# kessel/dune-pnp

Hardware: NVIDIA B200
Metric: newton_step_dofs_per_s (higher is better)
Workload: dtype f64

## Files before the change

### dune_pnp_b200/capi.py

```python
import ctypes as C
import os

import numpy as np

_HERE = os.path.dirname(os.path.abspath(__file__))
LIB_PATH = os.path.join(_HERE, "libpnp_b200.so")

OP_PB, OP_POISSON, OP_DIFFUSION, OP_MASS, OP_PNP = range(5)
JAC_FD_FAITHFUL, JAC_ANALYTIC = 0, 1
SOLVER_BCGS, SOLVER_CG = 0, 1
PREC_NONE, PREC_JACOBI, PREC_SSOR, PREC_ILU0, PREC_AMG = range(5)
TIME_ALEXANDER2, TIME_IMPLICIT_EULER = 0, 1
STATUS = {0: "PNP_OK", 1: "PNP_E_NOT_CONVERGED", 2: "PNP_E_LINEAR_SOLVER", 3: "PNP_E_LINE_SEARCH", 4: "PNP_E_NAN",
          5: "PNP_E_BREAKDOWN", 6: "PNP_E_CUDA", 7: "PNP_E_CONFIG", 8: "PNP_E_ARG", 9: "PNP_E_MESH"}

_dp = C.POINTER(C.c_double)
_ip = C.POINTER(C.c_int)


class LinResult(C.Structure):
    _fields_ = [("converged", C.c_int), ("iterations", C.c_int), ("reduction", C.c_double), ("conv_rate", C.c_double),
                ("seconds", C.c_double), ("status", C.c_int)]


class NewtonOpts(C.Structure):
    _fields_ = [("reduction", C.c_double), ("abs_limit", C.c_double), ("min_linear_reduction", C.c_double),
                ("reassemble_threshold", C.c_double), ("max_iterations", C.c_int),
                ("line_search_max_iterations", C.c_int), ("damping", C.c_double), ("jac_mode", C.c_int),
                ("fd_epsilon", C.c_double), ("verbosity", C.c_int), ("line_search_strategy", C.c_int)]


class NewtonResult(C.Structure):
    _fields_ = [("converged", C.c_int), ("iterations", C.c_int), ("first_defect", C.c_double), ("defect", C.c_double),
                ("reduction", C.c_double), ("linear_iterations", C.c_int), ("line_search_trials", C.c_int),
                ("jacobian_assemblies", C.c_int), ("residual_assemblies", C.c_int), ("seconds_assembly", C.c_double),
                ("seconds_solve", C.c_double), ("seconds_total", C.c_double), ("n_history", C.c_int),
                ("defect_history", C.c_double * 64), ("linear_iterations_history", C.c_int * 64)]


class PnpError(RuntimeError):
    def __init__(self, status, msg):
        super().__init__("%s: %s" % (STATUS.get(status, status), msg))
        self.status = status


_LIB = None


def lib():
    global _LIB
    if _LIB is None:
        if not os.path.exists(LIB_PATH):
            raise ImportError("libpnp_b200.so is missing: run `python -c 'import __graft_entry__ as g; g.build()'` "
                              "(make -C dune_pnp_b200/csrc)")
        try:
            import importlib.util
            for pkg, names in (("nvidia.nccl", ["libnccl.so.2"]), ("nvidia.nvjitlink", ["libnvJitLink.so.12"]),
                               ("nvidia.cublas", ["libcublasLt.so.12", "libcublas.so.12"]),
                               ("nvidia.cusparse", ["libcusparse.so.12"]), ("nvidia.cusolver", ["libcusolver.so.11"])):
                spec = importlib.util.find_spec(pkg)
                if spec is None or not spec.submodule_search_locations:
                    continue
                for nm in names:
                    cand = os.path.join(list(spec.submodule_search_locations)[0], "lib", nm)
                    if os.path.exists(cand):
                        C.CDLL(cand, mode=C.RTLD_GLOBAL)
        except Exception:
            pass
        L = C.CDLL(LIB_PATH)
        L.pnp_last_error.restype = C.c_char_p
        L.pnp_launch_count.restype = C.c_long
        _LIB = L
    return _LIB


def _d(a):
    return None if a is None else a.ctypes.data_as(_dp)


def _i(a):
    return None if a is None else a.ctypes.data_as(_ip)


def tune(name, value):
    st = lib().pnp_tune(name.encode(), C.c_double(value))
    if st != 0:
        raise PnpError(st, "unknown tuning knob " + name)


class Context:

    def __init__(self, device=0, parent=None):
        self._h = C.c_void_p()
        self._children = []
        if parent is not None:
            st = lib().pnp_ctx_create_child(parent._h, C.byref(self._h))
            parent._children.append(self)
        else:
            st = lib().pnp_ctx_create(device, C.byref(self._h))
        if st != 0:
            raise PnpError(st, "cannot create a context on CUDA device %d (no CPU fallback exists)" % device)

    def close(self):
        if self._h:
            lib().pnp_ctx_destroy(self._h)
            self._h = C.c_void_p()

    def __del__(self):
        try:
            self.close()
        except Exception:
            pass

    def _ck(self, st):
        if st != 0:
            raise PnpError(st, lib().pnp_last_error(self._h).decode())

    def profile_spmv(self, enable):
        self._ck(lib().pnp_profile_spmv(self._h, int(enable)))

    def profile_spmv_get(self):
        n = (C.c_long * 3)(); ms = (C.c_double * 3)()
        self._ck(lib().pnp_profile_spmv_get(self._h, n, ms))
        return list(n), list(ms)

    def profile_bytes(self, reset=False):
        out = (C.c_double * 6)()
        self._ck(lib().pnp_profile_bytes(self._h, int(reset), out))
        return dict(zip(("spmv_fine", "spmv_coarse", "assembly", "blas1", "transfer", "dense"), list(out)))

    def profiler_range(self, start):
        self._ck(lib().pnp_profiler_range(self._h, int(start)))

    def timer_start(self):
        self._ck(lib().pnp_timer_start(self._h))

    def timer_stop(self):
        ms = C.c_double()
        self._ck(lib().pnp_timer_stop(self._h, C.byref(ms)))
        return ms.value

    def launch_count(self):
        return lib().pnp_launch_count(self._h)

    def mesh_set(self, x, y, tri, ba, bb, bphys):
        x = np.ascontiguousarray(x, dtype=np.float64); y = np.ascontiguousarray(y, dtype=np.float64)
        tri = np.ascontiguousarray(tri, dtype=np.int32); ba = np.ascontiguousarray(ba, dtype=np.int32)
        bb = np.ascontiguousarray(bb, dtype=np.int32); bphys = np.ascontiguousarray(bphys, dtype=np.int32)
        self._ck(lib().pnp_mesh_set(self._h, C.c_long(len(x)), _d(x), _d(y), C.c_long(len(tri)), _i(tri), C.c_long(len(ba)),
                                    _i(ba), _i(bb), _i(bphys)))

    def mesh_read_gmsh(self, path):
        self._ck(lib().pnp_mesh_read_gmsh(self._h, path.encode()))

    def mesh_refine(self, levels):
        self._ck(lib().pnp_mesh_refine(self._h, levels))

    def carry_set(self, vecs):
        arr = (C.c_int * len(vecs))(*vecs)
        self._ck(lib().pnp_carry_set(self._h, arr, len(vecs)))

    def carry_get(self, index, vec):
        self._ck(lib().pnp_carry_get(self._h, index, vec))

    def carry_set_host(self, field):
        field = np.ascontiguousarray(field, dtype=np.float64)
        self._ck(lib().pnp_carry_set_host(self._h, field.shape[0] if field.ndim == 2 else 1, _d(field)))

    def carry_get_host(self, index, fields):
        out = np.zeros((fields, self.mesh_sizes()["nv"]))
        self._ck(lib().pnp_carry_get_host(self._h, index, _d(out)))
        return out

    def mesh_set_local(self, n_own, x, y, tri, ba, bb, bphys):
        x = np.ascontiguousarray(x, dtype=np.float64); y = np.ascontiguousarray(y, dtype=np.float64)
        tri = np.ascontiguousarray(tri, dtype=np.int32); ba = np.ascontiguousarray(ba, dtype=np.int32)
        bb = np.ascontiguousarray(bb, dtype=np.int32); bphys = np.ascontiguousarray(bphys, dtype=np.int32)
        self._ck(lib().pnp_mesh_set_local(self._h, C.c_long(len(x)), C.c_long(n_own), _d(x), _d(y), C.c_long(len(tri)), _i(tri),
                                          C.c_long(len(ba)), _i(ba), _i(bb), _i(bphys)))

    def mesh_owned(self):
        n = C.c_long()
        self._ck(lib().pnp_mesh_owned(self._h, C.byref(n)))
        return n.value

    @staticmethod
    def comm_unique_id():
        buf = C.create_string_buffer(128)
        if lib().pnp_comm_unique_id(buf) != 0:
            raise PnpError(6, "ncclGetUniqueId failed")
        return buf.raw

    def comm_init(self, rank, world, unique_id):
        self._ck(lib().pnp_comm_init(self._h, rank, world, C.c_char_p(unique_id) if world > 1 else None))

    def halo_set(self, nbr, send_ptr, send_idx, recv_ptr):
        nbr = np.ascontiguousarray(nbr, dtype=np.int32); send_ptr = np.ascontiguousarray(send_ptr, dtype=np.int32)
        send_idx = np.ascontiguousarray(send_idx, dtype=np.int32); recv_ptr = np.ascontiguousarray(recv_ptr, dtype=np.int32)
        self._ck(lib().pnp_halo_set(self._h, len(nbr), _i(nbr), _i(send_ptr), _i(send_idx), _i(recv_ptr)))

    def mg_push_level(self, child, par0, par1):
        par0 = np.ascontiguousarray(par0, dtype=np.int32); par1 = np.ascontiguousarray(par1, dtype=np.int32)
        self._ck(lib().pnp_mg_push_level(self._h, child._h, _i(par0), _i(par1)))

    def mg_set_coarse_global(self, gid, n_global):
        gid = np.ascontiguousarray(gid, dtype=np.int32)
        self._ck(lib().pnp_mg_set_coarse_global(self._h, _i(gid), C.c_long(n_global)))

    def mg_set_coarse_replica(self, replica, gid, n_global):
        gid = np.ascontiguousarray(gid, dtype=np.int32)
        self._ck(lib().pnp_mg_set_coarse_replica(self._h, replica._h, _i(gid), C.c_long(n_global)))

    def mg_set_coarse_aggregates(self, agg, n_agg):
        agg = np.ascontiguousarray(agg, dtype=np.int32)
        self._ck(lib().pnp_mg_set_coarse_aggregates(self._h, _i(agg), C.c_long(n_agg)))

    def halo_exchange(self, vec):
        self._ck(lib().pnp_halo_exchange(self._h, vec))

    def mesh_finalize(self, renumber=True):
        self._ck(lib().pnp_mesh_finalize(self._h, int(renumber)))

    def mesh_sizes(self):
        v = [C.c_long() for _ in range(4)]
        self._ck(lib().pnp_mesh_sizes(self._h, *[C.byref(a) for a in v]))
        return dict(nv=v[0].value, nT=v[1].value, nB=v[2].value, nslots=v[3].value)

    def mesh_get(self):
        s = self.mesh_sizes()
        x = np.zeros(s["nv"]); y = np.zeros(s["nv"]); tri = np.zeros((s["nT"], 3), dtype=np.int32)
        ba = np.zeros(s["nB"], dtype=np.int32); bb = np.zeros(s["nB"], dtype=np.int32); ph = np.zeros(s["nB"], dtype=np.int32)
        self._ck(lib().pnp_mesh_get(self._h, _d(x), _d(y), _i(tri), _i(ba), _i(bb), _i(ph)))
        return dict(x=x, y=y, tri=tri, ba=ba, bb=bb, bphys=ph)

    def params_set(self, sys, surf):
        sys = np.ascontiguousarray(sys, dtype=np.float64); surf = np.ascontiguousarray(surf, dtype=np.float64)
        self._ck(lib().pnp_params_set(self._h, _d(sys), _d(surf)))

    def params_read(self, path):
        self._ck(lib().pnp_params_read(self._h, path.encode()))

    def params_get(self):
        sys = np.zeros(16)
        self._ck(lib().pnp_params_get(self._h, _d(sys), None, None, 0))
        surf = np.zeros((int(sys[0]), 9)); buf = C.create_string_buffer(512)
        self._ck(lib().pnp_params_get(self._h, _d(sys), _d(surf), buf, 512))
        return sys, surf, buf.value.decode()

    def operator(self, op, comp0=0):
        h = C.c_int()
        self._ck(lib().pnp_operator_create(self._h, op, comp0, C.byref(h)))
        return h.value

    def operator_set_coefficient(self, op, which, vec):
        self._ck(lib().pnp_operator_set_coefficient(self._h, op, which, vec))

    def operator_set_valency(self, op, valency):
        self._ck(lib().pnp_operator_set_valency(self._h, op, C.c_double(valency)))

    def constraints(self, op, fields):
        out = np.zeros(fields * self.ndof(), dtype=np.int8)
        self._ck(lib().pnp_constraints_get(self._h, op, out.ctypes.data_as(C.c_char_p)))
        return out.astype(bool)

    def pattern(self, op, fields):
        nv = self.ndof()
        nnz = C.c_long(); rowptr = np.zeros(fields * nv + 1, dtype=np.int32)
        self._ck(lib().pnp_pattern_get(self._h, op, C.byref(nnz), _i(rowptr), None))
        col = np.zeros(nnz.value, dtype=np.int32)
        self._ck(lib().pnp_pattern_get(self._h, op, C.byref(nnz), _i(rowptr), _i(col)))
        return rowptr, col

    def vec(self, fields, host=None):
        h = C.c_int()
        self._ck(lib().pnp_vec_create(self._h, fields, C.byref(h)))
        if host is not None:
            self.upload(h.value, host)
        return h.value
# ... 158 lines not shown
```

### dune_pnp_b200/csrc/pnp_amg.cu

```cuda
#include <cub/cub.cuh>
#include <cusolverDn.h>

#include <chrono>
#include <cmath>
#include <cstdlib>
#include <cstring>

#include "pnp_common.cuh"
#include "pnp_spmv_tma.cuh"
#include "pnp_sweep.cuh"

namespace pnp {

std::shared_ptr<SweepPlan> sweep_plan_build(Ctx&, const SweepView&, int F);
void sweep_gs(Ctx&, const SweepPlan&, const SweepView&, const double* vals, long stride, const double* d, double* x, int dir);

namespace {

constexpr int BLK = 256;

struct Level {
  int nv = 0; long nslots = 0;
  const int* rp = nullptr; const unsigned* col = nullptr; const double* vals = nullptr;
  DBuf<int> rp_own; DBuf<unsigned> col_own; DBuf<double> vals_own;
  DBuf<double> dinv, x, x2, b, r;
  double lmax = 2.0;
  DBuf<int> agg, par1;
  DBuf<int> agg_ptr, agg_mem;
  DBuf<int> seg_ptr, seg_items;
  DBuf<unsigned char> seg_w;
  double alpha = 1.0;
  Ctx* lc = nullptr;
  Vec u; Matrix Amat;
  const unsigned char* dm = nullptr;
  bool redisc = false;
  DBuf<XY> xy_own; DBuf<unsigned char> dmask_own;
  std::shared_ptr<SweepPlan> gs_plan;
};

}

struct Amg {
  int NP = 1, F = 1;
  bool symbolic = false;
  long nv0 = -1, nslots0 = -1;
  long mg_epoch = -1;
  double sym_key = 0.0;
  double omega = 0.7, alpha = 1.6;
  int coarse_sweeps = 40;
  int gamma = 1;
  int wlevels = 99;
  int smoother = 0;
  double cheb_ratio = 8.0;
  int comp0 = 0;
  int pre_steps = -1, post_steps = -1;
  int dense_max = 4096, dense_n = 0;
  cusolverDnHandle_t cus = nullptr;
  DBuf<double> dense, dense_work;
  DBuf<int> dense_piv, dense_info;
  bool distributed = false;
  bool redisc = false;
  DBuf<double> grhs;
  std::unique_ptr<Solver> rep_solver; Matrix rep_A; Vec rep_u; DBuf<double> rep_x;
  int n_geo = 0;
  std::vector<std::unique_ptr<Level>> L;
  DBuf<unsigned char> tmp;
  void* temp(size_t bytes) { if (bytes > tmp.n) tmp.alloc(bytes); return tmp.p; }
  cudaGraphExec_t cg_exec = nullptr;
  bool cg_failed = false;
  int cg_calls = 0;
  double cg_key[8] = {0, 0, 0, 0, 0, 0, 0, 0};
  std::vector<std::pair<double*, double*>> cg_before, cg_after;
  long cg_launches = 0; double cg_bytes[Ctx::ACC_N] = {0, 0, 0, 0, 0, 0};
  void cg_reset() { if (cg_exec) cudaGraphExecDestroy(cg_exec); cg_exec = nullptr; cg_calls = 0; }
  ~Amg() { if (cg_exec) cudaGraphExecDestroy(cg_exec); if (cus) cusolverDnDestroy(cus); }
};

namespace {

__device__ __forceinline__ unsigned hash32(unsigned x) {
  x ^= x >> 16; x *= 0x7feb352du; x ^= x >> 15; x *= 0x846ca68bu; x ^= x >> 16;
  return x;
}
__global__ void k_mis_select(const int* __restrict__ rp, const unsigned* __restrict__ col, int nv,
                             const unsigned char* __restrict__ st, unsigned char* __restrict__ st_out) {
  for (int v = blockIdx.x * blockDim.x + threadIdx.x; v < nv; v += gridDim.x * blockDim.x) {
    unsigned char s = st[v];
    if (s == 0) {
      const unsigned pv = hash32((unsigned)v);
      bool win = true;
      for (int k = rp[v] + 1; k < rp[v + 1]; k++) {
        const int w = (int)(col[k] & STAR_VMASK);
        if (w >= nv || w == v || st[w] != 0) continue;
        const unsigned pw = hash32((unsigned)w);
        if (pw > pv || (pw == pv && w > v)) { win = false; break; }
      }
      if (win) s = 1;
    }
    st_out[v] = s;
  }
}
__global__ void k_mis_cover(const int* __restrict__ rp, const unsigned* __restrict__ col, int nv,
                            unsigned char* __restrict__ st, int* __restrict__ undecided) {
  int local = 0;
  for (int v = blockIdx.x * blockDim.x + threadIdx.x; v < nv; v += gridDim.x * blockDim.x) {
    if (st[v] != 0) continue;
    bool covered = false;
    for (int k = rp[v] + 1; k < rp[v + 1]; k++) {
      const int w = (int)(col[k] & STAR_VMASK);
      if (w < nv && st[w] == 1) { covered = true; break; }
    }
    if (covered) st[v] = 2; else local++;
  }
  if (local) atomicAdd(undecided, local);
}
__global__ void k_root_flag(const unsigned char* __restrict__ st, int nv, int* __restrict__ flag) {
  for (int v = blockIdx.x * blockDim.x + threadIdx.x; v < nv; v += gridDim.x * blockDim.x) flag[v] = st[v] == 1;
}
__global__ void k_attach(const int* __restrict__ rp, const unsigned* __restrict__ col, const double* __restrict__ vals,
                         int nv, const unsigned char* __restrict__ st, const int* __restrict__ root_id,
                         int* __restrict__ agg) {
  for (int v = blockIdx.x * blockDim.x + threadIdx.x; v < nv; v += gridDim.x * blockDim.x) {
    if (st[v] == 1) { agg[v] = root_id[v]; continue; }
    double best = -1.0; int bw = -1;
    for (int k = rp[v] + 1; k < rp[v + 1]; k++) {
      const int w = (int)(col[k] & STAR_VMASK);
      if (w >= nv || st[w] != 1) continue;
      const double s = fabs(vals[k]);
      if (s > best || (s == best && w < bw)) { best = s; bw = w; }
    }
    agg[v] = root_id[bw];
  }
}
__global__ void k_coarse_keys(const int* __restrict__ rp, const unsigned* __restrict__ col, int nv,
                              const int* __restrict__ agg, uint64_t* __restrict__ keys, int* __restrict__ slot_id) {
  for (int v = blockIdx.x * blockDim.x + threadIdx.x; v < nv; v += gridDim.x * blockDim.x) {
    const unsigned I = (unsigned)agg[v];
    for (int k = rp[v]; k < rp[v + 1]; k++) {
      const unsigned w = col[k] & STAR_VMASK;
      if (w >= (unsigned)nv) { keys[k] = ~0ull; slot_id[k] = k; continue; }
      const unsigned J = (unsigned)agg[w];
      keys[k] = ((uint64_t)I << 32) | (J == I ? 0u : J + 1u);
      slot_id[k] = k;
    }
  }
}
__global__ void k_coarse_cols(const uint64_t* __restrict__ ukeys, long n, unsigned* __restrict__ col) {
  for (long i = blockIdx.x * (long)blockDim.x + threadIdx.x; i < n; i += (long)gridDim.x * blockDim.x) {
    const unsigned lo = (unsigned)(ukeys[i] & 0xffffffffu);
    col[i] = lo == 0 ? (unsigned)(ukeys[i] >> 32) : lo - 1u;
  }
}
__global__ void k_row_starts(const uint64_t* __restrict__ ukeys, long n, int nc, int* __restrict__ rp) {
  for (int I = blockIdx.x * blockDim.x + threadIdx.x; I <= nc; I += gridDim.x * blockDim.x)
    rp[I] = (int)lower_bound_u64(ukeys, n, (uint64_t)(unsigned)I << 32);
}
__global__ void k_lower_bounds_i32(const int* __restrict__ sorted, int n, int m, int* __restrict__ out) {
  for (int I = blockIdx.x * blockDim.x + threadIdx.x; I <= m; I += gridDim.x * blockDim.x) {
    int lo = 0, hi = n;
    while (lo < hi) { int mid = (lo + hi) >> 1; if (sorted[mid] < I) lo = mid + 1; else hi = mid; }
    out[I] = lo;
  }
}
__global__ void k_iota(int* a, int n) {
  for (int i = blockIdx.x * blockDim.x + threadIdx.x; i < n; i += gridDim.x * blockDim.x) a[i] = i;
}

template <int NP>
__global__ void k_galerkin(const int* __restrict__ seg_ptr, const int* __restrict__ seg_items,
                           const unsigned char* __restrict__ seg_w, long nsc, const double* __restrict__ vf, long nsf, double* __restrict__ vc,
                           const unsigned char* __restrict__ dmask, const unsigned* __restrict__ colf, const int* __restrict__ rpf,
                           int comp0) {
  for (long cs = blockIdx.x * (long)blockDim.x + threadIdx.x; cs < nsc; cs += (long)gridDim.x * blockDim.x) {
    double acc[NP];
#pragma unroll
    for (int p = 0; p < NP; p++) acc[p] = 0.0;
    constexpr int U = 4;
    const int t1 = seg_ptr[cs + 1];
    for (int t0 = seg_ptr[cs]; t0 < t1; t0 += U) {
      int s[U]; double w[U]; double v[U][NP];
#pragma unroll
      for (int q = 0; q < U; q++) {
        const bool ok = t0 + q < t1;
        s[q] = ok ? seg_items[t0 + q] : -1;
        const unsigned char wc = (ok && seg_w) ? seg_w[t0 + q] : 0;
        w[q] = ok ? (wc == 0 ? 1.0 : (wc == 1 ? 0.5 : 0.25)) : 0.0;
      }
#pragma unroll
      for (int q = 0; q < U; q++)
#pragma unroll
        for (int p = 0; p < NP; p++) v[q][p] = s[q] >= 0 ? vf[p * nsf + s[q]] : 0.0;
      if (dmask) {
#pragma unroll
        for (int q = 0; q < U; q++) {
          if (s[q] < 0) continue;
          const unsigned wv = colf[s[q]] & STAR_VMASK;
          const unsigned m = dmask[wv];
          if (m && rpf[wv] == s[q]) {
            if (NP == 1) { if ((m >> comp0) & 1u) v[q][0] = 0.0; }
            else if (NP == PNP_COMPACT_PLANES) { if (m & 1u) v[q][0] = 0.0; }
            else {
              if (m & 1u) v[q][0] = 0.0;
              if (m & 2u) v[q][NP == 7 ? 4 : 0] = 0.0;
              if (m & 4u) v[q][NP == 7 ? 6 : 0] = 0.0;
            }
          }
        }
      }
#pragma unroll
      for (int q = 0; q < U; q++)
        if (s[q] >= 0) {
#pragma unroll
          for (int p = 0; p < NP; p++) acc[p] += w[q] * v[q][p];
        }
    }
#pragma unroll
    for (int p = 0; p < NP; p++) vc[p * nsc + cs] = acc[p];
  }
}
template <int NP>
__global__ void k_dinv(const int* __restrict__ rp, const double* __restrict__ vals, long stride, int nv,
                       double* __restrict__ dinv) {
  for (int v = blockIdx.x * blockDim.x + threadIdx.x; v < nv; v += gridDim.x * blockDim.x) {
    const int s = rp[v];
    if (NP == 1) { const double d = vals[s]; dinv[v] = d != 0.0 ? 1.0 / d : 0.0; }
// ... 74 lines not shown
      const double w = (par1 && par1[v] >= 0) ? 0.5 : 1.0;
#pragma unroll
      for (int k = 0; k < F; k++) acc[k] += w * r[F * v + k];
    }
#pragma unroll
    for (int k = 0; k < F; k++) bc[(long)F * I + k] = acc[k];
  }
}
template <int F>
__global__ void k_prolong(const int* __restrict__ agg, const int* __restrict__ par1, int nv, const double* __restrict__ xc,
                          double alpha, double* __restrict__ x, const unsigned char* __restrict__ dmask, int comp0) {
  for (int v = blockIdx.x * blockDim.x + threadIdx.x; v < nv; v += gridDim.x * blockDim.x) {
    const long I = agg[v];
    const long J = par1 ? par1[v] : -1;
    const unsigned m = dmask ? (F == 3 ? dmask[v] : (dmask[v] >> comp0) & 1u) : 0u;
#pragma unroll
    for (int k = 0; k < F; k++)
      if (!((m >> k) & 1u))
        x[(long)F * v + k] += alpha * (J >= 0 ? 0.5 * (xc[F * I + k] + xc[F * J + k]) : xc[F * I + k]);
  }
}
__global__ void k_level_geometry(const int* __restrict__ int2ext_c, const int* __restrict__ ext2int_f, const XY* __restrict__ xy_f,
                                 const unsigned char* __restrict__ dmask_f, int nvc, XY* __restrict__ xy_c,
                                 unsigned char* __restrict__ dmask_c) {
  for (int i = blockIdx.x * blockDim.x + threadIdx.x; i < nvc; i += gridDim.x * blockDim.x) {
    const int j = ext2int_f[int2ext_c[i]];
    xy_c[i] = xy_f[j]; dmask_c[i] = dmask_f[j];
  }
}
__global__ void k_geo_parents(const int* __restrict__ int2ext_f, int nvf, int nvc, const uint64_t* __restrict__ edges,
                              const int* __restrict__ ext2int_c, int* __restrict__ par0, int* __restrict__ par1) {
  for (int i = blockIdx.x * blockDim.x + threadIdx.x; i < nvf; i += gridDim.x * blockDim.x) {
    const int e = int2ext_f[i];
    if (e < nvc) { par0[i] = ext2int_c[e]; par1[i] = -1; }
    else {
      const uint64_t k = edges[e - nvc];
      par0[i] = ext2int_c[(int)(k >> 32)]; par1[i] = ext2int_c[(int)(k & 0xffffffffu)];
    }
  }
}
__global__ void k_geo_pairs(const int* __restrict__ par0, const int* __restrict__ par1, int nvf, int nrows_c,
                            int* __restrict__ key, int* __restrict__ val) {
  for (int i = blockIdx.x * blockDim.x + threadIdx.x; i < nvf; i += gridDim.x * blockDim.x) {
    key[2 * i] = (par0[i] >= 0 && par0[i] < nrows_c) ? par0[i] : 0x7fffffff; val[2 * i] = i;
    key[2 * i + 1] = (par1[i] >= 0 && par1[i] < nrows_c) ? par1[i] : 0x7fffffff; val[2 * i + 1] = i;
  }
}
template <int F>
__global__ void k_inject(const int* __restrict__ par0, const int* __restrict__ par1, int nvf, const double* __restrict__ uf,
                         double* __restrict__ uc) {
  for (int i = blockIdx.x * blockDim.x + threadIdx.x; i < nvf; i += gridDim.x * blockDim.x)
    if (par1[i] < 0 && par0[i] >= 0) {
#pragma unroll
      for (int k = 0; k < F; k++) uc[(long)F * par0[i] + k] = uf[(long)F * i + k];
    }
}
template <int F>
__global__ void k_mask_dirichlet(double* __restrict__ b, const unsigned char* __restrict__ dmask, int nv, int comp0) {
  for (int v = blockIdx.x * blockDim.x + threadIdx.x; v < nv; v += gridDim.x * blockDim.x) {
    const unsigned m = F == 3 ? dmask[v] : (dmask[v] >> comp0) & 1u;
#pragma unroll
    for (int k = 0; k < F; k++) if ((m >> k) & 1u) b[(long)F * v + k] = 0.0;
  }
}
template <int NP>
__global__ void k_dense_fill_global(const int* __restrict__ rp, const unsigned* __restrict__ col, const double* __restrict__ vals,
                                    long stride, int nrows, const int* __restrict__ gid, double* __restrict__ Ad, long n,
                                    const unsigned char* __restrict__ dmask, int comp0) {
  constexpr int F = NP == 1 ? 1 : 3;
  for (int r = blockIdx.x * blockDim.x + threadIdx.x; r < nrows; r += gridDim.x * blockDim.x) {
    const long rg = gid[r];
    for (int s = rp[r]; s < rp[r + 1]; s++) {
      const long cg = gid[col[s] & STAR_VMASK];
      const unsigned dm = (dmask && s == rp[r]) ? dmask[r] : 0u;
      if (NP == 1) { if (!((dm >> comp0) & 1u)) atomicAdd(&Ad[cg * n + rg], vals[s]); }
      else {
        const PnpBlock B = pnp_block_at<NP>(vals, stride, s);
#pragma unroll
        for (int ki = 0; ki < 3; ki++)
#pragma unroll
          for (int kj = 0; kj < 3; kj++)
            if (pnp_plane(ki, kj) >= 0 && !(ki == kj && ((dm >> ki) & 1u))) atomicAdd(&Ad[(F * cg + kj) * n + F * rg + ki], B.at(ki, kj));
      }
    }
  }
}
template <int F>
__global__ void k_to_global(const double* __restrict__ loc, const int* __restrict__ gid, int nrows, double* __restrict__ glob) {
  for (int v = blockIdx.x * blockDim.x + threadIdx.x; v < nrows; v += gridDim.x * blockDim.x)
#pragma unroll
    for (int k = 0; k < F; k++) atomicAdd(&glob[(long)F * gid[v] + k], loc[(long)F * v + k]);
}
template <int F>
__global__ void k_add_from_global(const double* __restrict__ glob, const int* __restrict__ gid, int nrows, double alpha,
                                  double* __restrict__ x, const unsigned char* __restrict__ dmask, int comp0) {
  for (int v = blockIdx.x * blockDim.x + threadIdx.x; v < nrows; v += gridDim.x * blockDim.x) {
    const unsigned m = F == 3 ? dmask[v] : (dmask[v] >> comp0) & 1u;
#pragma unroll
    for (int k = 0; k < F; k++) if (!((m >> k) & 1u)) x[(long)F * v + k] += alpha * glob[(long)F * gid[v] + k];
  }
}
template <int F>
__global__ void k_from_global(const double* __restrict__ glob, const int* __restrict__ gid, int nloc, double* __restrict__ loc) {
  for (int v = blockIdx.x * blockDim.x + threadIdx.x; v < nloc; v += gridDim.x * blockDim.x)
#pragma unroll
    for (int k = 0; k < F; k++) loc[(long)F * v + k] = glob[(long)F * gid[v] + k];
}
__device__ __forceinline__ int find_slot(const int* rp, const unsigned* col, int I, int J) {
  for (int s = rp[I]; s < rp[I + 1]; s++) if ((int)(col[s] & STAR_VMASK) == J) return s;
  return -1;
}
__global__ void k_geo_items(const int* __restrict__ rpf, const unsigned* __restrict__ colf, int nvf,
                            const int* __restrict__ par0, const int* __restrict__ par1, const int* __restrict__ rpc,
                            const unsigned* __restrict__ colc, int* __restrict__ key, unsigned* __restrict__ val,
                            int* __restrict__ err) {
  for (int i = blockIdx.x * blockDim.x + threadIdx.x; i < nvf; i += gridDim.x * blockDim.x) {
    const int I[2] = {par0[i], par1[i]};
    for (int s = rpf[i]; s < rpf[i + 1]; s++) {
      const int j = (int)(colf[s] & STAR_VMASK);
      const int J[2] = {par0[j], par1[j]};
#pragma unroll
      for (int a = 0; a < 2; a++)
#pragma unroll
        for (int b = 0; b < 2; b++) {
          const long o = 4l * s + 2 * a + b;
          if (I[a] < 0 || J[b] < 0) { key[o] = 0x7fffffff; val[o] = 0; continue; }
          const int cs = find_slot(rpc, colc, I[a], J[b]);
          if (cs < 0) { atomicExch(err, 1); key[o] = 0x7fffffff; val[o] = 0; continue; }
          const unsigned wc = (I[1] >= 0 ? 1u : 0u) + (J[1] >= 0 ? 1u : 0u);
          key[o] = cs; val[o] = (unsigned)s | (wc << 29);
        }
    }
  }
}
__global__ void k_geo_unpack(const unsigned* __restrict__ val, long n, int* __restrict__ items, unsigned char* __restrict__ w) {
  for (long t = blockIdx.x * (long)blockDim.x + threadIdx.x; t < n; t += (long)gridDim.x * blockDim.x) {
    items[t] = (int)(val[t] & 0x1fffffffu); w[t] = (unsigned char)(val[t] >> 29);
  }
}

#define KL(c, kern, n, ...)                                                                              \
  do { kern<<<grid_for((n), BLK), BLK, 0, (c).stream>>>(__VA_ARGS__); PNP_CHECK_LAUNCH(); (c).launches++; } while (0)

template <int EPI>
void level_op(Ctx& c, const Amg& A, const Level& l, const double* x, const double* b, double* y, double omega_or_c2 = -1.0,
              double c1 = 0.0, double* dvec = nullptr) {
  StarOpArgs a{l.rp, l.col, l.vals, l.nslots, l.nv, x, y};
  a.b = b; a.dinv = l.dinv.p; a.block = A.F == 3; a.omega = omega_or_c2 < 0 ? A.omega : omega_or_c2; a.c1 = c1; a.dvec = dvec;
  const bool fine = &l == A.L[0].get();
  if (A.distributed) halo_exchange(*l.lc, const_cast<double*>(x), A.F);
  if (fine) c.prof_mark(EPI == EPI_RESIDUAL ? 1 : 2);
  launch_star_op_auto<EPI, 0>(c, A.NP, a, fine);
  if (fine) c.prof_mark();
}

bool coarsen(Ctx& c, Amg& A, int li) {
  Level& f = *A.L[li];
  const int nv = f.nv;
  DBuf<unsigned char> st(nv), st2(nv);
  st.zero(c.stream);
  DBuf<int> d_und(1);
  for (int round = 0; round < 200; round++) {
    KL(c, k_mis_select, nv, f.rp, f.col, nv, st.p, st2.p);
    std::swap(st.p, st2.p);
    d_und.zero(c.stream);
    KL(c, k_mis_cover, nv, f.rp, f.col, nv, st.p, d_und.p);
    int und = 0;
    d_und.download(&und, 1, c.stream);
    if (und == 0) break;
    PNP_REQUIRE(round < 199, PNP_E_ARG, "AMG: independent-set selection did not terminate");
  }
  DBuf<int> flag(nv), root_id(nv);
  KL(c, k_root_flag, nv, st.p, nv, flag.p);
  size_t bytes = 0;
  cub::DeviceScan::ExclusiveSum(nullptr, bytes, flag.p, root_id.p, nv, c.stream);
  PNP_CUDA(cub::DeviceScan::ExclusiveSum(A.temp(bytes), bytes, flag.p, root_id.p, nv, c.stream));
  int last_id = 0, last_flag = 0;
  PNP_CUDA(cudaMemcpyAsync(&last_id, root_id.p + nv - 1, sizeof(int), cudaMemcpyDeviceToHost, c.stream));
  PNP_CUDA(cudaMemcpyAsync(&last_flag, flag.p + nv - 1, sizeof(int), cudaMemcpyDeviceToHost, c.stream));
  PNP_CUDA(cudaStreamSynchronize(c.stream));
  const int nc = last_id + last_flag;
  if (nc < 1 || nc > 0.8 * nv) return false;
  f.alpha = A.alpha;
  f.agg.alloc(nv);
  KL(c, k_attach, nv, f.rp, f.col, f.vals, nv, st.p, root_id.p, f.agg.p);
  {
    DBuf<int> ids(nv), agg_sorted(nv);
    f.agg_mem.alloc(nv); f.agg_ptr.alloc(nc + 1);
    KL(c, k_iota, nv, ids.p, nv);
    cub::DeviceRadixSort::SortPairs(nullptr, bytes, f.agg.p, agg_sorted.p, ids.p, f.agg_mem.p, nv, 0, 32, c.stream);
    PNP_CUDA(cub::DeviceRadixSort::SortPairs(A.temp(bytes), bytes, f.agg.p, agg_sorted.p, ids.p, f.agg_mem.p, nv, 0, 32,
                                            c.stream));
    KL(c, k_lower_bounds_i32, nc + 1, agg_sorted.p, nv, nc, f.agg_ptr.p);
  }
  auto nl = std::make_unique<Level>();
  {
    const long ns = f.nslots;
    PNP_REQUIRE(ns < (1l << 31), PNP_E_MESH, "AMG: too many matrix slots on one level");
    DBuf<uint64_t> keys(ns), skeys(ns), ukeys(ns);
    DBuf<int> slot(ns), counts(ns + 1), d_nu(1);
    f.seg_items.alloc(ns);
    KL(c, k_coarse_keys, nv, f.rp, f.col, nv, f.agg.p, keys.p, slot.p);
    cub::DeviceRadixSort::SortPairs(nullptr, bytes, keys.p, skeys.p, slot.p, f.seg_items.p, (int)ns, 0, 64, c.stream);
    PNP_CUDA(cub::DeviceRadixSort::SortPairs(A.temp(bytes), bytes, keys.p, skeys.p, slot.p, f.seg_items.p, (int)ns, 0, 64,
                                            c.stream));
    cub::DeviceRunLengthEncode::Encode(nullptr, bytes, skeys.p, ukeys.p, counts.p, d_nu.p, (int)ns, c.stream);
    PNP_CUDA(cub::DeviceRunLengthEncode::Encode(A.temp(bytes), bytes, skeys.p, ukeys.p, counts.p, d_nu.p, (int)ns, c.stream));
    int nu = 0;
    d_nu.download(&nu, 1, c.stream);
    {
      uint64_t lastkey = 0;
      PNP_CUDA(cudaMemcpyAsync(&lastkey, ukeys.p + (nu - 1), sizeof(uint64_t), cudaMemcpyDeviceToHost, c.stream));
      PNP_CUDA(cudaStreamSynchronize(c.stream));
      if (lastkey == ~0ull) nu--;
    }
    nl->nv = nc; nl->nslots = nu;
    PNP_CUDA(cudaMemsetAsync(counts.p + nu, 0, sizeof(int), c.stream));
    f.seg_ptr.alloc((size_t)nu + 1);
    cub::DeviceScan::ExclusiveSum(nullptr, bytes, counts.p, f.seg_ptr.p, nu + 1, c.stream);
    PNP_CUDA(cub::DeviceScan::ExclusiveSum(A.temp(bytes), bytes, counts.p, f.seg_ptr.p, nu + 1, c.stream));
    nl->rp_own.alloc((size_t)nc + 1); nl->col_own.alloc(nu);
    KL(c, k_row_starts, nc + 1, ukeys.p, (long)nu, nc, nl->rp_own.p);
    KL(c, k_coarse_cols, nu, ukeys.p, (long)nu, nl->col_own.p);
    c.launches += 8;
    PNP_CUDA(cudaStreamSynchronize(c.stream));
  }
  nl->vals_own.alloc((size_t)A.NP * nl->nslots);
  nl->rp = nl->rp_own.p; nl->col = nl->col_own.p; nl->vals = nl->vals_own.p;
  A.L.push_back(std::move(nl));
  return true;
}

void coarsen_geometric(Ctx& c, Amg& A, int li, const HierLevel& h, const int* int2ext_f, bool redisc) {
  Level& f = *A.L[li];
  const int nvf = f.nv, nvc = (int)h.nv;
  size_t bytes = 0;
  f.agg.alloc(nvf); f.par1.alloc(nvf);
  KL(c, k_geo_parents, nvf, int2ext_f, nvf, nvc, h.edges.p, h.ext2int.p, f.agg.p, f.par1.p);
  {
    DBuf<int> key(2 * (size_t)nvf), val(2 * (size_t)nvf), skey(2 * (size_t)nvf), sval(2 * (size_t)nvf);
    KL(c, k_geo_pairs, nvf, f.agg.p, f.par1.p, nvf, nvc, key.p, val.p);
    cub::DeviceRadixSort::SortPairs(nullptr, bytes, key.p, skey.p, val.p, sval.p, 2 * nvf, 0, 32, c.stream);
    PNP_CUDA(cub::DeviceRadixSort::SortPairs(A.temp(bytes), bytes, key.p, skey.p, val.p, sval.p, 2 * nvf, 0, 32, c.stream));
    f.agg_ptr.alloc((size_t)nvc + 1);
    KL(c, k_lower_bounds_i32, nvc + 1, skey.p, 2 * nvf, nvc, f.agg_ptr.p);
    int nvalid = 0;
    PNP_CUDA(cudaMemcpyAsync(&nvalid, f.agg_ptr.p + nvc, sizeof(int), cudaMemcpyDeviceToHost, c.stream));
    PNP_CUDA(cudaStreamSynchronize(c.stream));
    f.agg_mem.alloc(nvalid);
    PNP_CUDA(cudaMemcpyAsync(f.agg_mem.p, sval.p, (size_t)nvalid * sizeof(int), cudaMemcpyDeviceToDevice, c.stream));
    PNP_CUDA(cudaStreamSynchronize(c.stream));
  }
  auto nl = std::make_unique<Level>();
  nl->nv = nvc; nl->nslots = h.nslots; nl->rp = h.rp.p; nl->col = h.adj.p;
  nl->redisc = redisc;
  if (redisc) {
    nl->xy_own.alloc(nvc); nl->dmask_own.alloc(nvc);
    KL(c, k_level_geometry, nvc, h.int2ext.p, c.ext2int.p, c.xy.p, c.dmask.p, nvc, nl->xy_own.p, nl->dmask_own.p);
    nl->dm = nl->dmask_own.p;
    nl->u.fields = A.F; nl->u.d.alloc((size_t)A.F * nvc);
  } else {
    const long n4 = 4 * f.nslots;
    PNP_REQUIRE(n4 < (1l << 31) && f.nslots < (1l << 29), PNP_E_MESH, "multigrid: too many matrix slots on one level");
    DBuf<int> key(n4), skey(n4), err(1);
    DBuf<unsigned> val(n4), sval(n4);
    err.zero(c.stream);
    KL(c, k_geo_items, nvf, f.rp, f.col, nvf, f.agg.p, f.par1.p, nl->rp, nl->col, key.p, val.p, err.p);
    int herr = 0;
    err.download(&herr, 1, c.stream);
    PNP_REQUIRE(herr == 0, PNP_E_MESH, "multigrid: refinement levels are not nested");
    cub::DeviceRadixSort::SortPairs(nullptr, bytes, key.p, skey.p, val.p, sval.p, (int)n4, 0, 32, c.stream);
    PNP_CUDA(cub::DeviceRadixSort::SortPairs(A.temp(bytes), bytes, key.p, skey.p, val.p, sval.p, (int)n4, 0, 32, c.stream));
    key.release(); val.release();
    f.seg_ptr.alloc((size_t)nl->nslots + 1);
    KL(c, k_lower_bounds_i32, nl->nslots + 1, skey.p, (int)n4, (int)nl->nslots, f.seg_ptr.p);
    int nvalid = 0;
    PNP_CUDA(cudaMemcpyAsync(&nvalid, f.seg_ptr.p + nl->nslots, sizeof(int), cudaMemcpyDeviceToHost, c.stream));
    PNP_CUDA(cudaStreamSynchronize(c.stream));
    f.seg_items.alloc(nvalid); f.seg_w.alloc(nvalid);
    KL(c, k_geo_unpack, nvalid, sval.p, (long)nvalid, f.seg_items.p, f.seg_w.p);
    PNP_CUDA(cudaStreamSynchronize(c.stream));
    c.launches += 4;
  }
  f.alpha = 1.0;
  nl->vals_own.alloc((size_t)A.NP * nl->nslots);
  nl->vals = nl->vals_own.p;
  A.L.push_back(std::move(nl));
}

void alloc_work(Ctx& c, Amg& A, Level& l) {
  const size_t n = (size_t)A.F * l.nv, nall = (A.distributed && l.lc) ? (size_t)A.F * l.lc->nv : n;
  l.dinv.alloc(A.F == 3 ? 9 * (size_t)l.nv : n); l.x.alloc(nall); l.x2.alloc(nall); l.b.alloc(nall); l.r.alloc(nall);
  l.x.zero(c.stream); l.x2.zero(c.stream); l.b.zero(c.stream); l.r.zero(c.stream);
}

void coarsen_distributed(Ctx& c, Amg& A, int li, MgLevelRef& ref) {
  Level& f = *A.L[li];
  Ctx& fc = *f.lc; Ctx& kc = *ref.lc;
  const int nvf_all = (int)fc.nv, nvc = (int)kc.n_own;
  size_t bytes = 0;
  f.agg.alloc(nvf_all); f.par1.alloc(nvf_all);
  PNP_CUDA(cudaMemcpyAsync(f.agg.p, ref.par0.p, nvf_all * sizeof(int), cudaMemcpyDeviceToDevice, c.stream));
  PNP_CUDA(cudaMemcpyAsync(f.par1.p, ref.par1.p, nvf_all * sizeof(int), cudaMemcpyDeviceToDevice, c.stream));
  {
    DBuf<int> key(2 * (size_t)nvf_all), val(2 * (size_t)nvf_all), skey(2 * (size_t)nvf_all), sval(2 * (size_t)nvf_all);
    KL(c, k_geo_pairs, nvf_all, f.agg.p, f.par1.p, nvf_all, nvc, key.p, val.p);
// ... 115 lines not shown
  for (int r = blockIdx.x * blockDim.x + threadIdx.x; r < nv; r += gridDim.x * blockDim.x)
    for (int s = rp[r]; s < rp[r + 1]; s++) {
      const long cidx = col[s] & STAR_VMASK;
      if (cidx >= nv) continue;
      if (NP == 1) Ad[cidx * n + r] = vals[s];
      else {
        const PnpBlock B = pnp_block_at<NP>(vals, stride, s);
#pragma unroll
        for (int ki = 0; ki < 3; ki++)
#pragma unroll
          for (int kj = 0; kj < 3; kj++)
            if (pnp_plane(ki, kj) >= 0) Ad[(F * cidx + kj) * n + F * r + ki] = B.at(ki, kj);
      }
    }
}
__global__ void k_dense_fix_diag(double* __restrict__ Ad, long n) {
  for (long i = blockIdx.x * (long)blockDim.x + threadIdx.x; i < n; i += (long)gridDim.x * blockDim.x)
    if (Ad[i * n + i] == 0.0) Ad[i * n + i] = 1.0;
}
#define PNP_CUSOLVER(call)                                                                                          \
  do { cusolverStatus_t s_ = (call); if (s_ != CUSOLVER_STATUS_SUCCESS)                                             \
    throw ::pnp::Error(PNP_E_CUDA, std::string(#call) + " -> cusolver status " + std::to_string((int)s_)); } while (0)

void dense_factor(Ctx& c, Amg& A) {
  Level& l = *A.L.back();
  const long n = (long)A.F * l.nv;
  A.dense_n = (int)n;
  if (!A.cus) PNP_CUSOLVER(cusolverDnCreate(&A.cus));
  PNP_CUSOLVER(cusolverDnSetStream(A.cus, c.stream));
  if (A.dense.n != (size_t)(n * n)) { A.dense.alloc(n * n); A.dense_piv.alloc(n); A.dense_info.alloc(1); }
  A.dense.zero(c.stream);
  if (A.NP == 1) KL(c, k_dense_fill<1>, l.nv, l.rp, l.col, l.vals, l.nslots, l.nv, A.dense.p, n);
  else if (A.NP == PNP_COMPACT_PLANES) KL(c, k_dense_fill<PNP_COMPACT_PLANES>, l.nv, l.rp, l.col, l.vals, l.nslots, l.nv, A.dense.p, n);
  else KL(c, k_dense_fill<7>, l.nv, l.rp, l.col, l.vals, l.nslots, l.nv, A.dense.p, n);
  KL(c, k_dense_fix_diag, n, A.dense.p, n);
  int lwork = 0;
  PNP_CUSOLVER(cusolverDnDgetrf_bufferSize(A.cus, (int)n, (int)n, A.dense.p, (int)n, &lwork));
  if (A.dense_work.n < (size_t)lwork) A.dense_work.alloc(lwork);
  PNP_CUSOLVER(cusolverDnDgetrf(A.cus, (int)n, (int)n, A.dense.p, (int)n, A.dense_work.p, A.dense_piv.p, A.dense_info.p));
  c.acct(Ctx::ACC_DENSE, 24.0 * (double)n * (double)n);
  int info = 0;
  A.dense_info.download(&info, 1, c.stream);
  PNP_REQUIRE(info == 0, PNP_E_BREAKDOWN, "multigrid: coarsest-level matrix is singular (LU info " + std::to_string(info) + ")");
}
void dense_solve(Ctx& c, Amg& A, Level& l) {
  const long n = A.dense_n;
  PNP_CUDA(cudaMemcpyAsync(l.x.p, l.b.p, n * sizeof(double), cudaMemcpyDeviceToDevice, c.stream));
  PNP_CUSOLVER(cusolverDnDgetrs(A.cus, CUBLAS_OP_N, (int)n, 1, A.dense.p, (int)n, A.dense_piv.p, l.x.p, (int)n, A.dense_info.p));
  c.launches += 2; c.acct(Ctx::ACC_DENSE, 8.0 * (double)n * (double)n);
}

void dense_factor_global(Ctx& c, Amg& A) {
  Level& l = *A.L.back();
  const long n = (long)A.F * c.mg_nglobal;
  A.dense_n = (int)n;
  if (!A.cus) PNP_CUSOLVER(cusolverDnCreate(&A.cus));
  PNP_CUSOLVER(cusolverDnSetStream(A.cus, c.stream));
  if (A.dense.n != (size_t)(n * n)) { A.dense.alloc(n * n); A.dense_piv.alloc(n); A.dense_info.alloc(1); A.grhs.alloc(n); }
  A.dense.zero(c.stream);
  const unsigned char* dm = c.mg_aggregated ? l.lc->dmask.p : nullptr;
  if (A.NP == 1) KL(c, k_dense_fill_global<1>, l.nv, l.rp, l.col, l.vals, l.nslots, l.nv, c.mg_gid.p, A.dense.p, n, dm, A.comp0);
  else if (A.NP == PNP_COMPACT_PLANES)
    KL(c, k_dense_fill_global<PNP_COMPACT_PLANES>, l.nv, l.rp, l.col, l.vals, l.nslots, l.nv, c.mg_gid.p, A.dense.p, n, dm, A.comp0);
  else KL(c, k_dense_fill_global<7>, l.nv, l.rp, l.col, l.vals, l.nslots, l.nv, c.mg_gid.p, A.dense.p, n, dm, A.comp0);
  allreduce_sum(c, A.dense.p, (size_t)(n * n));
  KL(c, k_dense_fix_diag, n, A.dense.p, n);
  int lwork = 0;
  PNP_CUSOLVER(cusolverDnDgetrf_bufferSize(A.cus, (int)n, (int)n, A.dense.p, (int)n, &lwork));
  if (A.dense_work.n < (size_t)lwork) A.dense_work.alloc(lwork);
  static const bool timing = std::getenv("PNP_AMG_TIMING") != nullptr;
  if (timing) PNP_CUDA(cudaStreamSynchronize(c.stream));
  const auto t0 = std::chrono::steady_clock::now();
  PNP_CUSOLVER(cusolverDnDgetrf(A.cus, (int)n, (int)n, A.dense.p, (int)n, A.dense_work.p, A.dense_piv.p, A.dense_info.p));
  int info = 0;
  A.dense_info.download(&info, 1, c.stream);
  if (timing) std::printf("[amg] rank %d global dense LU n = %ld: %.1f ms\n", c.rank, n,
                          1e3 * std::chrono::duration<double>(std::chrono::steady_clock::now() - t0).count());
  PNP_REQUIRE(info == 0, PNP_E_BREAKDOWN, "multigrid: coarsest-level matrix is singular (LU info " + std::to_string(info) + ")");
}
void dense_correct_aggregated(Ctx& c, Amg& A, Level& l) {
  const long n = A.dense_n;
  A.grhs.zero(c.stream);
  if (A.F == 1) KL(c, k_to_global<1>, l.nv, l.r.p, c.mg_gid.p, l.nv, A.grhs.p);
  else KL(c, k_to_global<3>, l.nv, l.r.p, c.mg_gid.p, l.nv, A.grhs.p);
  allreduce_sum(c, A.grhs.p, (size_t)n);
  PNP_CUSOLVER(cusolverDnDgetrs(A.cus, CUBLAS_OP_N, (int)n, 1, A.dense.p, (int)n, A.dense_piv.p, A.grhs.p, (int)n, A.dense_info.p));
  if (A.F == 1) KL(c, k_add_from_global<1>, l.nv, A.grhs.p, c.mg_gid.p, l.nv, A.alpha, l.x.p, l.lc->dmask.p, A.comp0);
  else KL(c, k_add_from_global<3>, l.nv, A.grhs.p, c.mg_gid.p, l.nv, A.alpha, l.x.p, l.lc->dmask.p, A.comp0);
  c.launches += 2;
}
void dense_solve_global(Ctx& c, Amg& A, Level& l) {
  const long n = A.dense_n;
  A.grhs.zero(c.stream);
  if (A.F == 1) KL(c, k_to_global<1>, l.nv, l.b.p, c.mg_gid.p, l.nv, A.grhs.p);
  else KL(c, k_to_global<3>, l.nv, l.b.p, c.mg_gid.p, l.nv, A.grhs.p);
  allreduce_sum(c, A.grhs.p, (size_t)n);
  PNP_CUSOLVER(cusolverDnDgetrs(A.cus, CUBLAS_OP_N, (int)n, 1, A.dense.p, (int)n, A.dense_piv.p, A.grhs.p, (int)n, A.dense_info.p));
  const int nloc = (int)l.lc->nv;
  if (A.F == 1) KL(c, k_from_global<1>, nloc, A.grhs.p, c.mg_gid.p, nloc, l.x.p);
  else KL(c, k_from_global<3>, nloc, A.grhs.p, c.mg_gid.p, nloc, l.x.p);
  c.launches += 2;
}

}
void amg_setup(Ctx& c, Solver& S, const Matrix& M);
void amg_apply(Ctx& c, Solver& S, const Matrix&, const double* d, double* y);
namespace {
void replica_setup(Ctx& c, Amg& A) {
  Ctx& rc = *c.mg_replica;
  Level& l = *A.L.back();
  const long n = (long)A.F * c.mg_nglobal;
  A.dense_n = (int)n;
  if (A.grhs.n != (size_t)n) { A.grhs.alloc(n); A.rep_x.alloc(n); A.rep_u.d.alloc(n); }
  A.rep_u.fields = A.F;
  A.rep_u.d.zero(c.stream);
  if (A.F == 1) KL(c, k_to_global<1>, l.nv, l.u.d.p, c.mg_gid.p, l.nv, A.rep_u.d.p);
  else KL(c, k_to_global<3>, l.nv, l.u.d.p, c.mg_gid.p, l.nv, A.rep_u.d.p);
  allreduce_sum(c, A.rep_u.d.p, (size_t)n);
  Operator op = c.last_op; op.aux0 = op.aux1 = -1;
  A.rep_A.op = op.op; A.rep_A.nplanes = A.NP;
  if (A.rep_A.vals.n != (size_t)A.NP * rc.nslots) A.rep_A.vals.alloc((size_t)A.NP * rc.nslots);
  rc.launches = 0;
  assemble_jacobian(rc, op, A.rep_u, A.rep_A, c.last_mode, c.last_eps);
  if (!A.rep_solver) { A.rep_solver = std::make_unique<Solver>(); A.rep_solver->prec = PNP_PREC_AMG; }
  auto& ro = A.rep_solver->opts;
  ro["amg_geometric"] = 1;  ro["amg_omega"] = A.omega; ro["amg_alpha"] = A.alpha; ro["amg_gamma"] = A.gamma;
  ro["amg_dense_max"] = A.dense_max; ro["amg_coarse_sweeps"] = A.coarse_sweeps; ro["amg_smoother"] = A.smoother;
  ro["amg_cheb_ratio"] = A.cheb_ratio; ro["amg_pre_steps"] = A.pre_steps; ro["amg_post_steps"] = A.post_steps;
  amg_setup(rc, *A.rep_solver, A.rep_A);
  c.absorb(rc);
}
void replica_solve(Ctx& c, Amg& A, Level& l, int nu) {
  Ctx& rc = *c.mg_replica;
  const long n = (long)A.F * c.mg_nglobal;
  A.grhs.zero(c.stream);
  if (A.F == 1) KL(c, k_to_global<1>, l.nv, l.b.p, c.mg_gid.p, l.nv, A.grhs.p);
  else KL(c, k_to_global<3>, l.nv, l.b.p, c.mg_gid.p, l.nv, A.grhs.p);
  allreduce_sum(c, A.grhs.p, (size_t)n);
  A.rep_solver->prec_steps = nu;
  rc.launches = 0;
  amg_apply(rc, *A.rep_solver, A.rep_A, A.grhs.p, A.rep_x.p);
  const int nloc = (int)l.lc->nv;
  if (A.F == 1) KL(c, k_from_global<1>, nloc, A.rep_x.p, c.mg_gid.p, nloc, l.x.p);
  else KL(c, k_from_global<3>, nloc, A.rep_x.p, c.mg_gid.p, nloc, l.x.p);
  c.absorb(rc); c.launches += 2;
}

void jacobi0(Ctx& c, Amg& A, Level& l, double omega, double* dvec) {
  if (A.F == 1) KL(c, k_jacobi0<1>, l.nv, l.dinv.p, l.b.p, omega, l.x.p, l.nv, dvec);
  else KL(c, k_jacobi0<3>, l.nv, l.dinv.p, l.b.p, omega, l.x.p, l.nv, dvec);
  c.acct(Ctx::ACC_TRANSFER, ((A.F == 3 ? 72.0 : 8.0) + 16.0 * A.F + (dvec ? 8.0 * A.F : 0.0)) * l.nv);
}

void smooth(Ctx& c, Amg& A, Level& l, int steps, bool zero) {
  const long n = (long)A.F * l.nv;
  if (steps <= 0) { if (zero) PNP_CUDA(cudaMemsetAsync(l.x.p, 0, n * sizeof(double), c.stream)); return; }
  if (A.smoother == 0) {
    int s = 0;
    if (zero) { jacobi0(c, A, l, A.omega, nullptr); s = 1; }
    for (; s < steps; s++) { level_op<2>(c, A, l, l.x.p, l.b.p, l.x2.p); std::swap(l.x.p, l.x2.p); }
    return;
  }
  if (A.smoother == 2) {
    const bool finest = &l == A.L[0].get();
    const SweepView V{l.rp, l.col, finest ? c.int2ext.p : nullptr, l.nv};
    if (!l.gs_plan) l.gs_plan = sweep_plan_build(c, V, A.F);
    if (zero) PNP_CUDA(cudaMemsetAsync(l.x.p, 0, n * sizeof(double), c.stream));
    for (int s = 0; s < steps; s++) {
      sweep_gs(c, *l.gs_plan, V, l.vals, l.nslots, l.b.p, l.x.p, +1);
      sweep_gs(c, *l.gs_plan, V, l.vals, l.nslots, l.b.p, l.x.p, -1);
    }
    c.acct(finest ? Ctx::ACC_SPMV_FINE : Ctx::ACC_SPMV_COARSE, 2.0 * steps * ((8.0 * A.NP + 4.0) * (double)l.nslots + 24.0 * n));
    return;
  }
  const double lmx = 1.1 * l.lmax, lmn = l.lmax / A.cheb_ratio;
  const double theta = 0.5 * (lmx + lmn), delta = 0.5 * (lmx - lmn), sigma = theta / delta;
  double rho = 1.0 / sigma;
  int s = 0;
  if (zero) { jacobi0(c, A, l, 1.0 / theta, l.r.p); s = 1; }
  else { level_op<3>(c, A, l, l.x.p, l.b.p, l.x2.p, 1.0 / theta, 0.0, l.r.p); std::swap(l.x.p, l.x2.p); s = 1; }
  for (; s < steps; s++) {
    const double rho_new = 1.0 / (2.0 * sigma - rho);
    level_op<3>(c, A, l, l.x.p, l.b.p, l.x2.p, 2.0 * rho_new / delta, rho_new * rho, l.r.p);
    std::swap(l.x.p, l.x2.p);
    rho = rho_new;
  }
}

void cycle(Ctx& c, Amg& A, int li, int nu, int comp0, bool zero);

void coarse_correction(Ctx& c, Amg& A, int nu, int comp0) {
  auto direct = [&] {
    const int visits = 0 < A.wlevels ? A.gamma : 1;
    for (int g = 0; g < visits; g++) cycle(c, A, 1, nu, comp0, g == 0);
  };
  auto snapshot = [&](std::vector<std::pair<double*, double*>>& v) {
    v.clear();
    for (size_t li = 1; li < A.L.size(); li++) v.push_back({A.L[li]->x.p, A.L[li]->x2.p});
  };
  auto restore = [&](const std::vector<std::pair<double*, double*>>& v) {
    for (size_t li = 1; li < A.L.size(); li++) { A.L[li]->x.p = v[li - 1].first; A.L[li]->x2.p = v[li - 1].second; }
  };
  cudaStreamCaptureStatus cap = cudaStreamCaptureStatusNone;
  PNP_CUDA(cudaStreamIsCapturing(c.stream, &cap));
  if (!tune().graph || A.cg_failed || A.smoother != 0 || cap != cudaStreamCaptureStatusNone) { direct(); return; }
  const double key[8] = {(double)nu, A.omega, (double)A.gamma, (double)A.wlevels, (double)A.pre_steps, (double)A.post_steps,
                         (double)A.coarse_sweeps, (double)comp0 + 16.0 * A.dense_n};
  if (A.cg_exec && std::memcmp(key, A.cg_key, sizeof key) != 0) A.cg_reset();
  if (!A.cg_exec) {
    if (A.cg_calls++ < 1) { direct(); return; }
    std::memcpy(A.cg_key, key, sizeof key);
    snapshot(A.cg_before);
    const long l0 = c.launches;
    double b0[Ctx::ACC_N];
    for (int k = 0; k < Ctx::ACC_N; k++) b0[k] = c.alg_bytes[k];
    cudaGraph_t graph = nullptr;
    bool ok = cudaStreamBeginCapture(c.stream, cudaStreamCaptureModeThreadLocal) == cudaSuccess;
    if (ok) {
      try { direct(); } catch (const Error&) { ok = false; }
      if (cudaStreamEndCapture(c.stream, &graph) != cudaSuccess || !graph) ok = false;
    }
    if (ok && cudaGraphInstantiate(&A.cg_exec, graph, 0) != cudaSuccess) { ok = false; A.cg_exec = nullptr; }
    if (graph) cudaGraphDestroy(graph);
    A.cg_launches = c.launches - l0; c.launches = l0;
    for (int k = 0; k < Ctx::ACC_N; k++) { A.cg_bytes[k] = c.alg_bytes[k] - b0[k]; c.alg_bytes[k] = b0[k]; }
    snapshot(A.cg_after);
    if (!ok) {
      cudaGetLastError();
      A.cg_failed = true; A.cg_exec = nullptr;
      restore(A.cg_before);
      direct();
      return;
    }
  }
  restore(A.cg_before);
  PNP_CUDA(cudaGraphLaunch(A.cg_exec, c.stream));
  restore(A.cg_after);
  c.launches += A.cg_launches;
  for (int k = 0; k < Ctx::ACC_N; k++) c.alg_bytes[k] += A.cg_bytes[k];
}

void cycle(Ctx& c, Amg& A, int li, int nu, int comp0, bool zero) {
  Level& l = *A.L[li];
  const bool coarsest = li + 1 == (int)A.L.size();
  if (coarsest && A.dense_n > 0 && A.distributed && c.mg_aggregated) {
    smooth(c, A, l, nu, zero);
    level_op<1>(c, A, l, l.x.p, l.b.p, l.r.p);
    dense_correct_aggregated(c, A, l);
    smooth(c, A, l, nu, false);
    return;
  }
  if (coarsest && A.dense_n > 0) {
    if (A.distributed && c.mg_replica) replica_solve(c, A, l, nu);
    else if (A.distributed) dense_solve_global(c, A, l);
    else dense_solve(c, A, l);
    return;
  }
  const int nu_pre = A.pre_steps >= 0 ? A.pre_steps : nu, nu_post = A.post_steps >= 0 ? A.post_steps : nu;
  smooth(c, A, l, coarsest ? A.coarse_sweeps : nu_pre, zero);
  if (coarsest) return;
  Level& nx = *A.L[li + 1];
  level_op<1>(c, A, l, l.x.p, l.b.p, l.r.p);
  if (A.distributed) halo_exchange(*l.lc, l.r.p, A.F);
  if (A.F == 1) KL(c, k_restrict<1>, nx.nv, l.agg_ptr.p, l.agg_mem.p, l.par1.p, nx.nv, l.r.p, nx.b.p);
  else KL(c, k_restrict<3>, nx.nv, l.agg_ptr.p, l.agg_mem.p, l.par1.p, nx.nv, l.r.p, nx.b.p);
  c.acct(Ctx::ACC_TRANSFER, (8.0 * A.F + 4.0) * l.nv + 4.0 * (double)l.agg_mem.n + (8.0 * A.F + 4.0) * nx.nv);
  if (nx.dm) {
    if (A.F == 1) KL(c, k_mask_dirichlet<1>, nx.nv, nx.b.p, nx.dm, nx.nv, comp0);
    else KL(c, k_mask_dirichlet<3>, nx.nv, nx.b.p, nx.dm, nx.nv, comp0);
    c.acct(Ctx::ACC_TRANSFER, 1.0 * nx.nv);
  }
  if (li == 0) coarse_correction(c, A, nu, comp0);
  else {
    const int visits = li < A.wlevels ? A.gamma : 1;
    for (int g = 0; g < visits; g++) cycle(c, A, li + 1, nu, comp0, g == 0);
  }
  if (A.distributed && !(li + 2 == (int)A.L.size() && A.dense_n > 0 && !c.mg_aggregated)) halo_exchange(*nx.lc, nx.x.p, A.F);
  const unsigned char* dm = l.dm;
  if (A.F == 1) KL(c, k_prolong<1>, l.nv, l.agg.p, l.par1.p, l.nv, nx.x.p, l.alpha, l.x.p, dm, comp0);
  else KL(c, k_prolong<3>, l.nv, l.agg.p, l.par1.p, l.nv, nx.x.p, l.alpha, l.x.p, dm, comp0);
  c.acct(Ctx::ACC_TRANSFER, (16.0 * A.F + 9.0) * l.nv + 8.0 * A.F * nx.nv);
  smooth(c, A, l, nu_post, false);
}

}

int amg_graph_state(const Solver& S) { return !S.amg ? 0 : (S.amg->cg_exec ? 1 : (S.amg->cg_failed ? -1 : 0)); }

void amg_setup(Ctx& c, Solver& S, const Matrix& M) {
  if (!S.amg) S.amg = std::make_shared<Amg>();
  Amg& A = *S.amg;
  const int comp0 = M.comp0;
  A.comp0 = comp0;
  const bool want_redisc = S.opt("amg_geometric", 1) != 0 && S.opt("amg_rediscretise", 1) != 0 && c.n_own == c.nv &&
                           !c.hier.empty() && c.mg.empty() && c.last_u && c.last_vals == M.vals.p &&
                           (M.op == OP_PB || M.op == OP_PNP || M.op == OP_MASS);
  const double sym_key = S.opt("amg_geometric", 1) + 3.0 * S.opt("amg_dense_max", 4096) + 1e7 * S.opt("amg_alpha", 1.6);
  if (!A.symbolic || A.NP != M.nplanes || A.nv0 != c.n_own || A.nslots0 != c.nslots || A.redisc != want_redisc ||
      A.mg_epoch != c.mg_epoch || A.sym_key != sym_key) {
    A.L.clear(); A.cg_reset(); A.cg_failed = false;
    A.NP = M.nplanes; A.F = M.nplanes == 1 ? 1 : 3;
    A.nv0 = c.n_own; A.nslots0 = c.nslots; A.mg_epoch = c.mg_epoch; A.sym_key = sym_key;
    auto l0 = std::make_unique<Level>();
    l0->nv = (int)c.n_own; l0->nslots = c.nslots; l0->rp = c.rp.p; l0->col = c.adj.p; l0->vals = M.vals.p;
    A.L.push_back(std::move(l0));
    A.alpha = S.opt("amg_alpha", 1.6);
    A.L[0]->lc = &c;
    A.L[0]->dm = c.dmask.p;
    A.redisc = want_redisc;
    A.distributed = S.opt("amg_geometric", 1) != 0 && !c.mg.empty() && c.mg_nglobal > 0 &&
                    (M.op == OP_PB || M.op == OP_PNP || M.op == OP_MASS);
    if (A.distributed) {
      for (auto& ref : c.mg) coarsen_distributed(c, A, (int)A.L.size() - 1, ref);
      A.n_geo = (int)c.mg.size();
    }
    const bool geometric = !A.distributed && S.opt("amg_geometric", 1) != 0 && c.n_own == c.nv && !c.hier.empty();
    if (!A.distributed) A.n_geo = 0;
    if (geometric) {
      const int* i2e = c.int2ext.p;
      const double* uf = c.last_u;
      for (int hi = (int)c.hier.size() - 1; hi >= 0; hi--) {
        const int li = (int)A.L.size() - 1;
        coarsen_geometric(c, A, li, c.hier[hi], i2e, A.redisc);
        i2e = c.hier[hi].int2ext.p;
        uf = level_values(c, A, li, uf, comp0);
        A.n_geo++;
      }
    }
    A.dense_max = (int)S.opt("amg_dense_max", 4096);
    for (int li = (int)A.L.size() - 1; li < 24 && !A.distributed; li++) {
      if (A.L[li]->nv <= 64 || (long)A.F * A.L[li]->nv <= A.dense_max) break;
      if (!coarsen(c, A, li)) break;
      level_values(c, A, li, nullptr, comp0);
    }
    for (auto& l : A.L) alloc_work(c, A, *l);
    if (!A.distributed) {
      Level& l0r = *A.L[0];
      const size_t nall = (size_t)A.F * c.nv;
      l0r.x.alloc(nall); l0r.x2.alloc(nall);
      l0r.x.zero(c.stream); l0r.x2.zero(c.stream);
    }
    A.symbolic = true;
    if (S.verbosity > 0) {
      std::printf("multigrid hierarchy (%d geometric transfers):", A.n_geo);
      for (auto& l : A.L) std::printf(" %d", l->nv);
      std::printf("\n");
    }
  }
  A.L[0]->vals = M.vals.p;
  static const bool timing = std::getenv("PNP_AMG_TIMING") != nullptr;
  if (timing) PNP_CUDA(cudaStreamSynchronize(c.stream));
  const auto t_num0 = std::chrono::steady_clock::now();
  A.omega = S.opt("amg_omega", 0.7); A.gamma = (int)S.opt("amg_gamma", 1); A.wlevels = (int)S.opt("amg_wlevels", 99);
  A.coarse_sweeps = (int)S.opt("amg_coarse_sweeps", 40); A.smoother = (int)S.opt("amg_smoother", 0);
  PNP_REQUIRE(A.smoother >= 0 && A.smoother <= 2, PNP_E_ARG, "amg_smoother: 0 damped Jacobi, 1 Chebyshev, 2 symmetric Gauss-Seidel");
  PNP_REQUIRE(A.smoother != 2 || !A.distributed, PNP_E_ARG, "the Gauss-Seidel smoother sweeps the rows of one GPU: use Jacobi / Chebyshev on a partitioned mesh");
  PNP_REQUIRE(A.smoother != 2 || A.NP != PNP_COMPACT_PLANES, PNP_E_ARG, "the Gauss-Seidel smoother sweeps 7-plane PNP matrices only");
  A.cheb_ratio = S.opt("amg_cheb_ratio", 8.0);
  A.pre_steps = (int)S.opt("amg_pre_steps", -1); A.post_steps = (int)S.opt("amg_post_steps", -1);
  numeric(c, A, comp0);
  if (timing) {
    PNP_CUDA(cudaStreamSynchronize(c.stream));
    std::printf("[amg] rank %d numeric setup %.1f ms (levels %zu, dense n = %d, distributed %d)\n", c.rank,
                1e3 * std::chrono::duration<double>(std::chrono::steady_clock::now() - t_num0).count(), A.L.size(), A.dense_n,
                (int)A.distributed);
  }
}

void amg_apply(Ctx& c, Solver& S, const Matrix&, const double* d, double* y) {
  Amg& A = *S.amg;
  Level& l0 = *A.L[0];
  const long n = (long)A.F * l0.nv;
  const int nu = S.prec_steps > 0 ? S.prec_steps : 1;
  if (c.n_own == c.nv) {
    double *keep_b = l0.b.p, *keep_x = l0.x.p, *keep_x2 = l0.x2.p;
    const int pre = A.pre_steps >= 0 ? A.pre_steps : nu, post = A.post_steps >= 0 ? A.post_steps : nu;
    const int swaps = A.smoother == 2 ? 0 : (pre > 0 ? pre - 1 : 0) + post;
    struct Restore {
      Level& l; double *b, *x, *x2;
      ~Restore() { l.b.p = b; l.x.p = x; l.x2.p = x2; }
    } restore{l0, keep_b, keep_x, keep_x2};
    l0.b.p = const_cast<double*>(d);
    if (swaps & 1) l0.x2.p = y; else l0.x.p = y;
    cycle(c, A, 0, nu, A.comp0, true);
    double* result = l0.x.p;
    if (result != y) { PNP_CUDA(cudaMemcpyAsync(y, result, n * sizeof(double), cudaMemcpyDeviceToDevice, c.stream)); c.acct(Ctx::ACC_BLAS1, 16.0 * n); }
    return;
  }
  PNP_CUDA(cudaMemcpyAsync(l0.b.p, d, n * sizeof(double), cudaMemcpyDeviceToDevice, c.stream));
  cycle(c, A, 0, nu, A.comp0, true);
  PNP_CUDA(cudaMemcpyAsync(y, l0.x.p, n * sizeof(double), cudaMemcpyDeviceToDevice, c.stream));
}

}
```

### dune_pnp_b200/csrc/pnp_capi.cu

```cuda
#include <cuda_profiler_api.h>

#include <cstring>

#include "pnp_common.cuh"

namespace pnp {
int newton_apply(Ctx&, const Operator&, Vec&, Solver&, const pnp_newton_opts&, pnp_newton_result&);
int amg_graph_state(const Solver&);
LinResult slp_apply(Ctx&, const Operator&, Vec&, Solver&, double, int, double);
int onestep_apply(Ctx&, int, const Operator&, const Operator&, Solver&, double, Vec&, Vec&, Vec&, double, int, double, LinResult*);
namespace {
__global__ void k_fill(double* x, long n, double v) {
  for (long i = blockIdx.x * (long)blockDim.x + threadIdx.x; i < n; i += (long)gridDim.x * blockDim.x) x[i] = v;
}
__global__ void k_pack3(const double* a, const double* b, const double* c, long nv, double* out) {
  for (long i = blockIdx.x * (long)blockDim.x + threadIdx.x; i < nv; i += (long)gridDim.x * blockDim.x) {
    out[3 * i] = a[i]; out[3 * i + 1] = b[i]; out[3 * i + 2] = c[i];
  }
}
__global__ void k_extract(const double* in, long nv, int field, double* out) {
  for (long i = blockIdx.x * (long)blockDim.x + threadIdx.x; i < nv; i += (long)gridDim.x * blockDim.x) out[i] = in[3 * i + field];
}
void to_lin(const LinResult& lr, pnp_lin_result* out) {
  if (!out) return;
  out->converged = lr.converged; out->iterations = lr.iterations; out->reduction = lr.reduction;
  out->conv_rate = lr.conv_rate; out->seconds = lr.seconds; out->status = lr.status;
}
}
}

using namespace pnp;


#define API_BEGIN(ctx)                                  \
  if (!(ctx)) return PNP_E_ARG;                         \
  Ctx& c = (ctx)->c;                                    \
  try {                                                 \
    PNP_CUDA(cudaSetDevice(c.device));
#define API_END                                                      \
    return PNP_OK;                                                   \
  } catch (const pnp::Error& e) { c.err = e.what(); return e.code; } \
  catch (const std::exception& e) { c.err = e.what(); return PNP_E_ARG; }

namespace pnp {
Ctx* ctx_make_owned_child(Ctx& p) {
  pnp_ctx* h = new pnp_ctx;
  h->c.device = p.device; h->c.stream = p.stream; h->c.owns_stream = false; h->c.sm_count = p.sm_count;
  h->c.params = p.params;
  h->c.parent = &p; p.children.push_back(&h->c);
  p.owned_children.push_back(h);
  return &h->c;
}
void ctx_destroy_owned_child(Ctx& p, Ctx* child) {
  for (size_t i = 0; i < p.owned_children.size(); i++) {
    pnp_ctx* h = (pnp_ctx*)p.owned_children[i];
    if (&h->c != child) continue;
    p.owned_children.erase(p.owned_children.begin() + i);
    pnp_ctx_destroy(h);
    return;
  }
}
}

extern "C" {

pnp_status pnp_ctx_create(int device, pnp_ctx** out) {
  if (!out) return PNP_E_ARG;
  *out = nullptr;
  int ndev = 0;
  if (cudaGetDeviceCount(&ndev) != cudaSuccess || device < 0 || device >= ndev) return PNP_E_CUDA;
  pnp_ctx* h = new pnp_ctx;
  h->c.device = device;
  if (cudaSetDevice(device) != cudaSuccess || cudaStreamCreate(&h->c.stream) != cudaSuccess) { delete h; return PNP_E_CUDA; }
  cudaDeviceGetAttribute(&h->c.sm_count, cudaDevAttrMultiProcessorCount, device);
  *out = h;
  return PNP_OK;
}
pnp_status pnp_ctx_create_child(pnp_ctx* parent, pnp_ctx** out) {
  if (!parent || !out) return PNP_E_ARG;
  pnp_ctx* h = new pnp_ctx;
  Ctx& p = parent->c;
  h->c.device = p.device; h->c.stream = p.stream; h->c.owns_stream = false; h->c.sm_count = p.sm_count;
  h->c.rank = p.rank; h->c.world = p.world; h->c.nccl = p.nccl;
  h->c.params = p.params;
  h->c.parent = &p; p.children.push_back(&h->c);
  *out = h;
  return PNP_OK;
}
void pnp_ctx_destroy(pnp_ctx* ctx) {
  if (!ctx) return;
  Ctx& c = ctx->c;
  cudaSetDevice(c.device);
  if (c.parent) {
    Ctx& p = *c.parent;
    for (size_t i = 0; i < p.children.size(); i++) if (p.children[i] == &c) { p.children.erase(p.children.begin() + i); break; }
    for (size_t i = 0; i < p.mg.size(); i++) if (p.mg[i].lc == &c) { p.mg.resize(i); p.mg_gid.release(); p.mg_nglobal = 0; p.mg_replica = nullptr; break; }
    if (p.mg_replica == &c) { p.mg_replica = nullptr; p.mg_gid.release(); p.mg_nglobal = 0; }
    p.mg_epoch++;
  }
  if (c.stream) cudaStreamSynchronize(c.stream);
  c.solvers.clear();
  {
    std::vector<void*> owned;
    owned.swap(c.owned_children);
    for (void* h : owned) pnp_ctx_destroy((pnp_ctx*)h);
  }
  for (Ctx* k : c.children) { k->solvers.clear(); k->parent = nullptr; k->stream = nullptr; k->nccl = nullptr; }
  if (c.h_red) cudaFreeHost(c.h_red);
  for (cudaEvent_t e : c.prof_ev) cudaEventDestroy(e);
  if (c.tm0) cudaEventDestroy(c.tm0);
  if (c.tm1) cudaEventDestroy(c.tm1);
  if (c.owns_comm) comm_destroy(c);
  cudaStream_t s = c.owns_stream ? c.stream : nullptr;
  delete ctx;
  if (s) cudaStreamDestroy(s);
}
pnp_status pnp_mg_push_level(pnp_ctx* ctx, pnp_ctx* child, const int* par0, const int* par1) {
  API_BEGIN(ctx)
  PNP_REQUIRE(c.degree == 1, PNP_E_ARG, "built for linear elements only");
  PNP_REQUIRE(child && par0 && par1, PNP_E_ARG, "null arguments");
  Ctx& f = c.mg.empty() ? c : *c.mg.back().lc;
  Ctx& k = child->c;
  PNP_REQUIRE(f.finalized && k.finalized, PNP_E_ARG, "both levels must be finalized");
  std::vector<int> fi2e = f.int2ext.to_host(c.stream), ke2i = k.ext2int.to_host(c.stream);
  std::vector<int> p0(f.nv), p1(f.nv);
  for (long i = 0; i < f.nv; i++) {
    const int e = fi2e[i];
    PNP_REQUIRE(par0[e] < k.nv && par1[e] < k.nv, PNP_E_ARG, "parent index out of range");
    p0[i] = par0[e] >= 0 ? ke2i[par0[e]] : -1;
    p1[i] = par1[e] >= 0 ? ke2i[par1[e]] : -1;
  }
  MgLevelRef r; r.lc = &k;
  r.par0.alloc(f.nv); r.par1.alloc(f.nv);
  r.par0.upload(p0.data(), f.nv, c.stream); r.par1.upload(p1.data(), f.nv, c.stream);
  PNP_CUDA(cudaStreamSynchronize(c.stream));
  c.mg.push_back(std::move(r));
  c.mg_epoch++;
  API_END
}
pnp_status pnp_mg_set_coarse_aggregates(pnp_ctx* ctx, const int* agg, long n_aggregates) {
  const pnp_status st = pnp_mg_set_coarse_global(ctx, agg, n_aggregates);
  if (st == PNP_OK) ctx->c.mg_aggregated = true;
  return st;
}
pnp_status pnp_mg_set_coarse_global(pnp_ctx* ctx, const int* gid, long n_global) {
  API_BEGIN(ctx)
  c.mg_aggregated = false; c.mg_replica = nullptr;
  PNP_REQUIRE(!c.mg.empty() && gid && n_global > 0, PNP_E_ARG, "no multigrid level pushed");
  Ctx& k = *c.mg.back().lc;
  std::vector<int> i2e = k.int2ext.to_host(c.stream), g(k.nv);
  for (long i = 0; i < k.nv; i++) { g[i] = gid[i2e[i]]; PNP_REQUIRE(g[i] >= 0 && g[i] < n_global, PNP_E_ARG, "global index out of range"); }
  c.mg_gid.alloc(k.nv); c.mg_gid.upload(g.data(), k.nv, c.stream);
  PNP_CUDA(cudaStreamSynchronize(c.stream));
  c.mg_nglobal = n_global; c.mg_epoch++;
  API_END
}
pnp_status pnp_mg_set_coarse_replica(pnp_ctx* ctx, pnp_ctx* replica, const int* gid, long n_global) {
  API_BEGIN(ctx)
  c.mg_aggregated = false; c.mg_replica = nullptr;
  PNP_REQUIRE(!c.mg.empty() && gid && n_global > 0 && replica, PNP_E_ARG, "no multigrid level pushed / null arguments");
  Ctx& k = *c.mg.back().lc;
  Ctx& r = replica->c;
  PNP_REQUIRE(r.finalized && r.n_own == r.nv && r.nv == n_global, PNP_E_ARG, "the replica must hold the whole coarsest mesh, finalized");
  std::vector<int> i2e = k.int2ext.to_host(c.stream), re2i = r.ext2int.to_host(c.stream), g(k.nv);
  for (long i = 0; i < k.nv; i++) {
    const int gi = gid[i2e[i]];
    PNP_REQUIRE(gi >= 0 && gi < n_global, PNP_E_ARG, "global index out of range");
    g[i] = re2i[gi];
  }
  c.mg_gid.alloc(k.nv); c.mg_gid.upload(g.data(), k.nv, c.stream);
  PNP_CUDA(cudaStreamSynchronize(c.stream));
  c.mg_nglobal = n_global; c.mg_replica = &r; c.mg_epoch++;
  API_END
}
pnp_status pnp_profile_spmv(pnp_ctx* ctx, int enable) {
  API_BEGIN(ctx) c.prof = enable != 0; c.prof_used = 0; API_END
}
pnp_status pnp_profile_spmv_get(pnp_ctx* ctx, long* launches, double* total_ms) {
  API_BEGIN(ctx)
  PNP_CUDA(cudaStreamSynchronize(c.stream));
  for (int k = 0; k < 3; k++) { if (launches) launches[k] = 0; if (total_ms) total_ms[k] = 0; }
  for (size_t i = 0; i + 1 < c.prof_used; i += 2) {
    float t = 0; PNP_CUDA(cudaEventElapsedTime(&t, c.prof_ev[i], c.prof_ev[i + 1]));
    const int k = c.prof_kind[i / 2];
    if (launches) launches[k]++;
    if (total_ms) total_ms[k] += t;
  }
  API_END
}
pnp_status pnp_profile_bytes(pnp_ctx* ctx, int reset, double* out6) {
  API_BEGIN(ctx)
  for (int k = 0; k < Ctx::ACC_N; k++) { if (out6) out6[k] = c.alg_bytes[k]; if (reset) c.alg_bytes[k] = 0; }
  API_END
}
pnp_status pnp_profiler_range(pnp_ctx* ctx, int start) {
  API_BEGIN(ctx)
  PNP_CUDA(cudaStreamSynchronize(c.stream));
  if (start) cudaProfilerStart(); else cudaProfilerStop();
  API_END
}
pnp_status pnp_timer_start(pnp_ctx* ctx) {
  API_BEGIN(ctx)
  if (!c.tm0) { PNP_CUDA(cudaEventCreate(&c.tm0)); PNP_CUDA(cudaEventCreate(&c.tm1)); }
  PNP_CUDA(cudaEventRecord(c.tm0, c.stream));
  API_END
}
pnp_status pnp_timer_stop(pnp_ctx* ctx, double* ms) {
  API_BEGIN(ctx)
  PNP_REQUIRE(c.tm0 && ms, PNP_E_ARG, "timer not started");
  PNP_CUDA(cudaEventRecord(c.tm1, c.stream));
  PNP_CUDA(cudaEventSynchronize(c.tm1));
  float t = 0; PNP_CUDA(cudaEventElapsedTime(&t, c.tm0, c.tm1));
  *ms = t;
  API_END
}
pnp_status pnp_tune(const char* name, double value) {
  if (!name) return PNP_E_ARG;
  const std::string n(name);
  Tune& t = tune();
  if (n == "tma") t.tma = value != 0;
  else if (n == "tma_stages") t.tma_stages = (int)value;
  else if (n == "tma_lpr") t.tma_lpr = (int)value;
  else if (n == "graph") t.graph = value != 0;
  else if (n == "fd_warp") t.fd_warp = value != 0;
  else if (n == "jac_compact") t.jac_compact = value != 0;
  else if (n == "p2_chunk") t.p2_chunk = (long)value;
  else if (n == "tma_min_rows") t.tma_min_rows = (long)value;
  else return PNP_E_ARG;
  return PNP_OK;
}
const char* pnp_last_error(pnp_ctx* ctx) { return ctx ? ctx->c.err.c_str() : "null context"; }
long pnp_launch_count(pnp_ctx* ctx) { return ctx ? ctx->c.launches : 0; }

pnp_status pnp_mesh_set(pnp_ctx* ctx, long nv, const double* x, const double* y, long nT, const int* tri, long nB,
                        const int* ba, const int* bb, const int* bphys) {
  API_BEGIN(ctx) mesh_set(c, nv, x, y, nT, tri, nB, ba, bb, bphys, nv); API_END
}
pnp_status pnp_mesh_set_local(pnp_ctx* ctx, long nv, long n_own, const double* x, const double* y, long nT, const int* tri,
                              long nB, const int* ba, const int* bb, const int* bphys) {
  API_BEGIN(ctx) mesh_set(c, nv, x, y, nT, tri, nB, ba, bb, bphys, n_own); API_END
}
pnp_status pnp_comm_unique_id(char* out128) {
  try { comm_unique_id(out128); return PNP_OK; } catch (...) { return PNP_E_CUDA; }
}
pnp_status pnp_comm_init(pnp_ctx* ctx, int rank, int world, const char* unique_id128) {
  API_BEGIN(ctx) comm_init(c, rank, world, unique_id128); API_END
}
pnp_status pnp_comm_init_file(pnp_ctx* ctx, int rank, int world, const char* path) {
  API_BEGIN(ctx)
  PNP_REQUIRE(world == 1 || path, PNP_E_ARG, "null rendezvous path");
  comm_bootstrap_file(c, rank, world, path ? path : "");
  API_END
}
pnp_status pnp_comm_allgatherv(pnp_ctx* ctx, const void* send, long nbytes, void* recv, long cap, long* counts) {
  API_BEGIN(ctx)
  PNP_REQUIRE(nbytes >= 0 && counts && (nbytes == 0 || send), PNP_E_ARG, "bad all-gather arguments");
  std::vector<long> cnt;
  std::vector<unsigned char> all = comm_allgatherv(c, send, nbytes, cnt);
  for (int r = 0; r < c.world; r++) counts[r] = cnt[r];
  if (recv) {
    PNP_REQUIRE((long)all.size() <= cap, PNP_E_ARG, "receive buffer too small");
    std::memcpy(recv, all.data(), all.size());
  }
  API_END
}
pnp_status pnp_halo_set(pnp_ctx* ctx, int n_nbr, const int* nbr, const int* send_ptr, const int* send_idx, const int* recv_ptr) {
  API_BEGIN(ctx) halo_set(c, n_nbr, nbr, send_ptr, send_idx, recv_ptr); API_END
}
pnp_status pnp_halo_exchange(pnp_ctx* ctx, int vec_handle) {
  API_BEGIN(ctx)
  PNP_REQUIRE(c.degree == 1, PNP_E_ARG, "built for linear elements only");
  halo_exchange(c, c.vec(vec_handle).d.p, c.vec(vec_handle).fields);
  PNP_CUDA(cudaStreamSynchronize(c.stream));
  API_END
}
pnp_status pnp_mesh_read_gmsh(pnp_ctx* ctx, const char* path) {
  API_BEGIN(ctx)
  std::vector<double> x, y; std::vector<int> tri, ba, bb, ph;
  read_gmsh_file(path, x, y, tri, ba, bb, ph);
  mesh_set(c, (long)x.size(), x.data(), y.data(), (long)tri.size() / 3, tri.data(), (long)ba.size(), ba.data(), bb.data(),
           ph.data(), (long)x.size());
  API_END
}
pnp_status pnp_mesh_refine(pnp_ctx* ctx, int levels) { API_BEGIN(ctx) mesh_refine(c, levels); API_END }
pnp_status pnp_carry_set(pnp_ctx* ctx, const int* vec_handles, int n) { API_BEGIN(ctx) PNP_REQUIRE(c.degree == 1, PNP_E_ARG, "built for linear elements only"); carry_set(c, vec_handles, n); API_END }
pnp_status pnp_carry_get(pnp_ctx* ctx, int index, int vec_handle) { API_BEGIN(ctx) PNP_REQUIRE(c.degree == 1, PNP_E_ARG, "built for linear elements only"); carry_get(c, index, c.vec(vec_handle)); API_END }
pnp_status pnp_carry_set_host(pnp_ctx* ctx, int fields, const double* host) {
  API_BEGIN(ctx)
  PNP_REQUIRE(c.degree == 1, PNP_E_ARG, "built for linear elements only");
  PNP_REQUIRE(c.nv > 0 && fields >= 1 && host, PNP_E_ARG, "no mesh / bad field count");
  Vec cf; cf.fields = fields; cf.d.alloc((size_t)fields * c.nv);
  cf.d.upload(host, (size_t)fields * c.nv, c.stream);
  PNP_CUDA(cudaStreamSynchronize(c.stream));
  c.carry.clear();
  c.carry.push_back(std::move(cf));
  API_END
}
pnp_status pnp_carry_get_host(pnp_ctx* ctx, int index, double* host) {
  API_BEGIN(ctx)
  PNP_REQUIRE(c.degree == 1, PNP_E_ARG, "built for linear elements only");
  PNP_REQUIRE(index >= 0 && index < (int)c.carry.size() && host, PNP_E_ARG, "no such carried field");
  c.carry[index].d.download(host, c.carry[index].d.n, c.stream);
  API_END
}
pnp_status pnp_mesh_finalize(pnp_ctx* ctx, int renumber) { API_BEGIN(ctx) mesh_finalize(c, renumber != 0); API_END }
pnp_status pnp_mesh_sizes(pnp_ctx* ctx, long* nv, long* nT, long* nB, long* nslots) {
  API_BEGIN(ctx)
  if (nv) *nv = c.nv;
  if (nT) *nT = c.nT; if (nB) *nB = c.nB; if (nslots) *nslots = c.finalized ? c.nslots : 0;
  API_END
}
pnp_status pnp_mesh_get(pnp_ctx* ctx, double* x, double* y, int* tri, int* ba, int* bb, int* bphys) {
  API_BEGIN(ctx)
  if (x) c.cx.download(x, c.nv, c.stream);
  if (y) c.cy.download(y, c.nv, c.stream);
  if (tri) c.ctri.download(tri, 3 * c.nT, c.stream);
  if (ba) c.cba.download(ba, c.nB, c.stream);
  if (bb) c.cbb.download(bb, c.nB, c.stream);
  if (bphys) c.cbphys.download(bphys, c.nB, c.stream);
  API_END
}

pnp_status pnp_params_set(pnp_ctx* ctx, const double* sys, const double* surf) {
  API_BEGIN(ctx)
  PNP_REQUIRE(sys && (sys[0] == 0 || surf), PNP_E_ARG, "null parameter arrays");
  HostParams p;
  p.n_surfaces = (int)sys[0]; p.cylindrical = sys[1] != 0; p.l_b = sys[2]; p.c0 = sys[3]; p.PI = sys[4];
  p.linearSolverIterations = (int)sys[5]; p.newtonReassembleThreshold = sys[6]; p.newtonReduction = sys[7];
  p.newtonMinLinearReduction = sys[8]; p.newtonMaxIterations = sys[9]; p.newtonLineSearchMaxIteration = sys[10];
  p.tau = sys[11]; p.nSteps = (int)sys[12]; p.outputFreq = (int)sys[13]; p.potentialUpdateFreq = (int)sys[14];
  p.verbosity = (int)sys[15];
  PNP_REQUIRE(p.n_surfaces >= 0, PNP_E_CONFIG, "n_surfaces must be non-negative");
  p.surfaces.assign(p.n_surfaces, HostSurface());
  for (int i = 0; i < p.n_surfaces; i++)
    for (int k = 0; k < 3; k++) {
      p.surfaces[i].btype[k] = (int)surf[9 * i + 3 * k];
      p.surfaces[i].flux[k] = surf[9 * i + 3 * k + 1];
      p.surfaces[i].dval[k] = surf[9 * i + 3 * k + 2];
    }
  p.set = true;
  c.params = p;
  c.constraints_built = false;
  if (c.finalized) constraints_build(c);
  API_END
}
pnp_status pnp_params_read(pnp_ctx* ctx, const char* cfg_path) {
  API_BEGIN(ctx)
  read_config_file(cfg_path, c.params);
  c.constraints_built = false;
  if (c.finalized) constraints_build(c);
  API_END
}
pnp_status pnp_params_get(pnp_ctx* ctx, double* sys, double* surf, char* meshfile, int meshfile_cap) {
  API_BEGIN(ctx)
  PNP_REQUIRE(c.params.set, PNP_E_ARG, "parameters not set");
  const HostParams& p = c.params;
  const double v[16] = {(double)p.n_surfaces, (double)p.cylindrical, p.l_b, p.c0, p.PI, (double)p.linearSolverIterations,
                        p.newtonReassembleThreshold, p.newtonReduction, p.newtonMinLinearReduction, p.newtonMaxIterations,
                        p.newtonLineSearchMaxIteration, p.tau, (double)p.nSteps, (double)p.outputFreq,
                        (double)p.potentialUpdateFreq, (double)p.verbosity};
  if (sys) std::memcpy(sys, v, sizeof v);
  if (surf)
    for (int i = 0; i < p.n_surfaces; i++)
      for (int k = 0; k < 3; k++) {
        surf[9 * i + 3 * k] = p.surfaces[i].btype[k];
        surf[9 * i + 3 * k + 1] = p.surfaces[i].flux[k];
        surf[9 * i + 3 * k + 2] = p.surfaces[i].dval[k];
      }
  if (meshfile && meshfile_cap > 0) { std::strncpy(meshfile, p.meshfile.c_str(), meshfile_cap - 1); meshfile[meshfile_cap - 1] = 0; }
  API_END
}
pnp_status pnp_constraints_build(pnp_ctx* ctx) { API_BEGIN(ctx) constraints_build(c); API_END }

pnp_status pnp_operator_create(pnp_ctx* ctx, int op, int comp0, int* handle) {
  API_BEGIN(ctx)
  PNP_REQUIRE(op >= PNP_OP_PB && op <= PNP_OP_PNP && comp0 >= 0 && comp0 < 3 && handle, PNP_E_ARG, "bad operator arguments");
  auto o = std::make_unique<Operator>();
  o->op = op; o->comp0 = comp0;
  c.ops.push_back(std::move(o));
  *handle = (int)c.ops.size() - 1;
// ... 10 lines not shown
pnp_status pnp_constraints_get(pnp_ctx* ctx, int h, char* out) {
  API_BEGIN(ctx)
  PNP_REQUIRE(c.constraints_built, PNP_E_ARG, "constraints not built");
  const Operator& op = c.oper(h);
  if (c.degree >= 2) { p2_constraints_get(c, op, out); return PNP_OK; }
  const int F = op_fields(op.op);
  std::vector<unsigned char> m = c.dmask.to_host(c.stream);
  std::vector<int> i2e = c.int2ext.to_host(c.stream);
  for (long v = 0; v < c.nv; v++)
    for (int k = 0; k < F; k++) out[(long)k * c.nv + i2e[v]] = (char)((m[v] >> (F == 3 ? k : op.comp0)) & 1);
  API_END
}
pnp_status pnp_pattern_get(pnp_ctx* ctx, int h, long* nnz, int* rowptr, int* col) {
  API_BEGIN(ctx)
  long n = pattern_export(c, h, rowptr, col);
  if (nnz) *nnz = n;
  API_END
}

pnp_status pnp_vec_create(pnp_ctx* ctx, int fields, int* handle) {
  API_BEGIN(ctx)
  PNP_REQUIRE(c.finalized, PNP_E_ARG, "mesh not finalized");
  PNP_REQUIRE((fields == 1 || fields == 3) && handle, PNP_E_ARG, "fields must be 1 or 3");
  auto v = std::make_unique<Vec>();
  v->fields = fields; v->d.alloc((size_t)fields * c.cols()); v->d.zero(c.stream);
  c.vecs.push_back(std::move(v));
  *handle = (int)c.vecs.size() - 1;
  API_END
}
pnp_status pnp_vec_destroy(pnp_ctx* ctx, int h) {
  API_BEGIN(ctx)
  if (c.vec(h).d.p == c.last_u) { c.last_u = nullptr; c.last_vals = nullptr; }
  c.vecs[h].reset();
  API_END
}
pnp_status pnp_vec_upload(pnp_ctx* ctx, int h, const double* host) { API_BEGIN(ctx) vec_upload(c, c.vec(h), host); API_END }
pnp_status pnp_vec_download(pnp_ctx* ctx, int h, double* host) { API_BEGIN(ctx) vec_download(c, c.vec(h), host); API_END }
pnp_status pnp_vec_set(pnp_ctx* ctx, int h, double value) {
  API_BEGIN(ctx)
  Vec& v = c.vec(h);
  k_fill<<<grid_for((long)v.d.n, 256), 256, 0, c.stream>>>(v.d.p, (long)v.d.n, value);
  PNP_CHECK_LAUNCH(); c.launches++;
  API_END
}
pnp_status pnp_vec_copy(pnp_ctx* ctx, int dst, int src) {
  API_BEGIN(ctx)
  PNP_REQUIRE(c.vec(dst).d.n == c.vec(src).d.n, PNP_E_ARG, "vector sizes differ");
  vec_copy(c, c.vec(src).d.p, c.vec(dst).d.p, (long)c.vec(src).d.n);
  API_END
}
pnp_status pnp_vec_axpy(pnp_ctx* ctx, int y, double a, int x) {
  API_BEGIN(ctx)
  PNP_REQUIRE(c.vec(y).d.n == c.vec(x).d.n, PNP_E_ARG, "vector sizes differ");
  vec_axpy(c, a, c.vec(x).d.p, c.vec(y).d.p, (long)c.vec(x).d.n);
  API_END
}
pnp_status pnp_vec_norm(pnp_ctx* ctx, int x, double* out) {
  API_BEGIN(ctx) *out = vec_norm(c, c.vec(x).d.p, c.rows() * c.vec(x).fields); API_END
}
pnp_status pnp_vec_dot(pnp_ctx* ctx, int x, int y, double* out) {
  API_BEGIN(ctx)
  PNP_REQUIRE(c.vec(y).d.n == c.vec(x).d.n, PNP_E_ARG, "vector sizes differ");
  *out = vec_dot(c, c.vec(x).d.p, c.vec(y).d.p, c.rows() * c.vec(x).fields);
  API_END
}
pnp_status pnp_vec_pack3(pnp_ctx* ctx, int dst3, int phi, int cp, int cm) {
  API_BEGIN(ctx)
  PNP_REQUIRE(c.vec(dst3).fields == 3 && c.vec(phi).fields == 1 && c.vec(cp).fields == 1 && c.vec(cm).fields == 1,
              PNP_E_ARG, "pack3 needs one 3-field and three 1-field vectors");
  if (c.degree >= 2) {
    const int src[3] = {phi, cp, cm};
    for (int k = 0; k < 3; k++) vec_copy(c, c.vec(src[k]).d.p, c.vec(dst3).d.p + k * c.p2_nd, c.p2_nd);
    return PNP_OK;
  }
  k_pack3<<<grid_for(c.nv, 256), 256, 0, c.stream>>>(c.vec(phi).d.p, c.vec(cp).d.p, c.vec(cm).d.p, c.nv, c.vec(dst3).d.p);
  PNP_CHECK_LAUNCH(); c.launches++;
  API_END
}
pnp_status pnp_vec_extract(pnp_ctx* ctx, int src3, int field, int dst1) {
  API_BEGIN(ctx)
  PNP_REQUIRE(c.vec(src3).fields == 3 && c.vec(dst1).fields == 1 && field >= 0 && field < 3, PNP_E_ARG, "bad extract arguments");
  if (c.degree >= 2) { vec_copy(c, c.vec(src3).d.p + field * c.p2_nd, c.vec(dst1).d.p, c.p2_nd); return PNP_OK; }
  k_extract<<<grid_for(c.nv, 256), 256, 0, c.stream>>>(c.vec(src3).d.p, c.nv, field, c.vec(dst1).d.p);
  PNP_CHECK_LAUNCH(); c.launches++;
  API_END
}

pnp_status pnp_matrix_create(pnp_ctx* ctx, int op_handle, int* handle) {
  API_BEGIN(ctx)
  PNP_REQUIRE(c.finalized && handle, PNP_E_ARG, "mesh not finalized");
  auto m = std::make_unique<Matrix>();
  m->op = c.oper(op_handle).op; m->nplanes = op_planes(m->op);
  if (c.degree >= 2) { PNP_REQUIRE(c.constraints_built, PNP_E_ARG, "constraints not built"); p2_matrix_init(c, *m, c.oper(op_handle)); }
  else { m->vals.alloc((size_t)m->nplanes * c.nslots); m->vals.zero(c.stream); }
  c.mats.push_back(std::move(m));
  *handle = (int)c.mats.size() - 1;
  API_END
}
pnp_status pnp_matrix_destroy(pnp_ctx* ctx, int h) {
  API_BEGIN(ctx)
  if (c.mat(h).vals.p == c.last_vals) c.last_vals = nullptr;
  c.mats[h].reset();
  API_END
}
pnp_status pnp_residual(pnp_ctx* ctx, int op, int u, int r) {
  API_BEGIN(ctx)
  assemble_residual(c, c.oper(op), c.vec(u), c.vec(r));
  PNP_CUDA(cudaStreamSynchronize(c.stream));
  API_END
}
pnp_status pnp_jacobian(pnp_ctx* ctx, int op, int u, int A, int mode, double eps) {
  API_BEGIN(ctx)
  assemble_jacobian(c, c.oper(op), c.vec(u), c.mat(A), mode, eps);
  PNP_CUDA(cudaStreamSynchronize(c.stream));
  API_END
}
pnp_status pnp_matrix_values_get(pnp_ctx* ctx, int op, int A, double* val) {
  API_BEGIN(ctx) matrix_export(c, op, c.mat(A), val); API_END
}
pnp_status pnp_spmv(pnp_ctx* ctx, int A, int x, int y) {
  API_BEGIN(ctx)
  const Matrix& M = c.mat(A);
  PNP_REQUIRE(c.vec(x).fields == (M.nplanes == 1 ? 1 : 3) && c.vec(y).fields == c.vec(x).fields && x != y, PNP_E_ARG,
              "spmv operands do not match the matrix");
  spmv(c, M, c.vec(x).d.p, c.vec(y).d.p);
  PNP_CUDA(cudaStreamSynchronize(c.stream));
  API_END
}

pnp_status pnp_solver_create(pnp_ctx* ctx, int kind, int prec, int maxit, int prec_steps, int verbosity, int* handle) {
  API_BEGIN(ctx)
  PNP_REQUIRE((kind == PNP_SOLVER_BCGS || kind == PNP_SOLVER_CG) && prec >= PNP_PREC_NONE && prec <= PNP_PREC_AMG && handle,
              PNP_E_ARG, "bad solver arguments");
  auto s = std::make_unique<Solver>();
  s->kind = kind; s->prec = prec; s->maxit = maxit; s->prec_steps = prec_steps; s->verbosity = verbosity;
  c.solvers.push_back(std::move(s));
  *handle = (int)c.solvers.size() - 1;
  API_END
}
pnp_status pnp_solver_set_option(pnp_ctx* ctx, int s, const char* name, double value) {
  API_BEGIN(ctx)
  PNP_REQUIRE(name, PNP_E_ARG, "null option name");
  c.solver(s).opts[name] = value;
  API_END
}
pnp_status pnp_solver_get(pnp_ctx* ctx, int s, const char* name, double* value) {
  API_BEGIN(ctx)
  PNP_REQUIRE(name && value, PNP_E_ARG, "null argument");
  const std::string n(name);
  if (c.degree >= 2 && (n == "ssor_levels" || n == "ilu0_levels")) *value = c.solver(s).csr_levels;
  else if (n == "ssor_levels") *value = sweep_levels(c.solver(s), false);
  else if (n == "ilu0_levels") *value = sweep_levels(c.solver(s), true);
  else if (n == "amg_graph") *value = amg_graph_state(c.solver(s));
  else PNP_REQUIRE(false, PNP_E_ARG, "unknown solver fact");
  API_END
}
pnp_status pnp_precond_apply(pnp_ctx* ctx, int s, int A, int d, int v) {
  API_BEGIN(ctx)
  precond_apply(c, c.solver(s), c.mat(A), c.vec(d), c.vec(v));
  PNP_CUDA(cudaStreamSynchronize(c.stream));
  API_END
}
pnp_status pnp_solver_apply(pnp_ctx* ctx, int s, int A, int z, int r, double reduction, pnp_lin_result* out) {
  API_BEGIN(ctx)
  LinResult lr = solver_apply(c, c.solver(s), c.mat(A), c.vec(z), c.vec(r), reduction);
  to_lin(lr, out);
  if (lr.status == PNP_E_BREAKDOWN) { c.err = "BiCGSTAB breakdown (rho, omega or h vanished)"; return PNP_E_BREAKDOWN; }
  if (lr.status == PNP_E_NAN) { c.err = "non-finite residual norm in the linear solver"; return PNP_E_NAN; }
  API_END
}

void pnp_newton_opts_default(pnp_newton_opts* o) {
  if (!o) return;
  o->reduction = 1e-8; o->abs_limit = 1e-12; o->min_linear_reduction = 1e-3; o->reassemble_threshold = 0.0;
  o->max_iterations = 40; o->line_search_max_iterations = 10; o->damping = 0.5;
  o->jac_mode = PNP_JAC_FD_FAITHFUL; o->fd_epsilon = 1e-11; o->verbosity = 0;
  o->line_search_strategy = PNP_LS_HACKBUSCH_REUSKEN_ACCEPT_BEST;
}
pnp_status pnp_newton_opts_from_params(pnp_ctx* ctx, pnp_newton_opts* o) {
  API_BEGIN(ctx)
  PNP_REQUIRE(c.params.set && o, PNP_E_ARG, "parameters not set");
  pnp_newton_opts_default(o);
  o->reassemble_threshold = c.params.newtonReassembleThreshold;
  o->reduction = c.params.newtonReduction;
  o->min_linear_reduction = c.params.newtonMinLinearReduction;
  o->max_iterations = (int)c.params.newtonMaxIterations;
  o->line_search_max_iterations = (int)c.params.newtonLineSearchMaxIteration;
  o->verbosity = c.params.verbosity;
  API_END
}
pnp_status pnp_newton_apply(pnp_ctx* ctx, int op, int u, int solver, const pnp_newton_opts* o, pnp_newton_result* res) {
  API_BEGIN(ctx)
  PNP_REQUIRE(o && res, PNP_E_ARG, "null options/result");
  int st = newton_apply(c, c.oper(op), c.vec(u), c.solver(solver), *o, *res);
  if (st != PNP_OK) {
    static const char* msg[] = {"", "Newton did not converge within max_iterations", "linear solver did not converge",
                                "line search failed", "defect is not finite", "BiCGSTAB breakdown"};
    c.err = msg[st <= 5 ? st : 0];
    return st;
  }
  API_END
}
pnp_status pnp_slp_apply(pnp_ctx* ctx, int op, int u, int solver, double reduction, int jac_mode, double eps,
                         pnp_lin_result* out) {
  API_BEGIN(ctx)
  LinResult lr = slp_apply(c, c.oper(op), c.vec(u), c.solver(solver), reduction, jac_mode, eps);
  to_lin(lr, out);
  if (lr.status == PNP_E_BREAKDOWN) { c.err = "BiCGSTAB breakdown (rho, omega or h vanished)"; return PNP_E_BREAKDOWN; }
  if (lr.status == PNP_E_NAN) { c.err = "non-finite residual norm in the linear solver"; return PNP_E_NAN; }
  API_END
}
pnp_status pnp_onestep_apply(pnp_ctx* ctx, int method, int op_space, int op_time, int solver, double time, double dt,
                             int x_old, int dirichlet_values, int x_new, double reduction, int jac_mode, double eps,
                             pnp_lin_result* stage_results) {
  API_BEGIN(ctx)
  (void)time;
  LinResult lr[2];
  const int st = onestep_apply(c, method, c.oper(op_space), c.oper(op_time), c.solver(solver), dt, c.vec(x_old),
                               c.vec(dirichlet_values), c.vec(x_new), reduction, jac_mode, eps, lr);
  if (stage_results) for (int k = 0; k < (method == PNP_TIME_IMPLICIT_EULER ? 1 : 2); k++) to_lin(lr[k], stage_results + k);
  if (st == PNP_E_BREAKDOWN) { c.err = "BiCGSTAB breakdown in a stage solve"; return PNP_E_BREAKDOWN; }
  if (st == PNP_E_NAN) { c.err = "non-finite residual norm in a stage solve"; return PNP_E_NAN; }
  API_END
}
pnp_status pnp_ion_flux(pnp_ctx* ctx, int phi, int cp, int cm, double* ip, double* im) {
  API_BEGIN(ctx)
  PNP_REQUIRE(ip && im, PNP_E_ARG, "null output");
  ion_flux(c, c.vec(phi), c.vec(cp), c.vec(cm), ip, im);
  API_END
}
pnp_status pnp_write_cell_data(pnp_ctx* ctx, int v, const char* filename) {
  API_BEGIN(ctx)
  PNP_REQUIRE(filename, PNP_E_ARG, "null file name");
  write_cell_data(c, c.vec(v), filename);
  API_END
}
pnp_status pnp_write_vtk(pnp_ctx* ctx, const char* name, int n, const int* vec_handles, const char* const* names, int ascii) {
  API_BEGIN(ctx)
  PNP_REQUIRE(name && n >= 0 && (n == 0 || (vec_handles && names)), PNP_E_ARG, "null arguments");
  std::vector<const Vec*> f(n);
  for (int i = 0; i < n; i++) f[i] = &c.vec(vec_handles[i]);
  write_vtk(c, name, n, f.data(), names, ascii);
  API_END
}
pnp_status pnp_matrix_set_csr(pnp_ctx* ctx, int op_handle, int mat_handle, const int* rowptr, const int* col, const double* val) {
  API_BEGIN(ctx) matrix_import(c, op_handle, c.mat(mat_handle), rowptr, col, val); API_END
}
pnp_status pnp_mesh_renumber(pnp_ctx* ctx, const int* new_index) { API_BEGIN(ctx) mesh_renumber(c, new_index); API_END }
pnp_status pnp_mesh_owned(pnp_ctx* ctx, long* n_own) { API_BEGIN(ctx) if (n_own) *n_own = c.n_own; API_END }
pnp_status pnp_interpolate_bcext(pnp_ctx* ctx, int component, int pb_vec, int out_vec) {
  API_BEGIN(ctx)
  PNP_REQUIRE(c.n_own == c.nv, PNP_E_ARG, "interpolate(BCExtension) follows the global element order: run it before partitioning");
  if (c.degree >= 2) p2_interpolate_bcext(c, component, pb_vec >= 0 ? &c.vec(pb_vec) : nullptr, c.vec(out_vec));
  else interpolate_bcext(c, component, pb_vec >= 0 ? &c.vec(pb_vec) : nullptr, c.vec(out_vec));
  API_END
}
pnp_status pnp_space_set_degree(pnp_ctx* ctx, int degree) {
  API_BEGIN(ctx)
  PNP_REQUIRE(degree >= 1 && degree <= 3, PNP_E_ARG, "polynomial degree must be 1, 2 or 3");
  PNP_REQUIRE(!c.finalized, PNP_E_ARG, "set the degree before pnp_mesh_finalize");
  PNP_REQUIRE(degree == 1 || (c.world == 1 && !c.parent), PNP_E_ARG, "quadratic and cubic elements run on one GPU");
  c.degree = degree;
  API_END
}
pnp_status pnp_space_sizes(pnp_ctx* ctx, int* degree, long* n_edges, long* ndof) {
  API_BEGIN(ctx)
  PNP_REQUIRE(c.finalized, PNP_E_ARG, "mesh not finalized");
  if (degree) *degree = c.degree;
  if (c.degree >= 2) p2_sizes(c, n_edges, ndof);
  else { if (n_edges) *n_edges = 0; if (ndof) *ndof = c.nv; }
  API_END
}
pnp_status pnp_space_edges(pnp_ctx* ctx, int* va, int* vb) { API_BEGIN(ctx) p2_edges(c, va, vb); API_END }
pnp_status pnp_space_offsets(pnp_ctx* ctx, long* edge_offset, long* vertex_offset) {
  API_BEGIN(ctx)
  PNP_REQUIRE(c.finalized, PNP_E_ARG, "mesh not finalized");
  if (c.degree >= 2) p2_offsets(c, edge_offset, vertex_offset);
  else { if (edge_offset) *edge_offset = 0; if (vertex_offset) *vertex_offset = 0; }
  API_END
}
pnp_status pnp_operator_set_intorder(pnp_ctx* ctx, int h, int intorder) {
  API_BEGIN(ctx)
  PNP_REQUIRE(intorder == 0 || (intorder == 5 && c.degree >= 2), PNP_E_ARG,
              "quadrature order: 0 (the order the reference's drivers end up with) or, for degree 2 and 3, 5");
  c.oper(h).intorder = intorder;
  API_END
}

}
```

### dune_pnp_b200/csrc/pnp_common.cuh

```cuda
#pragma once
#include <cuda_runtime.h>

#include <cstdint>
#include <cstdio>
#include <map>
#include <memory>
#include <stdexcept>
#include <string>
#include <vector>

#include "../../include/pnp_b200.h"
#include "pnp_setup_algos.cuh"
#include "pnp_star.cuh"

namespace pnp {

struct Error : std::runtime_error {
  int code;
  Error(int c, const std::string& m) : std::runtime_error(m), code(c) {}
};

#define PNP_CUDA(call)                                                                               \
  do {                                                                                               \
    cudaError_t e_ = (call);                                                                         \
    if (e_ != cudaSuccess)                                                                           \
      throw ::pnp::Error(PNP_E_CUDA, std::string(__FILE__) + ":" + std::to_string(__LINE__) + " " +  \
                                         #call + " -> " + cudaGetErrorString(e_));                   \
  } while (0)
#define PNP_CHECK_LAUNCH() PNP_CUDA(cudaGetLastError())
#define PNP_REQUIRE(cond, code, msg)                                                                 \
  do { if (!(cond)) throw ::pnp::Error(code, std::string(msg)); } while (0)

template <class T> struct DBuf {
  T* p = nullptr;
  size_t n = 0;
  DBuf() = default;
  explicit DBuf(size_t n_) { alloc(n_); }
  DBuf(const DBuf&) = delete;
  DBuf& operator=(const DBuf&) = delete;
  DBuf(DBuf&& o) noexcept : p(o.p), n(o.n) { o.p = nullptr; o.n = 0; }
  DBuf& operator=(DBuf&& o) noexcept { if (this != &o) { release(); p = o.p; n = o.n; o.p = nullptr; o.n = 0; } return *this; }
  ~DBuf() { release(); }
  void release() { if (p) cudaFree(p); p = nullptr; n = 0; }
  void alloc(size_t n_) {
    release();
    n = n_;
    if (n) PNP_CUDA(cudaMalloc(&p, n * sizeof(T) + 64));
  }
  void zero(cudaStream_t s) { if (n) PNP_CUDA(cudaMemsetAsync(p, 0, n * sizeof(T), s)); }
  void upload(const T* h, size_t cnt, cudaStream_t s) {
    if (cnt) PNP_CUDA(cudaMemcpyAsync(p, h, cnt * sizeof(T), cudaMemcpyHostToDevice, s));
  }
  void download(T* h, size_t cnt, cudaStream_t s) const {
    if (cnt) PNP_CUDA(cudaMemcpyAsync(h, p, cnt * sizeof(T), cudaMemcpyDeviceToHost, s));
    PNP_CUDA(cudaStreamSynchronize(s));
  }
  std::vector<T> to_host(cudaStream_t s) const { std::vector<T> h(n); download(h.data(), n, s); return h; }
};

struct Tune {
  int tma = 1;
  int tma_stages = 2;
  int tma_lpr = 2;
  long tma_min_rows = -1;
  int graph = 1;
  int fd_warp = 1;
  int jac_compact = 1;
  long p2_chunk = 0;
};
inline Tune& tune() { static Tune t; return t; }

inline int grid_for(long n, int block, int max_blocks = 148 * 32) {
  long g = (n + block - 1) / block;
  if (g < 1) g = 1;
  return (int)(g > max_blocks ? max_blocks : g);
}

struct HostSurface { int btype[3] = {1, 1, 1}; double flux[3] = {0, 0, 0}; double dval[3] = {0, 0, 0}; };
struct HostParams {
  bool set = false;
  int n_surfaces = 0, verbosity = 0, cylindrical = 0;
  double l_b = 1, c0 = 0.06, PI = 3.1415;
  int linearSolverIterations = 50;
  double newtonReassembleThreshold = 0, newtonReduction = 1e-5, newtonMinLinearReduction = 1e-5;
  double newtonMaxIterations = 50, newtonLineSearchMaxIteration = 500, tau = 0.1;
  int nSteps = 100, outputFreq = 1, potentialUpdateFreq = 1;
  std::string meshfile;
  std::vector<HostSurface> surfaces;
};

struct Vec {
  int fields = 1;
  DBuf<double> d;
};
struct Matrix {
  int op = 0;
  int nplanes = 1;
  int comp0 = 0;
  DBuf<double> vals;
  const int* csr_rp = nullptr; const int* csr_col = nullptr; long csr_nnz = 0, csr_n = 0;
  void* csr_pattern = nullptr;
};

struct Operator {
  int op = OP_PB;
  int comp0 = 0;
  double valency = 1.0;
  int aux0 = -1, aux1 = -1;
  int intorder = 0;
};

struct HierLevel {
  long nv = 0, nslots = 0, nE = 0;
  DBuf<int> rp, int2ext, ext2int;
  DBuf<unsigned> adj;
  DBuf<uint64_t> edges;
};

struct Ctx;
struct MgLevelRef {
  Ctx* lc = nullptr;
  DBuf<int> par0, par1;
};

struct Amg;
struct P2Space;
struct SweepPrec;
struct SweepPlan;

struct Solver {
  int kind = PNP_SOLVER_BCGS, prec = PNP_PREC_NONE, maxit = 5000, prec_steps = 1, verbosity = 0;
  std::shared_ptr<Amg> amg;
  std::shared_ptr<SweepPrec> sweep;
  std::map<std::string, double> opts;
  double opt(const char* name, double dflt) const { auto it = opts.find(name); return it == opts.end() ? dflt : it->second; }
  DBuf<double> w[6];
  DBuf<double> dinv;
  DBuf<double> csr_lu; int csr_levels = 0;
  std::shared_ptr<void> pmg;
  void ensure(size_t n) { for (auto& b : w) if (b.n != n) b.alloc(n); if (dinv.n != n) dinv.alloc(n); }
};

struct Ctx {
  int device = 0;
  cudaStream_t stream = nullptr;
  std::string err;
  int sm_count = 148;
  long nv = 0, nT = 0, nB = 0;
  long n_own = 0;
  int degree = 1; long p2_nd = 0;
  std::shared_ptr<P2Space> p2;
  long rows() const { return degree >= 2 ? p2_nd : n_own; }
  long cols() const { return degree >= 2 ? p2_nd : nv; }
  int rank = 0, world = 1;
  void* nccl = nullptr;
  std::vector<int> halo_nbr, halo_send_ptr, halo_recv_ptr;
  std::vector<int> halo_send_ext;
  DBuf<int> halo_send_idx;
  DBuf<double> halo_send_buf;
  DBuf<double> cx, cy;
  DBuf<int> ctri, cba, cbb, cbphys;
  bool finalized = false;
  long nslots = 0;
  DBuf<int> rp;
  DBuf<unsigned> adj;
  DBuf<XY> xy;
  DBuf<unsigned char> dmask;
  DBuf<int> int2ext, ext2int;
  std::vector<BFace> bfaces;
  DBuf<BFace> d_bfaces;
  DBuf<int> d_bv, d_bv_ptr, d_bv_items;
  int n_bv = 0;
  DBuf<double> d_surf;
  DBuf<unsigned char> d_surf_dir;
  HostParams params;
  bool constraints_built = false;
  long launches = 0;
  enum { ACC_SPMV_FINE = 0, ACC_SPMV_COARSE = 1, ACC_ASSEMBLY = 2, ACC_BLAS1 = 3, ACC_TRANSFER = 4, ACC_DENSE = 5, ACC_N = 6 };
  double alg_bytes[ACC_N] = {0, 0, 0, 0, 0, 0};
  void acct(int cls, double bytes) { alg_bytes[cls] += bytes; }
  void absorb(Ctx& child) {
    launches += child.launches; child.launches = 0;
    for (int k = 0; k < ACC_N; k++) { alg_bytes[k] += child.alg_bytes[k]; child.alg_bytes[k] = 0; }
  }
  bool prof = false;
  std::vector<cudaEvent_t> prof_ev;
  std::vector<int> prof_kind;
  size_t prof_used = 0;
  cudaEvent_t tm0 = nullptr, tm1 = nullptr;
  void prof_mark(int kind = 0) {
    if (!prof) return;
    if (prof_used == prof_ev.size()) { cudaEvent_t e; cudaEventCreate(&e); prof_ev.push_back(e); }
    if (prof_used % 2 == 0) { if (prof_kind.size() <= prof_used / 2) prof_kind.resize(prof_used / 2 + 1); prof_kind[prof_used / 2] = kind; }
    cudaEventRecord(prof_ev[prof_used++], stream);
  }
  std::vector<std::unique_ptr<Vec>> vecs;
  std::vector<std::unique_ptr<Matrix>> mats;
  std::vector<std::unique_ptr<Operator>> ops;
  std::vector<std::unique_ptr<Solver>> solvers;
  Vec ws_r, ws_z, ws_prev;
  Matrix ws_A;
  Vec ws_stage[6];
  Matrix ws_B;
  DBuf<double> io_stage;
  bool owns_stream = true;
  std::vector<MgLevelRef> mg;
  DBuf<int> mg_gid; long mg_nglobal = 0; bool mg_aggregated = false;
  Ctx* mg_replica = nullptr;
  long mg_epoch = 0;
  Ctx* parent = nullptr;
  std::vector<Ctx*> children;
  std::vector<void*> owned_children;
  bool owns_comm = false;
  const double* last_u = nullptr; Operator last_op; int last_mode = 0; double last_eps = 1e-11;
  const double* last_vals = nullptr;
  std::vector<HierLevel> hier;
  std::vector<Vec> carry;
  void invalidate_mesh_objects() {
    finalized = false; constraints_built = false; p2.reset(); p2_nd = 0;
    vecs.clear(); mats.clear(); ops.clear(); solvers.clear();
    last_u = nullptr; last_vals = nullptr;
    ws_r.d.release(); ws_z.d.release(); ws_prev.d.release(); ws_A.vals.release(); ws_B.vals.release();
    for (auto& v : ws_stage) v.d.release();
    io_stage.release();
  }
  DBuf<double> red_partial, red_out;
  double* h_red = nullptr;

  StarView star() const { return StarView{rp.p, adj.p, xy.p, dmask.p, (int)n_own}; }
  PhysParams phys(double valency) const {
    PhysParams P; P.PI = params.PI; P.l_b = params.l_b; P.c0 = params.c0; P.valency = valency;
    P.cylindrical = params.cylindrical; return P;
  }
  Vec& vec(int h) { PNP_REQUIRE(h >= 0 && h < (int)vecs.size() && vecs[h], PNP_E_ARG, "bad vector handle"); return *vecs[h]; }
  Matrix& mat(int h) { PNP_REQUIRE(h >= 0 && h < (int)mats.size() && mats[h], PNP_E_ARG, "bad matrix handle"); return *mats[h]; }
  Operator& oper(int h) { PNP_REQUIRE(h >= 0 && h < (int)ops.size() && ops[h], PNP_E_ARG, "bad operator handle"); return *ops[h]; }
  Solver& solver(int h) { PNP_REQUIRE(h >= 0 && h < (int)solvers.size() && solvers[h], PNP_E_ARG, "bad solver handle"); return *solvers[h]; }
};

inline int op_fields(int op) { return op == OP_PNP ? 3 : 1; }
inline int op_planes(int op) { return op == OP_PNP ? 7 : 1; }

void mesh_set(Ctx&, long nv, const double* x, const double* y, long nT, const int* tri, long nB, const int* ba,
              const int* bb, const int* bphys, long n_own);
void mesh_refine(Ctx&, int levels);
void mesh_finalize(Ctx&, bool renumber);
void constraints_build(Ctx&);
void comm_init(Ctx&, int rank, int world, const char* unique_id128);
void comm_unique_id(char* out128);
void comm_destroy(Ctx&);
void comm_bootstrap_file(Ctx&, int rank, int world, const std::string& path);
std::vector<unsigned char> comm_allgatherv(Ctx&, const void* send, long nbytes, std::vector<long>& counts);
void halo_set(Ctx&, int n_nbr, const int* nbr, const int* send_ptr, const int* send_idx, const int* recv_ptr);
void halo_finalize(Ctx&);
void halo_exchange(Ctx&, double* x, int fields);
void allreduce_sum(Ctx&, double* dev, size_t n);
void allreduce_max_u64(Ctx&, unsigned long long* dev, size_t n);
void carry_set(Ctx&, const int* handles, int n);
void carry_get(Ctx&, int i, Vec& out);
void vec_upload(Ctx&, Vec&, const double* host_lex);
void vec_download(Ctx&, const Vec&, double* host_lex);
void vec_from_lex_device(Ctx&, Vec&, const double* d_lex);
void vec_to_lex_device(Ctx&, const Vec&, double* d_lex);
Ctx* ctx_make_owned_child(Ctx& parent);
void ctx_destroy_owned_child(Ctx& parent, Ctx* child);
long pattern_export(Ctx&, int op_handle, int* rowptr, int* col);
void matrix_export(Ctx&, int op_handle, const Matrix&, double* val);
void matrix_import(Ctx&, int op_handle, Matrix&, const int* rowptr, const int* col, const double* val);
void mesh_renumber(Ctx&, const int* new_index);
void read_gmsh_file(const std::string& path, std::vector<double>& x, std::vector<double>& y, std::vector<int>& tri,
                    std::vector<int>& ba, std::vector<int>& bb, std::vector<int>& bphys);
void read_config_file(const std::string& path, HostParams& p);
void interpolate_bcext(Ctx&, int comp, const Vec* pb, Vec& out);
void assemble_residual(Ctx&, const Operator&, Vec& u, Vec& r);
void assemble_jacobian(Ctx&, const Operator&, Vec& u, Matrix& A, int mode, double eps);
void assemble_jacobian_on(Ctx&, const StarView& M, long stride, const Operator&, const double* u, double* vals, int nplanes,
                          int mode, double eps);
void spmv(Ctx&, const Matrix& A, double* x, double* y);
double vec_norm(Ctx&, const double* x, long n);
double vec_dot(Ctx&, const double* x, const double* y, long n);
void vec_axpy(Ctx&, double a, const double* x, double* y, long n);
void vec_copy(Ctx&, const double* x, double* y, long n);
void vec_zero(Ctx&, double* x, long n);
struct LinResult { bool converged = false; int iterations = 0; double reduction = 1, conv_rate = 1; int status = 0; double seconds = 0; };
LinResult solver_apply(Ctx&, Solver&, const Matrix& A, Vec& z, Vec& r, double reduction);
void precond_apply(Ctx&, Solver&, const Matrix& A, Vec& d, Vec& v);
int sweep_levels(const Solver&, bool ilu);
void p2_build(Ctx&);
void p2_constraints(Ctx&);
void p2_matrix_init(Ctx&, Matrix&, const Operator&);
void p2_assemble_residual(Ctx&, const Operator&, Vec& u, Vec& r);
void p2_assemble_jacobian(Ctx&, const Operator&, Vec& u, Matrix& A, int mode, double eps);
void csr_spmv(Ctx&, const Matrix& A, const double* x, double* y);
void csr_diag_inverse(Ctx&, const Matrix& A, double* dinv);
void csr_sweep_setup(Ctx&, Solver&, const Matrix& A, bool ilu);
void csr_ssor_apply(Ctx&, Solver&, const Matrix& A, const double* d, double* y);
void csr_ilu0_apply(Ctx&, Solver&, const Matrix& A, const double* d, double* y);
void pmg_setup(Ctx&, Solver&, const Matrix& A);
void pmg_apply(Ctx&, Solver&, const Matrix& A, const double* d, double* y);
const unsigned char* p2_dirichlet_flags(Ctx&);
void p2_sizes(Ctx&, long* nE, long* nd);
void p2_offsets(Ctx&, long* eoff, long* voff);
void p2_edges(Ctx&, int* eva, int* evb);
void p2_constraints_get(Ctx&, const Operator&, char* out);
long p2_pattern_export(Ctx&, const Operator&, int* rowptr, int* col);
void p2_matrix_import(Ctx&, const Operator&, Matrix&, const int* rowptr, const int* col, const double* val);
void p2_interpolate_bcext(Ctx&, int comp, const Vec* pb, Vec& out);
void p2_ion_flux(Ctx&, const Vec& phi, const Vec& cp, const Vec& cm, double* ip, double* im);
void p2_write_cell_data(Ctx&, const Vec& u, const std::string& filename);
void p2_vertex_values(Ctx&, const Vec& u, double* out);
void ion_flux(Ctx&, const Vec& phi, const Vec& cp, const Vec& cm, double* ip, double* im);
void write_cell_data(Ctx&, const Vec& u, const std::string& filename);
void write_vtk(Ctx&, const std::string& name, int nfields, const Vec* const* fields, const char* const* names, int ascii);

}

struct pnp_ctx { pnp::Ctx c; };
```

### dune_pnp_b200/csrc/pnp_spmv_tma.cuh

```cuda
#pragma once
#include "pnp_spmv.cuh"

namespace pnp {

constexpr int TMA_TR = 128;
constexpr int tma_nw(int lpr) { return TMA_TR * lpr / 32; }
constexpr int tma_producers(int np, int epi, int ndot) { return np + 3 + ((epi != EPI_PLAIN || ndot >= 1) ? 1 : 0); }
constexpr int tma_threads(int np, int epi, int ndot, int lpr) { return (tma_nw(lpr) + tma_producers(np, epi, ndot)) * 32; }
constexpr int TMA_CAP = 960;
constexpr int TMA_MAX_STAGES = 3;
constexpr int TMA_W = 128;

template <int NP> struct TmaLayout {
  static constexpr int F = NP == 1 ? 1 : 3;
  static constexpr int PLANE = (TMA_CAP + 2) * 8;
  static constexpr int COLS = NP * PLANE;
  static constexpr int RP = COLS + (TMA_CAP + 4) * 4;
  static constexpr int B = RP + (TMA_TR + 4) * 4;
  static constexpr int XW = B + (F * TMA_TR + 2) * 8;
  static constexpr int STAGE = XW + (F * (TMA_TR + 2 * TMA_W) + 2) * 8;
  static constexpr int YBUF = TMA_TR * F * 8;
  static constexpr int HEAD = 128;
  static_assert(PLANE % 16 == 0 && COLS % 16 == 0 && RP % 16 == 0 && B % 16 == 0 && XW % 16 == 0 && STAGE % 16 == 0, "bulk copy alignment");
  static constexpr int smem_bytes(int stages) { return HEAD + stages * STAGE + YBUF; }
};

__device__ __forceinline__ unsigned smem_u32(const void* p) { return (unsigned)__cvta_generic_to_shared(p); }
__device__ __forceinline__ void mbar_init(uint64_t* bar, unsigned count) {
  asm volatile("mbarrier.init.shared::cta.b64 [%0], %1;" ::"r"(smem_u32(bar)), "r"(count) : "memory");
}
__device__ __forceinline__ void mbar_expect_tx(uint64_t* bar, unsigned bytes) {
  asm volatile("mbarrier.arrive.expect_tx.shared::cta.b64 _, [%0], %1;" ::"r"(smem_u32(bar)), "r"(bytes) : "memory");
}
__device__ __forceinline__ void mbar_arrive(uint64_t* bar) {
  asm volatile("mbarrier.arrive.shared::cta.b64 _, [%0];" ::"r"(smem_u32(bar)) : "memory");
}
__device__ __forceinline__ void mbar_wait(uint64_t* bar, unsigned parity) {
  unsigned done;
  do {
    asm volatile("{\n .reg .pred p;\n mbarrier.try_wait.parity.shared::cta.b64 p, [%1], %2;\n selp.u32 %0, 1, 0, p;\n}"
                 : "=r"(done) : "r"(smem_u32(bar)), "r"(parity) : "memory");
  } while (!done);
}
__device__ __forceinline__ void bulk_g2s(void* dst, const void* src, unsigned bytes, uint64_t* bar) {
  asm volatile("cp.async.bulk.shared::cluster.global.mbarrier::complete_tx::bytes [%0], [%1], %2, [%3];"
               ::"r"(smem_u32(dst)), "l"(src), "r"(bytes), "r"(smem_u32(bar)) : "memory");
}

template <int NP>
__device__ __forceinline__ void block_inverse_row(const double* dv, int k, double* o) {
  const PnpBlock B = pnp_block<NP>(dv);
  const double a = B.a, b = B.b, c_ = B.c, d = B.d, e = B.e, f = B.f, g = B.g;
  const double det = a * e * g - b * d * g - c_ * e * f;
  const double scale = fabs(a * e * g) + fabs(b * d * g) + fabs(c_ * e * f);
  if (fabs(det) > 1e-12 * scale && scale > 0.0) {
    const double id = 1.0 / det;
    if (k == 0) { o[0] = e * g * id; o[1] = -b * g * id; o[2] = -c_ * e * id; }
    else if (k == 1) { o[0] = -d * g * id; o[1] = (a * g - c_ * f) * id; o[2] = c_ * d * id; }
    else { o[0] = -e * f * id; o[1] = b * f * id; o[2] = (a * e - b * d) * id; }
  } else {
    const double dd = k == 0 ? a : (k == 1 ? e : g);
    const double inv = dd != 0.0 ? 1.0 / dd : 0.0;
    o[0] = k == 0 ? inv : 0.0; o[1] = k == 1 ? inv : 0.0; o[2] = k == 2 ? inv : 0.0;
  }
}

template <int NP, bool STAGED>
__device__ __forceinline__ void slot_product(const StarOpArgs& a, bool ok, int s, const double* sv, const int* vb, const unsigned* sc,
                                             int cbase, const double* sx, int wlo, unsigned wn, double* acc, double* dg) {
  constexpr int F = NP == 1 ? 1 : 3;
  const unsigned c = !ok ? 0u : ((STAGED ? sc[s - cbase] : a.col[s]) & STAR_VMASK);
  const unsigned cw = c - (unsigned)wlo;
  const bool in = cw < wn;
  double x[F], v[NP];
#pragma unroll
  for (int k = 0; k < F; k++) x[k] = !ok ? 0.0 : (in ? sx[F * cw + k] : a.x[(size_t)F * c + k]);
#pragma unroll
  for (int p = 0; p < NP; p++) v[p] = !ok ? 0.0 : (STAGED ? sv[vb[p] + s] : a.vals[(size_t)p * a.stride + s]);
  if (dg) {
#pragma unroll
    for (int p = 0; p < NP; p++) dg[p] = v[p];
  }
  if constexpr (NP == 1) acc[0] += v[0] * x[0];
  else block_mac<NP>(v, x, acc);
}

template <int NP, int EPI, int NDOT, int LPR>
__global__ void __launch_bounds__(tma_threads(NP, EPI, NDOT, LPR), 1) k_star_op_tma(const StarOpArgs a, const int nstages) {
  using L = TmaLayout<NP>;
  constexpr int F = L::F;
  constexpr int TMA_NW = tma_nw(LPR);
  constexpr int RW = 32 / LPR;
  extern __shared__ __align__(128) unsigned char smem[];
  uint64_t* full = reinterpret_cast<uint64_t*>(smem);
  uint64_t* empty = full + TMA_MAX_STAGES;
  unsigned char* stages = smem + L::HEAD;
  double* ybuf = reinterpret_cast<double*>(stages + (size_t)nstages * L::STAGE);
  const int warp = threadIdx.x >> 5, lane = threadIdx.x & 31;
  const int ntiles = (a.nv + TMA_TR - 1) / TMA_TR;
  const int sp = (int)(a.stride & 1);
  if (threadIdx.x == 0) {
    for (int s = 0; s < nstages; s++) { mbar_init(&full[s], tma_producers(NP, EPI, NDOT)); mbar_init(&empty[s], TMA_NW); }
    asm volatile("fence.mbarrier_init.release.cluster;" ::: "memory");
  }
  __syncthreads();
  double dsum[NDOT > 0 ? NDOT : 1];
#pragma unroll
  for (int j = 0; j < (NDOT > 0 ? NDOT : 1); j++) dsum[j] = 0.0;

  if (warp >= TMA_NW) {
    const int role = warp - TMA_NW;
    auto load_batch = [&](int batch, int& lo, int& hi) {
      const long tt = blockIdx.x + (long)(batch * 32 + lane) * gridDim.x;
      lo = 0; hi = 0;
      if (tt < ntiles) { lo = a.rp[tt * TMA_TR]; hi = a.rp[min((int)tt * TMA_TR + TMA_TR, a.nv)]; }
    };
    int cur_lo, cur_hi, nxt_lo, nxt_hi;
    load_batch(0, cur_lo, cur_hi);
    load_batch(1, nxt_lo, nxt_hi);
    int t = blockIdx.x;
    for (int it = 0; t < ntiles; t += gridDim.x, it++) {
      if (it > 0 && (it & 31) == 0) { cur_lo = nxt_lo; cur_hi = nxt_hi; load_batch(it / 32 + 1, nxt_lo, nxt_hi); }
      const int lo = __shfl_sync(0xffffffffu, cur_lo, it & 31), hi = __shfl_sync(0xffffffffu, cur_hi, it & 31);
      if (lane == 0) {
        const int stage = it % nstages;
        const unsigned parity = (unsigned)((it / nstages) & 1);
        mbar_wait(&empty[stage], parity ^ 1u);
        unsigned char* st = stages + (size_t)stage * L::STAGE;
        const int r0 = t * TMA_TR, rows = min(TMA_TR, a.nv - r0);
        const bool staged = hi - lo <= TMA_CAP;
        const void* src = nullptr; void* dst = nullptr; unsigned nb = 0;
        if (role < NP) {
          if (staged) {
            const int o = (lo + role * sp) & 1;
            nb = (unsigned)(((hi - lo + o) + 1) & ~1) * 8u;
            src = a.vals + (size_t)role * a.stride + (lo - o); dst = st + role * L::PLANE;
          }
        } else if (role == NP) {
          if (staged) {
            const int lo_c = lo & ~3;
            nb = (unsigned)(((hi - lo_c) + 3) & ~3) * 4u;
            src = a.col + lo_c; dst = st + L::COLS;
          }
        } else if (role == NP + 1) {
          nb = (unsigned)((rows + 1 + 3) & ~3) * 4u;
          src = a.rp + r0; dst = st + L::RP;
        } else if (role == NP + 2) {
          const int wlo = max(r0 - TMA_W, 0), whi = min(r0 + TMA_TR + TMA_W, a.nv);
          nb = (unsigned)((F * (whi - wlo) + 1) & ~1) * 8u;
          src = a.x + (size_t)F * wlo; dst = st + L::XW;
        } else {
          nb = (unsigned)((F * rows + 1) & ~1) * 8u;
          src = (EPI == EPI_PLAIN ? a.w1 : a.b) + (size_t)F * r0; dst = st + L::B;
        }
        if (nb) { mbar_expect_tx(&full[stage], nb); bulk_g2s(dst, src, nb, &full[stage]); }
        else mbar_arrive(&full[stage]);
      }
      __syncwarp();
    }
  } else {
    const int sub = lane % LPR;
    double* yw = ybuf + warp * RW * F;
    int t = blockIdx.x;
    for (int it = 0; t < ntiles; t += gridDim.x, it++) {
      const int stage = it % nstages;
      const unsigned parity = (unsigned)((it / nstages) & 1);
      mbar_wait(&full[stage], parity);
      const unsigned char* st = stages + (size_t)stage * L::STAGE;
      const double* sv = reinterpret_cast<const double*>(st);
      const unsigned* sc = reinterpret_cast<const unsigned*>(st + L::COLS);
      const int* srp = reinterpret_cast<const int*>(st + L::RP);
      const double* sb = reinterpret_cast<const double*>(st + L::B);
      const double* sx = reinterpret_cast<const double*>(st + L::XW);
      const int r0 = t * TMA_TR, rows = min(TMA_TR, a.nv - r0);
      const int wlo = max(r0 - TMA_W, 0);
      const unsigned wn = (unsigned)(min(r0 + TMA_TR + TMA_W, a.nv) - wlo);
      const double* sxo = sx + (size_t)F * (r0 - wlo);
      const int lo = srp[0], hi = srp[rows];
      const bool staged = hi - lo <= TMA_CAP;
      const int cbase = lo & ~3;
      int vb[NP];
#pragma unroll
      for (int p = 0; p < NP; p++) vb[p] = p * (TMA_CAP + 2) - lo + ((lo + p * sp) & 1);
      const int rl = RW * warp + lane / LPR;
      const bool valid = rl < rows;
      const int b0 = valid ? srp[rl] : hi, e0 = valid ? srp[rl + 1] : hi;
      double acc[F], dg[NP];
#pragma unroll
      for (int k = 0; k < F; k++) acc[k] = 0.0;
#pragma unroll
      for (int p = 0; p < NP; p++) dg[p] = 0.0;
      const int len = e0 - b0;
      const int maxlen = __reduce_max_sync(0xffffffffu, len);
      if (staged) {
        constexpr int MAXS = (8 + LPR - 1) / LPR;
        unsigned cj[MAXS];
        bool okj[MAXS];
        double xj[MAXS][F];
#pragma unroll
        for (int u = 0; u < MAXS; u++) {
          const int j = sub + u * LPR;
          okj[u] = j < len;
          cj[u] = okj[u] ? (sc[b0 + j - cbase] & STAR_VMASK) : 0u;
        }
#pragma unroll
        for (int u = 0; u < MAXS; u++) {
          const unsigned cw = cj[u] - (unsigned)wlo;
          const bool in = cw < wn;
          const bool ldg = okj[u] && !in, lds = okj[u] && in;
#pragma unroll
          for (int k = 0; k < F; k++) {
            double xg = 0.0, xs = 0.0;
            if (ldg) xg = a.x[(size_t)F * cj[u] + k];
            if (lds) xs = sx[F * cw + k];
            xj[u][k] = in ? xs : xg;
          }
        }
#pragma unroll
        for (int u = 0; u < MAXS; u++) {
          const int s = b0 + sub + u * LPR;
          double v[NP];
#pragma unroll
          for (int p = 0; p < NP; p++) v[p] = okj[u] ? sv[vb[p] + s] : 0.0;
          if (EPI == EPI_JACOBI && u == 0) {
#pragma unroll
            for (int p = 0; p < NP; p++) dg[p] = v[p];
          }
          if constexpr (NP == 1) acc[0] += v[0] * xj[u][0];
          else block_mac<NP>(v, xj[u], acc);
        }
        for (int j = sub + MAXS * LPR; j < maxlen; j += LPR)
          slot_product<NP, true>(a, j < len, b0 + j, sv, vb, sc, cbase, sx, wlo, wn, acc, nullptr);
      } else {
        slot_product<NP, false>(a, sub < len, b0 + sub, sv, vb, sc, cbase, sx, wlo, wn, acc, EPI == EPI_JACOBI ? dg : nullptr);
        for (int j = sub + LPR; j < maxlen; j += LPR)
          slot_product<NP, false>(a, j < len, b0 + j, sv, vb, sc, cbase, sx, wlo, wn, acc, nullptr);
      }
      if (LPR > 1) {
#pragma unroll
        for (int k = 0; k < F; k++)
#pragma unroll
          for (int o = LPR / 2; o > 0; o >>= 1) acc[k] += __shfl_xor_sync(0xffffffffu, acc[k], o);
      }
      const bool mine = valid && sub == 0;
      double yv[F];
#pragma unroll
      for (int k = 0; k < F; k++) yv[k] = 0.0;
      if (mine) {
        if (EPI == EPI_PLAIN) {
#pragma unroll
          for (int k = 0; k < F; k++) {
            yv[k] = acc[k];
            if (NDOT >= 1) dsum[0] += acc[k] * sb[F * rl + k];
            if (NDOT >= 2) dsum[NDOT >= 2 ? 1 : 0] += acc[k] * acc[k];
          }
        } else if (EPI == EPI_RESIDUAL) {
#pragma unroll
          for (int k = 0; k < F; k++) yv[k] = sb[F * rl + k] - acc[k];
        } else {
          double r[F], z[F];
#pragma unroll
          for (int k = 0; k < F; k++) r[k] = sb[F * rl + k] - acc[k];
          if constexpr (F == 3) {
#pragma unroll
            for (int k = 0; k < F; k++) {
              double o[3];
              block_inverse_row<NP>(dg, k, o);
              z[k] = o[0] * r[0] + o[1] * r[1] + o[2] * r[2];
            }
          } else z[0] = (dg[0] != 0.0 ? 1.0 / dg[0] : 0.0) * r[0];
#pragma unroll
          for (int k = 0; k < F; k++) yv[k] = sxo[F * rl + k] + a.omega * z[k];
        }
      }
      if (sub == 0) {
#pragma unroll
        for (int k = 0; k < F; k++) yw[F * (lane / LPR) + k] = yv[k];
      }
      __syncwarp();
      {
        const size_t g0 = (size_t)F * (r0 + RW * warp);
        const size_t gend = (size_t)F * a.nv;
#pragma unroll
        for (int i = lane; i < RW * F; i += 32)
          if (g0 + i < gend) a.y[g0 + i] = yw[i];
      }
      __syncwarp();
      if (lane == 0) mbar_arrive(&empty[stage]);
    }
  }
  if (NDOT > 0) {
    __shared__ double sm[NDOT > 0 ? NDOT : 1][TMA_NW];
#pragma unroll
    for (int j = 0; j < (NDOT > 0 ? NDOT : 1); j++) {
      double s = dsum[j];
#pragma unroll
      for (int o = 16; o > 0; o >>= 1) s += __shfl_xor_sync(0xffffffffu, s, o);
      if (lane == 0 && warp < TMA_NW) sm[j][warp] = s;
    }
    __syncthreads();
    if (warp == 0) {
#pragma unroll
      for (int j = 0; j < (NDOT > 0 ? NDOT : 1); j++) {
        double s = lane < TMA_NW ? sm[j][lane] : 0.0;
#pragma unroll
        for (int o = 16; o > 0; o >>= 1) s += __shfl_xor_sync(0xffffffffu, s, o);
        if (lane == 0) a.partial[(long)blockIdx.x * NDOT + j] = s;
      }
    }
  }
}

inline bool star_op_tma_ok(const Ctx& c, const StarOpArgs& a, int epi) {
  const Tune& t = tune();
  if (!t.tma || epi == EPI_CHEBYSHEV) return false;
  if ((long)a.nv < (t.tma_min_rows >= 0 ? t.tma_min_rows : 2l * TMA_TR * c.sm_count)) return false;
  auto al = [](const void* p) { return (reinterpret_cast<uintptr_t>(p) & 15u) == 0; };
  return al(a.rp) && al(a.col) && al(a.vals) && al(a.x) && (!a.b || al(a.b)) && (!a.w1 || al(a.w1));
}

inline int star_op_tma_stages() {
  const int v = tune().tma_stages;
  return v < 2 ? 2 : (v > TMA_MAX_STAGES ? TMA_MAX_STAGES : v);
}

template <int NP, int EPI, int NDOT, int LPR>
inline int launch_star_op_tma_lpr(Ctx& c, const StarOpArgs& a) {
  using L = TmaLayout<NP>;
  const int nstages = star_op_tma_stages();
  const int smem = L::smem_bytes(nstages);
  static unsigned long long configured = 0;
  if (!(configured >> (c.device & 63) & 1ull)) {
    PNP_CUDA(cudaFuncSetAttribute(k_star_op_tma<NP, EPI, NDOT, LPR>, cudaFuncAttributeMaxDynamicSharedMemorySize, L::smem_bytes(TMA_MAX_STAGES)));
    configured |= 1ull << (c.device & 63);
  }
  const int ntiles = (a.nv + TMA_TR - 1) / TMA_TR;
  const int grid = ntiles < c.sm_count ? ntiles : c.sm_count;
  k_star_op_tma<NP, EPI, NDOT, LPR><<<grid, tma_threads(NP, EPI, NDOT, LPR), smem, c.stream>>>(a, nstages);
  PNP_CHECK_LAUNCH(); c.launches++;
  return grid;
}
template <int NP, int EPI, int NDOT>
inline int launch_star_op_tma_inst(Ctx& c, const StarOpArgs& a) {
  return tune().tma_lpr == 2 ? launch_star_op_tma_lpr<NP, EPI, NDOT, 2>(c, a) : launch_star_op_tma_lpr<NP, EPI, NDOT, 1>(c, a);
}

template <int EPI, int NDOT>
inline double star_op_bytes(int nplanes, const StarOpArgs& a) {
  const double F = nplanes == 1 ? 1 : 3, nv = a.nv, ns = a.rp ? (double)a.stride : 0.0;
  double b = (8.0 * nplanes + 4.0) * ns + (4.0 + 16.0 * F) * nv;
  if (EPI != EPI_PLAIN) b += 8.0 * F * nv;
  if (EPI == EPI_PLAIN && NDOT >= 1) b += 8.0 * F * nv;
  if (EPI == EPI_CHEBYSHEV) b += 16.0 * F * nv;
  return b;
}
template <int EPI, int NDOT>
inline int launch_star_op_auto(Ctx& c, int nplanes, const StarOpArgs& a, bool fine = true) {
  c.acct(fine ? Ctx::ACC_SPMV_FINE : Ctx::ACC_SPMV_COARSE, star_op_bytes<EPI, NDOT>(nplanes, a));
  if (EPI != EPI_CHEBYSHEV && star_op_tma_ok(c, a, EPI)) {
    constexpr int E = EPI == EPI_CHEBYSHEV ? EPI_PLAIN : EPI;
    return nplanes == 1 ? launch_star_op_tma_inst<1, E, NDOT>(c, a)
         : nplanes == PNP_COMPACT_PLANES ? launch_star_op_tma_inst<PNP_COMPACT_PLANES, E, NDOT>(c, a)
                                         : launch_star_op_tma_inst<7, E, NDOT>(c, a);
  }
  return launch_star_op<EPI, NDOT>(c, nplanes, a);
}

}
```

### include/pnp_b200.h

```cpp
#ifndef PNP_B200_H
#define PNP_B200_H

#ifdef __cplusplus
extern "C" {
#endif

typedef struct pnp_ctx pnp_ctx;
typedef int pnp_status;

enum {
  PNP_OK = 0,
  PNP_E_NOT_CONVERGED = 1,
  PNP_E_LINEAR_SOLVER = 2,
  PNP_E_LINE_SEARCH = 3,
  PNP_E_NAN = 4,
  PNP_E_BREAKDOWN = 5,
  PNP_E_CUDA = 6,
  PNP_E_CONFIG = 7,
  PNP_E_ARG = 8,
  PNP_E_MESH = 9
};

enum { PNP_OP_PB = 0, PNP_OP_POISSON = 1, PNP_OP_DIFFUSION = 2, PNP_OP_MASS = 3, PNP_OP_PNP = 4 };
enum { PNP_JAC_FD_FAITHFUL = 0, PNP_JAC_ANALYTIC = 1 };
enum { PNP_SOLVER_BCGS = 0, PNP_SOLVER_CG = 1 };
enum { PNP_PREC_NONE = 0, PNP_PREC_JACOBI = 1, PNP_PREC_SSOR = 2, PNP_PREC_ILU0 = 3, PNP_PREC_AMG = 4 };

pnp_status pnp_ctx_create(int device, pnp_ctx** out);
void pnp_ctx_destroy(pnp_ctx* ctx);
const char* pnp_last_error(pnp_ctx* ctx);
pnp_status pnp_tune(const char* name, double value);
long pnp_launch_count(pnp_ctx* ctx);

pnp_status pnp_profile_spmv(pnp_ctx*, int enable);
pnp_status pnp_profile_spmv_get(pnp_ctx*, long* launches, double* total_ms);
pnp_status pnp_profile_bytes(pnp_ctx*, int reset, double* out6);
pnp_status pnp_profiler_range(pnp_ctx*, int start);
pnp_status pnp_timer_start(pnp_ctx*);
pnp_status pnp_timer_stop(pnp_ctx*, double* elapsed_ms);

pnp_status pnp_mesh_set(pnp_ctx*, long nv, const double* x, const double* y, long nT, const int* tri ,
                        long nB, const int* ba, const int* bb, const int* bphys);
pnp_status pnp_mesh_read_gmsh(pnp_ctx*, const char* path);
pnp_status pnp_mesh_set_local(pnp_ctx*, long nv, long n_own, const double* x, const double* y, long nT, const int* tri,
                              long nB, const int* ba, const int* bb, const int* bphys);
pnp_status pnp_mesh_owned(pnp_ctx*, long* n_own);
pnp_status pnp_comm_unique_id(char* out128);
pnp_status pnp_comm_init(pnp_ctx*, int rank, int world, const char* unique_id128);
pnp_status pnp_comm_init_file(pnp_ctx*, int rank, int world, const char* path);
pnp_status pnp_comm_allgatherv(pnp_ctx*, const void* send, long nbytes, void* recv, long cap, long* counts);
pnp_status pnp_halo_set(pnp_ctx*, int n_nbr, const int* nbr, const int* send_ptr, const int* send_idx, const int* recv_ptr);
pnp_status pnp_halo_exchange(pnp_ctx*, int vec_handle);
pnp_status pnp_ctx_create_child(pnp_ctx* parent, pnp_ctx** child);
pnp_status pnp_mg_push_level(pnp_ctx*, pnp_ctx* child, const int* par0, const int* par1);
pnp_status pnp_mg_set_coarse_global(pnp_ctx*, const int* global_vertex_index, long n_global);
pnp_status pnp_mg_set_coarse_aggregates(pnp_ctx*, const int* aggregate, long n_aggregates);
pnp_status pnp_mg_set_coarse_replica(pnp_ctx*, pnp_ctx* replica, const int* global_vertex_index, long n_global);
typedef struct pnp_part pnp_part;
pnp_status pnp_part_create(long nv, const double* x, const double* y, long nT, const int* tri, long nB, const int* ba,
                           const int* bb, const int* bphys, int world, int rank, int levels, pnp_part** out);
void pnp_part_destroy(pnp_part*);
const char* pnp_part_last_error(pnp_part*);
pnp_status pnp_part_ghost_keys(pnp_part*, int level, long* n, unsigned long long* keys );
pnp_status pnp_part_claim(pnp_part*, int level, const long* ghost_ptr , const unsigned long long* ghost_keys_all,
                          long* claim_ptr , long* claim_pos );
pnp_status pnp_part_finalize(pnp_part*, int level, const long* mine_ptr , const long* mine_pos);
pnp_status pnp_part_sizes(pnp_part*, int level, long* sizes);
pnp_status pnp_part_get(pnp_part*, int level, double* x, double* y, int* tri, int* ba, int* bb, int* bphys, int* nbr,
                        int* send_ptr, int* send_idx, int* recv_ptr, int* par0, int* par1, int* gid);
pnp_status pnp_partition_build(pnp_ctx* root, int levels, int replica_level, int field_level, int nfields, long nf,
                               const double* fx, const double* fy, const double* fields, int* start_vec);
pnp_status pnp_mesh_refine(pnp_ctx*, int levels);
pnp_status pnp_carry_set(pnp_ctx*, const int* vec_handles, int n);
pnp_status pnp_carry_get(pnp_ctx*, int index, int vec_handle);
pnp_status pnp_carry_set_host(pnp_ctx*, int fields, const double* host);
pnp_status pnp_carry_get_host(pnp_ctx*, int index, double* host);
pnp_status pnp_mesh_renumber(pnp_ctx*, const int* new_index);
pnp_status pnp_mesh_finalize(pnp_ctx*, int renumber);
pnp_status pnp_mesh_sizes(pnp_ctx*, long* nv, long* nT, long* nB, long* nslots);
pnp_status pnp_mesh_get(pnp_ctx*, double* x, double* y, int* tri, int* ba, int* bb, int* bphys);

pnp_status pnp_params_set(pnp_ctx*, const double* sys, const double* surf);
pnp_status pnp_params_read(pnp_ctx*, const char* cfg_path);
pnp_status pnp_params_get(pnp_ctx*, double* sys, double* surf , char* meshfile, int meshfile_cap);
pnp_status pnp_constraints_build(pnp_ctx*);

pnp_status pnp_operator_create(pnp_ctx*, int op, int comp0, int* op_handle);
pnp_status pnp_operator_set_coefficient(pnp_ctx*, int op_handle, int which, int vec_handle);
pnp_status pnp_operator_set_valency(pnp_ctx*, int op_handle, double valency);
pnp_status pnp_constraints_get(pnp_ctx*, int op_handle, char* is_dirichlet);
pnp_status pnp_pattern_get(pnp_ctx*, int op_handle, long* nnz, int* rowptr, int* col);

pnp_status pnp_vec_create(pnp_ctx*, int fields, int* vec_handle);
pnp_status pnp_vec_destroy(pnp_ctx*, int vec_handle);
pnp_status pnp_vec_upload(pnp_ctx*, int vec_handle, const double* host);
pnp_status pnp_vec_download(pnp_ctx*, int vec_handle, double* host);
pnp_status pnp_vec_set(pnp_ctx*, int vec_handle, double value);
pnp_status pnp_vec_copy(pnp_ctx*, int dst, int src);
pnp_status pnp_vec_axpy(pnp_ctx*, int y, double a, int x);
pnp_status pnp_vec_norm(pnp_ctx*, int x, double* two_norm);
pnp_status pnp_vec_dot(pnp_ctx*, int x, int y, double* result);

pnp_status pnp_matrix_create(pnp_ctx*, int op_handle, int* mat_handle);
pnp_status pnp_matrix_destroy(pnp_ctx*, int mat_handle);
pnp_status pnp_residual(pnp_ctx*, int op_handle, int u, int r);
pnp_status pnp_jacobian(pnp_ctx*, int op_handle, int u, int mat_handle, int mode, double fd_epsilon);
pnp_status pnp_matrix_values_get(pnp_ctx*, int op_handle, int mat_handle, double* val);
pnp_status pnp_spmv(pnp_ctx*, int mat_handle, int x, int y);
pnp_status pnp_matrix_set_csr(pnp_ctx*, int op_handle, int mat_handle, const int* rowptr, const int* col, const double* val);

typedef struct {
  int converged;
  int iterations;
  double reduction;
  double conv_rate;
  double seconds;
  int status;
} pnp_lin_result;
pnp_status pnp_solver_create(pnp_ctx*, int kind, int prec, int maxit, int prec_steps, int verbosity, int* solver);
pnp_status pnp_solver_set_option(pnp_ctx*, int solver, const char* name, double value);
pnp_status pnp_solver_get(pnp_ctx*, int solver, const char* name, double* value);
pnp_status pnp_precond_apply(pnp_ctx*, int solver, int mat_handle, int d, int v);
pnp_status pnp_solver_apply(pnp_ctx*, int solver, int mat_handle, int z, int r, double reduction, pnp_lin_result*);

enum { PNP_LS_HACKBUSCH_REUSKEN_ACCEPT_BEST = 0, PNP_LS_NONE = 1, PNP_LS_HACKBUSCH_REUSKEN = 2 };
typedef struct {
  double reduction;
  double abs_limit;
  double min_linear_reduction;
  double reassemble_threshold;
  int max_iterations;
  int line_search_max_iterations;
  double damping;
  int jac_mode;
  double fd_epsilon;
  int verbosity;
  int line_search_strategy;
} pnp_newton_opts;
typedef struct {
  int converged;
  int iterations;
  double first_defect, defect, reduction;
  int linear_iterations, line_search_trials, jacobian_assemblies, residual_assemblies;
  double seconds_assembly, seconds_solve, seconds_total;
  int n_history;
  double defect_history[64];
  int linear_iterations_history[64];
} pnp_newton_result;
void pnp_newton_opts_default(pnp_newton_opts*);
pnp_status pnp_newton_opts_from_params(pnp_ctx*, pnp_newton_opts*);
pnp_status pnp_newton_apply(pnp_ctx*, int op_handle, int u, int solver, const pnp_newton_opts*, pnp_newton_result*);
pnp_status pnp_slp_apply(pnp_ctx*, int op_handle, int u, int solver, double reduction, int jac_mode, double fd_epsilon,
                         pnp_lin_result*);

enum { PNP_TIME_ALEXANDER2 = 0, PNP_TIME_IMPLICIT_EULER = 1 };
pnp_status pnp_onestep_apply(pnp_ctx*, int method, int op_space, int op_time, int solver, double time, double dt, int x_old,
                             int dirichlet_values, int x_new, double reduction, int jac_mode, double fd_epsilon,
                             pnp_lin_result* stage_results);

pnp_status pnp_ion_flux(pnp_ctx*, int phi, int cp, int cm, double* ip, double* im);
pnp_status pnp_write_cell_data(pnp_ctx*, int vec_handle, const char* filename);

pnp_status pnp_write_vtk(pnp_ctx*, const char* name, int n, const int* vec_handles, const char* const* names, int ascii);

pnp_status pnp_interpolate_bcext(pnp_ctx*, int component, int pb_vec, int out_vec);

pnp_status pnp_space_set_degree(pnp_ctx*, int degree);
pnp_status pnp_space_sizes(pnp_ctx*, int* degree, long* n_edges, long* ndof);
pnp_status pnp_space_edges(pnp_ctx*, int* va , int* vb);
pnp_status pnp_space_offsets(pnp_ctx*, long* edge_offset, long* vertex_offset);
pnp_status pnp_operator_set_intorder(pnp_ctx*, int op_handle, int intorder);
pnp_status pnp_vec_pack3(pnp_ctx*, int dst3, int phi, int cp, int cm);
pnp_status pnp_vec_extract(pnp_ctx*, int src3, int field, int dst1);

#ifdef __cplusplus
}
#endif
#endif
```

Measured before the change: 441.4 million.

## Fuse paired Jacobi smoother sweeps into one persistent cooperative TMA kernel

Adds a cooperative persistent kernel that runs two consecutive Jacobi smoothing steps, or a step plus the residual, in a single launch. Tiles of the second sweep wait on per-block progress counters for their dependencies, and rows whose neighbours lie too far ahead are deferred to a final pass. The goal is to cut launch count and reuse the matrix stream across the fused pair at each multigrid level. The cost is new symbolic setup, inter-block spin synchronisation with a timeout fallback, and three-buffer pointer rotation, which makes the smoother schedule and CUDA graph keying more complex.

```diff
diff --git a/dune_pnp_b200/capi.py b/dune_pnp_b200/capi.py
--- a/dune_pnp_b200/capi.py
+++ b/dune_pnp_b200/capi.py
@@ -124,6 +124,11 @@
         self._ck(lib().pnp_profile_spmv_get(self._h, n, ms))
         return list(n), list(ms)
 
+    def profile_spmv_fused_get(self):
+        n = C.c_long(); ms = C.c_double()
+        self._ck(lib().pnp_profile_spmv_fused_get(self._h, C.byref(n), C.byref(ms)))
+        return n.value, ms.value
+
     def profile_bytes(self, reset=False):
         out = (C.c_double * 6)()
         self._ck(lib().pnp_profile_bytes(self._h, int(reset), out))
diff --git a/dune_pnp_b200/csrc/pnp_amg.cu b/dune_pnp_b200/csrc/pnp_amg.cu
--- a/dune_pnp_b200/csrc/pnp_amg.cu
+++ b/dune_pnp_b200/csrc/pnp_amg.cu
@@ -1,6 +1,8 @@
 #include <cub/cub.cuh>
 #include <cusolverDn.h>
-
+#include <thrust/iterator/counting_iterator.h>
+
+#include <array>
 #include <chrono>
 #include <cmath>
 #include <cstdlib>
@@ -36,6 +38,8 @@
   bool redisc = false;
   DBuf<XY> xy_own; DBuf<unsigned char> dmask_own;
   std::shared_ptr<SweepPlan> gs_plan;
+  DBuf<int2> fuse_dep; DBuf<int> fuse_rows; DBuf<unsigned long long> fuse_prog; DBuf<unsigned> fuse_gen;
+  int fuse_grid = 0, fuse_lag = 0, fuse_reach = 0, fuse_nrows = 0;
 };
 
 }
@@ -69,8 +73,9 @@
   cudaGraphExec_t cg_exec = nullptr;
   bool cg_failed = false;
   int cg_calls = 0;
-  double cg_key[8] = {0, 0, 0, 0, 0, 0, 0, 0};
-  std::vector<std::pair<double*, double*>> cg_before, cg_after;
+  double cg_key[9] = {0, 0, 0, 0, 0, 0, 0, 0, 0};
+  std::vector<std::array<double*, 3>> cg_before, cg_after;
+  DBuf<int> fuse_err;
   long cg_launches = 0; double cg_bytes[Ctx::ACC_N] = {0, 0, 0, 0, 0, 0};
   void cg_reset() { if (cg_exec) cudaGraphExecDestroy(cg_exec); cg_exec = nullptr; cg_calls = 0; }
   ~Amg() { if (cg_exec) cudaGraphExecDestroy(cg_exec); if (cus) cusolverDnDestroy(cus); }
@@ -451,6 +456,81 @@
   if (fine) c.prof_mark(EPI == EPI_RESIDUAL ? 1 : 2);
   launch_star_op_auto<EPI, 0>(c, A.NP, a, fine);
   if (fine) c.prof_mark();
+}
+
+__global__ void k_fuse_tiles(const int* __restrict__ rp, const unsigned* __restrict__ col, int nv, int reach,
+                             int2* __restrict__ dep, int* __restrict__ overfull) {
+  const int ntiles = (nv + TMA_TR - 1) / TMA_TR;
+  for (int t = blockIdx.x * blockDim.x + threadIdx.x; t < ntiles; t += gridDim.x * blockDim.x) {
+    int lo, hi;
+    const int nd = fuse_tile_deps(rp, col, nv, t, reach, &lo, &hi);
+    dep[t] = make_int2(lo, hi | (nd ? FUSE_HAS_DEFERRED : 0));
+    if (rp[min(t * TMA_TR + TMA_TR, nv)] - rp[t * TMA_TR] > TMA_CAP) atomicExch(overfull, 1);
+  }
+}
+__global__ void k_fuse_rows(const int* __restrict__ rp, const unsigned* __restrict__ col, int nv, int reach,
+                            unsigned char* __restrict__ flag) {
+  for (int r = blockIdx.x * blockDim.x + threadIdx.x; r < nv; r += gridDim.x * blockDim.x)
+    flag[r] = fuse_row_deferred(rp, col, r, r / TMA_TR + reach) ? 1 : 0;
+}
+
+void fuse_build(Ctx& c, Amg& A, Level& l) {
+  const int ntiles = (l.nv + TMA_TR - 1) / TMA_TR;
+  const long min_rows = tune().tma_min_rows >= 0 ? tune().tma_min_rows : 2l * TMA_TR * c.sm_count;
+  l.fuse_grid = 0;
+  if (!tune().tma || (long)l.nv < min_rows || ntiles < 2) return;
+  const int grid = ntiles < c.sm_count ? ntiles : c.sm_count, lag = tune().mg_fuse_lag;
+  const int reach = (lag > 1 ? lag - 1 : 1) * grid;
+  DBuf<int> overfull(1);
+  overfull.zero(c.stream);
+  l.fuse_dep.alloc(ntiles);
+  KL(c, k_fuse_tiles, ntiles, l.rp, l.col, l.nv, reach, l.fuse_dep.p, overfull.p);
+  DBuf<unsigned char> flag(l.nv);
+  DBuf<int> rows(l.nv), nsel(1);
+  KL(c, k_fuse_rows, l.nv, l.rp, l.col, l.nv, reach, flag.p);
+  size_t bytes = 0;
+  cub::DeviceSelect::Flagged(nullptr, bytes, thrust::counting_iterator<int>(0), flag.p, rows.p, nsel.p, l.nv, c.stream);
+  PNP_CUDA(cub::DeviceSelect::Flagged(A.temp(bytes), bytes, thrust::counting_iterator<int>(0), flag.p, rows.p, nsel.p, l.nv, c.stream));
+  int h[2] = {0, 0};
+  nsel.download(&h[0], 1, c.stream);
+  overfull.download(&h[1], 1, c.stream);
+  if (h[1]) return;
+  l.fuse_nrows = h[0];
+  l.fuse_rows.alloc(h[0] > 0 ? h[0] : 1);
+  if (h[0] > 0) PNP_CUDA(cudaMemcpyAsync(l.fuse_rows.p, rows.p, h[0] * sizeof(int), cudaMemcpyDeviceToDevice, c.stream));
+  l.fuse_prog.alloc(grid); l.fuse_prog.zero(c.stream);
+  l.fuse_gen.alloc(2); l.fuse_gen.zero(c.stream);
+  if (!A.fuse_err.n) { A.fuse_err.alloc(1); A.fuse_err.zero(c.stream); }
+  PNP_CUDA(cudaStreamSynchronize(c.stream));
+  l.fuse_grid = grid; l.fuse_lag = lag; l.fuse_reach = reach;
+}
+
+bool fuse_ok(const Ctx& c, const Amg& A, const Level& l) {
+  if (!tune().mg_fuse || c.mg_fuse_off || A.smoother != 0 || A.distributed || !l.fuse_grid) return false;
+  StarOpArgs a{l.rp, l.col, l.vals, l.nslots, l.nv, l.x.p, l.x2.p};
+  a.b = l.b.p;
+  auto al = [](const void* p) { return (reinterpret_cast<uintptr_t>(p) & 15u) == 0; };
+  return star_op_tma_ok(c, a, EPI_JACOBI) && al(l.x2.p) && al(l.r.p);
+}
+
+template <int EPI2>
+void level_pair(Ctx& c, Amg& A, Level& l) {
+  StarOpArgs a{l.rp, l.col, l.vals, l.nslots, l.nv, l.x.p, l.x2.p};
+  a.b = l.b.p; a.dinv = l.dinv.p; a.block = A.F == 3; a.omega = A.omega;
+  const FuseArgs f{l.r.p, l.fuse_dep.p, l.fuse_rows.p, l.fuse_nrows, l.fuse_prog.p, l.fuse_gen.p, A.fuse_err.p, l.fuse_lag, l.fuse_reach};
+  const bool fine = &l == A.L[0].get();
+  if (fine) c.prof_mark(3);
+  const bool ok = launch_star_op2_tma<EPI2>(c, A.NP, a, f, l.fuse_grid);
+  if (fine) c.prof_mark();
+  if (ok) {
+    const double F = A.F, ns = (double)l.nslots, slot = 8.0 * A.NP + 4.0;
+    const double bytes = slot * ns + 4.0 * l.nv + slot * ns * ((double)l.fuse_nrows / l.nv) + 32.0 * F * l.nv;
+    c.acct(fine ? Ctx::ACC_SPMV_FINE : Ctx::ACC_SPMV_COARSE, bytes);
+    return;
+  }
+  c.mg_fuse_off = true;
+  level_op<2>(c, A, l, l.x.p, l.b.p, l.x2.p);
+  level_op<EPI2>(c, A, l, l.x2.p, l.b.p, l.r.p);
 }
 
 bool coarsen(Ctx& c, Amg& A, int li) {
@@ -872,16 +952,36 @@
   c.acct(Ctx::ACC_TRANSFER, ((A.F == 3 ? 72.0 : 8.0) + 16.0 * A.F + (dvec ? 8.0 * A.F : 0.0)) * l.nv);
 }
 
-void smooth(Ctx& c, Amg& A, Level& l, int steps, bool zero) {
+enum JacobiOp { JOP_ZERO, JOP_STEP, JOP_PAIR, JOP_STEP_RESIDUAL, JOP_RESIDUAL };
+template <class Fn>
+void jacobi_schedule(int steps, bool zero, bool residual, bool paired, Fn&& op) {
+  int s = 0;
+  if (zero) { op(JOP_ZERO); s = 1; }
+  const bool pair_res = paired && residual && s < steps;
+  const int n = pair_res ? steps - 1 : steps;
+  if (paired)
+    for (; s + 2 <= n; s += 2) op(JOP_PAIR);
+  for (; s < n; s++) op(JOP_STEP);
+  if (pair_res) op(JOP_STEP_RESIDUAL);
+  else if (residual) op(JOP_RESIDUAL);
+}
+
+void smooth(Ctx& c, Amg& A, Level& l, int steps, bool zero, bool residual = false) {
   const long n = (long)A.F * l.nv;
-  if (steps <= 0) { if (zero) PNP_CUDA(cudaMemsetAsync(l.x.p, 0, n * sizeof(double), c.stream)); return; }
-  if (A.smoother == 0) {
-    int s = 0;
-    if (zero) { jacobi0(c, A, l, A.omega, nullptr); s = 1; }
-    for (; s < steps; s++) { level_op<2>(c, A, l, l.x.p, l.b.p, l.x2.p); std::swap(l.x.p, l.x2.p); }
+  if (steps <= 0) {
+    if (zero) PNP_CUDA(cudaMemsetAsync(l.x.p, 0, n * sizeof(double), c.stream));
+  } else if (A.smoother == 0) {
+    jacobi_schedule(steps, zero, residual, fuse_ok(c, A, l), [&](int op) {
+      switch (op) {
+        case JOP_ZERO: jacobi0(c, A, l, A.omega, nullptr); break;
+        case JOP_STEP: level_op<2>(c, A, l, l.x.p, l.b.p, l.x2.p); std::swap(l.x.p, l.x2.p); break;
+        case JOP_PAIR: level_pair<EPI_JACOBI>(c, A, l); std::swap(l.x.p, l.r.p); break;
+        case JOP_STEP_RESIDUAL: level_pair<EPI_RESIDUAL>(c, A, l); std::swap(l.x.p, l.x2.p); break;
+        default: level_op<1>(c, A, l, l.x.p, l.b.p, l.r.p);
+      }
+    });
     return;
-  }
-  if (A.smoother == 2) {
+  } else if (A.smoother == 2) {
     const bool finest = &l == A.L[0].get();
     const SweepView V{l.rp, l.col, finest ? c.int2ext.p : nullptr, l.nv};
     if (!l.gs_plan) l.gs_plan = sweep_plan_build(c, V, A.F);
@@ -891,20 +991,21 @@
       sweep_gs(c, *l.gs_plan, V, l.vals, l.nslots, l.b.p, l.x.p, -1);
     }
     c.acct(finest ? Ctx::ACC_SPMV_FINE : Ctx::ACC_SPMV_COARSE, 2.0 * steps * ((8.0 * A.NP + 4.0) * (double)l.nslots + 24.0 * n));
-    return;
-  }
-  const double lmx = 1.1 * l.lmax, lmn = l.lmax / A.cheb_ratio;
-  const double theta = 0.5 * (lmx + lmn), delta = 0.5 * (lmx - lmn), sigma = theta / delta;
-  double rho = 1.0 / sigma;
-  int s = 0;
-  if (zero) { jacobi0(c, A, l, 1.0 / theta, l.r.p); s = 1; }
-  else { level_op<3>(c, A, l, l.x.p, l.b.p, l.x2.p, 1.0 / theta, 0.0, l.r.p); std::swap(l.x.p, l.x2.p); s = 1; }
-  for (; s < steps; s++) {
-    const double rho_new = 1.0 / (2.0 * sigma - rho);
-    level_op<3>(c, A, l, l.x.p, l.b.p, l.x2.p, 2.0 * rho_new / delta, rho_new * rho, l.r.p);
-    std::swap(l.x.p, l.x2.p);
-    rho = rho_new;
-  }
+  } else {
+    const double lmx = 1.1 * l.lmax, lmn = l.lmax / A.cheb_ratio;
+    const double theta = 0.5 * (lmx + lmn), delta = 0.5 * (lmx - lmn), sigma = theta / delta;
+    double rho = 1.0 / sigma;
+    int s = 0;
+    if (zero) { jacobi0(c, A, l, 1.0 / theta, l.r.p); s = 1; }
+    else { level_op<3>(c, A, l, l.x.p, l.b.p, l.x2.p, 1.0 / theta, 0.0, l.r.p); std::swap(l.x.p, l.x2.p); s = 1; }
+    for (; s < steps; s++) {
+      const double rho_new = 1.0 / (2.0 * sigma - rho);
+      level_op<3>(c, A, l, l.x.p, l.b.p, l.x2.p, 2.0 * rho_new / delta, rho_new * rho, l.r.p);
+      std::swap(l.x.p, l.x2.p);
+      rho = rho_new;
+    }
+  }
+  if (residual) level_op<1>(c, A, l, l.x.p, l.b.p, l.r.p);
 }
 
 void cycle(Ctx& c, Amg& A, int li, int nu, int comp0, bool zero);
@@ -914,18 +1015,18 @@
     const int visits = 0 < A.wlevels ? A.gamma : 1;
     for (int g = 0; g < visits; g++) cycle(c, A, 1, nu, comp0, g == 0);
   };
-  auto snapshot = [&](std::vector<std::pair<double*, double*>>& v) {
+  auto snapshot = [&](std::vector<std::array<double*, 3>>& v) {
     v.clear();
-    for (size_t li = 1; li < A.L.size(); li++) v.push_back({A.L[li]->x.p, A.L[li]->x2.p});
+    for (size_t li = 1; li < A.L.size(); li++) v.push_back({A.L[li]->x.p, A.L[li]->x2.p, A.L[li]->r.p});
   };
-  auto restore = [&](const std::vector<std::pair<double*, double*>>& v) {
-    for (size_t li = 1; li < A.L.size(); li++) { A.L[li]->x.p = v[li - 1].first; A.L[li]->x2.p = v[li - 1].second; }
+  auto restore = [&](const std::vector<std::array<double*, 3>>& v) {
+    for (size_t li = 1; li < A.L.size(); li++) { A.L[li]->x.p = v[li - 1][0]; A.L[li]->x2.p = v[li - 1][1]; A.L[li]->r.p = v[li - 1][2]; }
   };
   cudaStreamCaptureStatus cap = cudaStreamCaptureStatusNone;
   PNP_CUDA(cudaStreamIsCapturing(c.stream, &cap));
   if (!tune().graph || A.cg_failed || A.smoother != 0 || cap != cudaStreamCaptureStatusNone) { direct(); return; }
-  const double key[8] = {(double)nu, A.omega, (double)A.gamma, (double)A.wlevels, (double)A.pre_steps, (double)A.post_steps,
-                         (double)A.coarse_sweeps, (double)comp0 + 16.0 * A.dense_n};
+  const double key[9] = {(double)nu, A.omega, (double)A.gamma, (double)A.wlevels, (double)A.pre_steps, (double)A.post_steps,
+                         (double)A.coarse_sweeps, (double)comp0 + 16.0 * A.dense_n, (double)(tune().mg_fuse && !c.mg_fuse_off)};
   if (A.cg_exec && std::memcmp(key, A.cg_key, sizeof key) != 0) A.cg_reset();
   if (!A.cg_exec) {
     if (A.cg_calls++ < 1) { direct(); return; }
@@ -977,10 +1078,9 @@
     return;
   }
   const int nu_pre = A.pre_steps >= 0 ? A.pre_steps : nu, nu_post = A.post_steps >= 0 ? A.post_steps : nu;
-  smooth(c, A, l, coarsest ? A.coarse_sweeps : nu_pre, zero);
+  smooth(c, A, l, coarsest ? A.coarse_sweeps : nu_pre, zero, !coarsest);
   if (coarsest) return;
   Level& nx = *A.L[li + 1];
-  level_op<1>(c, A, l, l.x.p, l.b.p, l.r.p);
   if (A.distributed) halo_exchange(*l.lc, l.r.p, A.F);
   if (A.F == 1) KL(c, k_restrict<1>, nx.nv, l.agg_ptr.p, l.agg_mem.p, l.par1.p, nx.nv, l.r.p, nx.b.p);
   else KL(c, k_restrict<3>, nx.nv, l.agg_ptr.p, l.agg_mem.p, l.par1.p, nx.nv, l.r.p, nx.b.p);
@@ -1003,6 +1103,15 @@
   smooth(c, A, l, nu_post, false);
 }
 
+}
+
+double amg_fuse_fact(const Solver& S, int which) {
+  if (!S.amg || S.amg->L.empty()) return which == 0 ? 0 : -1;
+  const Amg& A = *S.amg;
+  if (which == 1) return A.L[0]->fuse_grid ? A.L[0]->fuse_nrows : -1;
+  int n = 0;
+  for (auto& l : A.L) n += l->fuse_grid ? 1 : 0;
+  return n;
 }
 
 int amg_graph_state(const Solver& S) { return !S.amg ? 0 : (S.amg->cg_exec ? 1 : (S.amg->cg_failed ? -1 : 0)); }
@@ -1059,6 +1168,7 @@
       const size_t nall = (size_t)A.F * c.nv;
       l0r.x.alloc(nall); l0r.x2.alloc(nall);
       l0r.x.zero(c.stream); l0r.x2.zero(c.stream);
+      for (auto& l : A.L) fuse_build(c, A, *l);
     }
     A.symbolic = true;
     if (S.verbosity > 0) {
@@ -1068,6 +1178,15 @@
     }
   }
   A.L[0]->vals = M.vals.p;
+  if (A.fuse_err.n) {
+    int e = 0;
+    A.fuse_err.download(&e, 1, c.stream);
+    if (e) {
+      c.mg_fuse_off = true;
+      A.fuse_err.zero(c.stream);
+      PNP_REQUIRE(false, PNP_E_CUDA, "multigrid: a paired smoother launch timed out waiting for its first step; single launches from now on");
+    }
+  }
   static const bool timing = std::getenv("PNP_AMG_TIMING") != nullptr;
   if (timing) PNP_CUDA(cudaStreamSynchronize(c.stream));
   const auto t_num0 = std::chrono::steady_clock::now();
@@ -1093,15 +1212,28 @@
   const long n = (long)A.F * l0.nv;
   const int nu = S.prec_steps > 0 ? S.prec_steps : 1;
   if (c.n_own == c.nv) {
-    double *keep_b = l0.b.p, *keep_x = l0.x.p, *keep_x2 = l0.x2.p;
+    double *keep_b = l0.b.p, *keep_x = l0.x.p, *keep_x2 = l0.x2.p, *keep_r = l0.r.p;
     const int pre = A.pre_steps >= 0 ? A.pre_steps : nu, post = A.post_steps >= 0 ? A.post_steps : nu;
-    const int swaps = A.smoother == 2 ? 0 : (pre > 0 ? pre - 1 : 0) + post;
     struct Restore {
-      Level& l; double *b, *x, *x2;
-      ~Restore() { l.b.p = b; l.x.p = x; l.x2.p = x2; }
-    } restore{l0, keep_b, keep_x, keep_x2};
+      Level& l; double *b, *x, *x2, *r;
+      ~Restore() { l.b.p = b; l.x.p = x; l.x2.p = x2; l.r.p = r; }
+    } restore{l0, keep_b, keep_x, keep_x2, keep_r};
     l0.b.p = const_cast<double*>(d);
-    if (swaps & 1) l0.x2.p = y; else l0.x.p = y;
+    if (A.smoother == 0) {
+      int pos[3] = {0, 1, 2};
+      const bool paired = fuse_ok(c, A, l0);
+      auto rotate = [&](int op) {
+        if (op == JOP_PAIR) std::swap(pos[0], pos[2]);
+        else if (op == JOP_STEP || op == JOP_STEP_RESIDUAL) std::swap(pos[0], pos[1]);
+      };
+      if (pre > 0) jacobi_schedule(pre, true, true, paired, rotate);
+      if (post > 0) jacobi_schedule(post, false, false, paired, rotate);
+      double** role[3] = {&l0.x.p, &l0.x2.p, &l0.r.p};
+      *role[pos[0]] = y;
+    } else {
+      const int swaps = A.smoother == 2 ? 0 : (pre > 0 ? pre - 1 : 0) + post;
+      if (swaps & 1) l0.x2.p = y; else l0.x.p = y;
+    }
     cycle(c, A, 0, nu, A.comp0, true);
     double* result = l0.x.p;
     if (result != y) { PNP_CUDA(cudaMemcpyAsync(y, result, n * sizeof(double), cudaMemcpyDeviceToDevice, c.stream)); c.acct(Ctx::ACC_BLAS1, 16.0 * n); }
diff --git a/dune_pnp_b200/csrc/pnp_capi.cu b/dune_pnp_b200/csrc/pnp_capi.cu
--- a/dune_pnp_b200/csrc/pnp_capi.cu
+++ b/dune_pnp_b200/csrc/pnp_capi.cu
@@ -7,6 +7,7 @@
 namespace pnp {
 int newton_apply(Ctx&, const Operator&, Vec&, Solver&, const pnp_newton_opts&, pnp_newton_result&);
 int amg_graph_state(const Solver&);
+double amg_fuse_fact(const Solver&, int which);
 LinResult slp_apply(Ctx&, const Operator&, Vec&, Solver&, double, int, double);
 int onestep_apply(Ctx&, int, const Operator&, const Operator&, Solver&, double, Vec&, Vec&, Vec&, double, int, double, LinResult*);
 namespace {
@@ -183,8 +184,22 @@
   for (size_t i = 0; i + 1 < c.prof_used; i += 2) {
     float t = 0; PNP_CUDA(cudaEventElapsedTime(&t, c.prof_ev[i], c.prof_ev[i + 1]));
     const int k = c.prof_kind[i / 2];
+    if (k >= 3) continue;
     if (launches) launches[k]++;
     if (total_ms) total_ms[k] += t;
+  }
+  API_END
+}
+pnp_status pnp_profile_spmv_fused_get(pnp_ctx* ctx, long* launches, double* total_ms) {
+  API_BEGIN(ctx)
+  PNP_CUDA(cudaStreamSynchronize(c.stream));
+  if (launches) *launches = 0;
+  if (total_ms) *total_ms = 0;
+  for (size_t i = 0; i + 1 < c.prof_used; i += 2) {
+    if (c.prof_kind[i / 2] != 3) continue;
+    float t = 0; PNP_CUDA(cudaEventElapsedTime(&t, c.prof_ev[i], c.prof_ev[i + 1]));
+    if (launches) ++*launches;
+    if (total_ms) *total_ms += t;
   }
   API_END
 }
@@ -226,6 +241,8 @@
   else if (n == "jac_compact") t.jac_compact = value != 0;
   else if (n == "p2_chunk") t.p2_chunk = (long)value;
   else if (n == "tma_min_rows") t.tma_min_rows = (long)value;
+  else if (n == "mg_fuse") t.mg_fuse = value != 0;
+  else if (n == "mg_fuse_lag" && (value == 1 || value == 2)) t.mg_fuse_lag = (int)value;
   else return PNP_E_ARG;
   return PNP_OK;
 }
@@ -542,6 +559,8 @@
   else if (n == "ssor_levels") *value = sweep_levels(c.solver(s), false);
   else if (n == "ilu0_levels") *value = sweep_levels(c.solver(s), true);
   else if (n == "amg_graph") *value = amg_graph_state(c.solver(s));
+  else if (n == "amg_fuse_levels") *value = amg_fuse_fact(c.solver(s), 0);
+  else if (n == "amg_fuse_deferred") *value = amg_fuse_fact(c.solver(s), 1);
   else PNP_REQUIRE(false, PNP_E_ARG, "unknown solver fact");
   API_END
 }
diff --git a/dune_pnp_b200/csrc/pnp_common.cuh b/dune_pnp_b200/csrc/pnp_common.cuh
--- a/dune_pnp_b200/csrc/pnp_common.cuh
+++ b/dune_pnp_b200/csrc/pnp_common.cuh
@@ -67,6 +67,8 @@
   int fd_warp = 1;
   int jac_compact = 1;
   long p2_chunk = 0;
+  int mg_fuse = 1;
+  int mg_fuse_lag = 2;
 };
 inline Tune& tune() { static Tune t; return t; }
 
@@ -207,6 +209,7 @@
   std::vector<MgLevelRef> mg;
   DBuf<int> mg_gid; long mg_nglobal = 0; bool mg_aggregated = false;
   Ctx* mg_replica = nullptr;
+  bool mg_fuse_off = false;
   long mg_epoch = 0;
   Ctx* parent = nullptr;
   std::vector<Ctx*> children;
diff --git a/dune_pnp_b200/csrc/pnp_fuse.cuh b/dune_pnp_b200/csrc/pnp_fuse.cuh
--- /dev/null
+++ b/dune_pnp_b200/csrc/pnp_fuse.cuh
@@ -0,0 +1,30 @@
+#pragma once
+#include "pnp_setup_algos.cuh"
+
+namespace pnp {
+
+constexpr int FUSE_TILE_ROWS = 128;
+constexpr int FUSE_HAS_DEFERRED = 1 << 30;
+
+PNP_HD bool fuse_row_deferred(const int* rp, const unsigned* col, int row, int lim_tile) {
+  for (int s = rp[row]; s < rp[row + 1]; s++)
+    if ((int)((col[s] & STAR_VMASK) / FUSE_TILE_ROWS) > lim_tile) return true;
+  return false;
+}
+
+PNP_HD int fuse_tile_deps(const int* rp, const unsigned* col, int nv, int t, int reach, int* lo, int* hi) {
+  const int ntiles = (nv + FUSE_TILE_ROWS - 1) / FUSE_TILE_ROWS;
+  const int r0 = t * FUSE_TILE_ROWS, r1 = r0 + FUSE_TILE_ROWS < nv ? r0 + FUSE_TILE_ROWS : nv;
+  int l = t > 0 ? t - 1 : 0, h = t + 1 < ntiles ? t + 1 : ntiles - 1, ndef = 0;
+  for (int r = r0; r < r1; r++) {
+    if (fuse_row_deferred(rp, col, r, t + reach)) { ndef++; continue; }
+    for (int s = rp[r]; s < rp[r + 1]; s++) {
+      const int u = (int)((col[s] & STAR_VMASK) / FUSE_TILE_ROWS);
+      l = u < l ? u : l; h = u > h ? u : h;
+    }
+  }
+  *lo = l; *hi = h;
+  return ndef;
+}
+
+}
diff --git a/dune_pnp_b200/csrc/pnp_spmv_tma.cuh b/dune_pnp_b200/csrc/pnp_spmv_tma.cuh
--- a/dune_pnp_b200/csrc/pnp_spmv_tma.cuh
+++ b/dune_pnp_b200/csrc/pnp_spmv_tma.cuh
@@ -1,4 +1,7 @@
 #pragma once
+#include <climits>
+
+#include "pnp_fuse.cuh"
 #include "pnp_spmv.cuh"
 
 namespace pnp {
@@ -85,8 +88,318 @@
   else block_mac<NP>(v, x, acc);
 }
 
+template <int NP, int EPI, int NDOT>
+__device__ __forceinline__ void tma_produce(const StarOpArgs& a, unsigned char* st, int t, int lo, int hi, int role, uint64_t* bar) {
+  using L = TmaLayout<NP>;
+  constexpr int F = L::F;
+  const int sp = (int)(a.stride & 1);
+  const int r0 = t * TMA_TR, rows = min(TMA_TR, a.nv - r0);
+  const bool staged = hi - lo <= TMA_CAP;
+  const void* src = nullptr; void* dst = nullptr; unsigned nb = 0;
+  if (role < NP) {
+    if (staged) {
+      const int o = (lo + role * sp) & 1;
+      nb = (unsigned)(((hi - lo + o) + 1) & ~1) * 8u;
+      src = a.vals + (size_t)role * a.stride + (lo - o); dst = st + role * L::PLANE;
+    }
+  } else if (role == NP) {
+    if (staged) {
+      const int lo_c = lo & ~3;
+      nb = (unsigned)(((hi - lo_c) + 3) & ~3) * 4u;
+      src = a.col + lo_c; dst = st + L::COLS;
+    }
+  } else if (role == NP + 1) {
+    nb = (unsigned)((rows + 1 + 3) & ~3) * 4u;
+    src = a.rp + r0; dst = st + L::RP;
+  } else if (role == NP + 2) {
+    const int wlo = max(r0 - TMA_W, 0), whi = min(r0 + TMA_TR + TMA_W, a.nv);
+    nb = (unsigned)((F * (whi - wlo) + 1) & ~1) * 8u;
+    src = a.x + (size_t)F * wlo; dst = st + L::XW;
+  } else {
+    nb = (unsigned)((F * rows + 1) & ~1) * 8u;
+    src = (EPI == EPI_PLAIN ? a.w1 : a.b) + (size_t)F * r0; dst = st + L::B;
+  }
+  if (nb) { mbar_expect_tx(bar, nb); bulk_g2s(dst, src, nb, bar); }
+  else mbar_arrive(bar);
+}
+
+struct TmaTileBounds {
+  int cur_lo, cur_hi, nxt_lo, nxt_hi;
+  __device__ void load(const StarOpArgs& a, int ntiles, int batch, int lane, int& lo, int& hi) {
+    const long tt = blockIdx.x + (long)(batch * 32 + lane) * gridDim.x;
+    lo = 0; hi = 0;
+    if (tt < ntiles) { lo = a.rp[tt * TMA_TR]; hi = a.rp[min((int)tt * TMA_TR + TMA_TR, a.nv)]; }
+  }
+  __device__ void init(const StarOpArgs& a, int ntiles, int lane) {
+    load(a, ntiles, 0, lane, cur_lo, cur_hi);
+    load(a, ntiles, 1, lane, nxt_lo, nxt_hi);
+  }
+  __device__ void next(const StarOpArgs& a, int ntiles, int j, int lane, int& lo, int& hi) {
+    if (j > 0 && (j & 31) == 0) { cur_lo = nxt_lo; cur_hi = nxt_hi; load(a, ntiles, j / 32 + 1, lane, nxt_lo, nxt_hi); }
+    lo = __shfl_sync(0xffffffffu, cur_lo, j & 31); hi = __shfl_sync(0xffffffffu, cur_hi, j & 31);
+  }
+};
+
+template <int NP, int EPI, int NDOT>
+__device__ __forceinline__ void tma_epilogue(const StarOpArgs& a, const double* acc, const double* dg, const double* bv,
+                                             const double* xo, double* yv, double* dsum) {
+  constexpr int F = NP == 1 ? 1 : 3;
+  if (EPI == EPI_PLAIN) {
+#pragma unroll
+    for (int k = 0; k < F; k++) {
+      yv[k] = acc[k];
+      if (NDOT >= 1) dsum[0] += acc[k] * bv[k];
+      if (NDOT >= 2) dsum[NDOT >= 2 ? 1 : 0] += acc[k] * acc[k];
+    }
+  } else if (EPI == EPI_RESIDUAL) {
+#pragma unroll
+    for (int k = 0; k < F; k++) yv[k] = bv[k] - acc[k];
+  } else {
+    double r[F], z[F];
+#pragma unroll
+    for (int k = 0; k < F; k++) r[k] = bv[k] - acc[k];
+    if constexpr (F == 3) {
+#pragma unroll
+      for (int k = 0; k < F; k++) {
+        double o[3];
+        block_inverse_row<NP>(dg, k, o);
+        z[k] = o[0] * r[0] + o[1] * r[1] + o[2] * r[2];
+      }
+    } else z[0] = (dg[0] != 0.0 ? 1.0 / dg[0] : 0.0) * r[0];
+#pragma unroll
+    for (int k = 0; k < F; k++) yv[k] = xo[k] + a.omega * z[k];
+  }
+}
+
+template <int NP, int EPI, int NDOT, int LPR, bool DEFER>
+__device__ __forceinline__ void tma_consume_tile(const StarOpArgs& a, const unsigned char* st, int t, int warp, int lane,
+                                                 double* ybuf, double* dsum, int lim) {
+  using L = TmaLayout<NP>;
+  constexpr int F = L::F;
+  constexpr int RW = 32 / LPR;
+  const int sp = (int)(a.stride & 1);
+  const int sub = lane % LPR;
+  double* yw = ybuf + warp * RW * F;
+  const double* sv = reinterpret_cast<const double*>(st);
+  const unsigned* sc = reinterpret_cast<const unsigned*>(st + L::COLS);
+  const int* srp = reinterpret_cast<const int*>(st + L::RP);
+  const double* sb = reinterpret_cast<const double*>(st + L::B);
+  const double* sx = reinterpret_cast<const double*>(st + L::XW);
+  const int r0 = t * TMA_TR, rows = min(TMA_TR, a.nv - r0);
+  const int wlo = max(r0 - TMA_W, 0);
+  const unsigned wn = (unsigned)(min(r0 + TMA_TR + TMA_W, a.nv) - wlo);
+  const double* sxo = sx + (size_t)F * (r0 - wlo);
+  const int lo = srp[0], hi = srp[rows];
+  const bool staged = hi - lo <= TMA_CAP;
+  const int cbase = lo & ~3;
+  int vb[NP];
+#pragma unroll
+  for (int p = 0; p < NP; p++) vb[p] = p * (TMA_CAP + 2) - lo + ((lo + p * sp) & 1);
+  const int rl = RW * warp + lane / LPR;
+  const bool valid = rl < rows;
+  const int b0 = valid ? srp[rl] : hi, e0 = valid ? srp[rl + 1] : hi;
+  double acc[F], dg[NP];
+#pragma unroll
+  for (int k = 0; k < F; k++) acc[k] = 0.0;
+#pragma unroll
+  for (int p = 0; p < NP; p++) dg[p] = 0.0;
+  const int len = e0 - b0;
+  const int maxlen = __reduce_max_sync(0xffffffffu, len);
+  unsigned deferred = 0;
+  if (staged) {
+    constexpr int MAXS = (8 + LPR - 1) / LPR;
+    unsigned cj[MAXS];
+    bool okj[MAXS];
+    double xj[MAXS][F];
+#pragma unroll
+    for (int u = 0; u < MAXS; u++) {
+      const int j = sub + u * LPR;
+      okj[u] = j < len;
+      cj[u] = okj[u] ? (sc[b0 + j - cbase] & STAR_VMASK) : 0u;
+    }
+#pragma unroll
+    for (int u = 0; u < MAXS; u++) {
+      const unsigned cw = cj[u] - (unsigned)wlo;
+      const bool in = cw < wn;
+      const bool ldg = okj[u] && !in, lds = okj[u] && in;
+#pragma unroll
+      for (int k = 0; k < F; k++) {
+        double xg = 0.0, xs = 0.0;
+        if (ldg) xg = a.x[(size_t)F * cj[u] + k];
+        if (lds) xs = sx[F * cw + k];
+        xj[u][k] = in ? xs : xg;
+      }
+    }
+#pragma unroll
+    for (int u = 0; u < MAXS; u++) {
+      const int s = b0 + sub + u * LPR;
+      double v[NP];
+#pragma unroll
+      for (int p = 0; p < NP; p++) v[p] = okj[u] ? sv[vb[p] + s] : 0.0;
+      if (EPI == EPI_JACOBI && u == 0) {
+#pragma unroll
+        for (int p = 0; p < NP; p++) dg[p] = v[p];
+      }
+      if constexpr (NP == 1) acc[0] += v[0] * xj[u][0];
+      else block_mac<NP>(v, xj[u], acc);
+    }
+    for (int j = sub + MAXS * LPR; j < maxlen; j += LPR)
+      slot_product<NP, true>(a, j < len, b0 + j, sv, vb, sc, cbase, sx, wlo, wn, acc, nullptr);
+    if (DEFER && lim != INT_MAX) {
+      bool d = false;
+      for (int j = sub; j < len; j += LPR) d |= (int)((sc[b0 + j - cbase] & STAR_VMASK) / TMA_TR) > lim;
+      deferred = __ballot_sync(0xffffffffu, d);
+    }
+  } else {
+    slot_product<NP, false>(a, sub < len, b0 + sub, sv, vb, sc, cbase, sx, wlo, wn, acc, EPI == EPI_JACOBI ? dg : nullptr);
+    for (int j = sub + LPR; j < maxlen; j += LPR)
+      slot_product<NP, false>(a, j < len, b0 + j, sv, vb, sc, cbase, sx, wlo, wn, acc, nullptr);
+  }
+  if (LPR > 1) {
+#pragma unroll
+    for (int k = 0; k < F; k++)
+#pragma unroll
+      for (int o = LPR / 2; o > 0; o >>= 1) acc[k] += __shfl_xor_sync(0xffffffffu, acc[k], o);
+  }
+  const bool mine = valid && sub == 0;
+  double yv[F];
+#pragma unroll
+  for (int k = 0; k < F; k++) yv[k] = 0.0;
+  if (mine) tma_epilogue<NP, EPI, NDOT>(a, acc, dg, sb + F * rl, sxo + F * rl, yv, dsum);
+  if (sub == 0) {
+#pragma unroll
+    for (int k = 0; k < F; k++) yw[F * (lane / LPR) + k] = yv[k];
+  }
+  __syncwarp();
+  {
+    const size_t g0 = (size_t)F * (r0 + RW * warp);
+    const size_t gend = (size_t)F * a.nv;
+#pragma unroll
+    for (int i = lane; i < RW * F; i += 32)
+      if (g0 + i < gend && !(DEFER && ((deferred >> (i / F * LPR)) & ((1u << LPR) - 1u)))) a.y[g0 + i] = yw[i];
+  }
+}
+
 template <int NP, int EPI, int NDOT, int LPR>
 __global__ void __launch_bounds__(tma_threads(NP, EPI, NDOT, LPR), 1) k_star_op_tma(const StarOpArgs a, const int nstages) {
+  using L = TmaLayout<NP>;
+  constexpr int TMA_NW = tma_nw(LPR);
+  extern __shared__ __align__(128) unsigned char smem[];
+  uint64_t* full = reinterpret_cast<uint64_t*>(smem);
+  uint64_t* empty = full + TMA_MAX_STAGES;
+  unsigned char* stages = smem + L::HEAD;
+  double* ybuf = reinterpret_cast<double*>(stages + (size_t)nstages * L::STAGE);
+  const int warp = threadIdx.x >> 5, lane = threadIdx.x & 31;
+  const int ntiles = (a.nv + TMA_TR - 1) / TMA_TR;
+  if (threadIdx.x == 0) {
+    for (int s = 0; s < nstages; s++) { mbar_init(&full[s], tma_producers(NP, EPI, NDOT)); mbar_init(&empty[s], TMA_NW); }
+    asm volatile("fence.mbarrier_init.release.cluster;" ::: "memory");
+  }
+  __syncthreads();
+  double dsum[NDOT > 0 ? NDOT : 1];
+#pragma unroll
+  for (int j = 0; j < (NDOT > 0 ? NDOT : 1); j++) dsum[j] = 0.0;
+
+  if (warp >= TMA_NW) {
+    const int role = warp - TMA_NW;
+    TmaTileBounds tb;
+    tb.init(a, ntiles, lane);
+    int t = blockIdx.x;
+    for (int it = 0; t < ntiles; t += gridDim.x, it++) {
+      int lo, hi;
+      tb.next(a, ntiles, it, lane, lo, hi);
+      if (lane == 0) {
+        const int stage = it % nstages;
+        const unsigned parity = (unsigned)((it / nstages) & 1);
+        mbar_wait(&empty[stage], parity ^ 1u);
+        tma_produce<NP, EPI, NDOT>(a, stages + (size_t)stage * L::STAGE, t, lo, hi, role, &full[stage]);
+      }
+      __syncwarp();
+    }
+  } else {
+    int t = blockIdx.x;
+    for (int it = 0; t < ntiles; t += gridDim.x, it++) {
+      const int stage = it % nstages;
+      const unsigned parity = (unsigned)((it / nstages) & 1);
+      mbar_wait(&full[stage], parity);
+      tma_consume_tile<NP, EPI, NDOT, LPR, false>(a, stages + (size_t)stage * L::STAGE, t, warp, lane, ybuf, dsum, INT_MAX);
+      __syncwarp();
+      if (lane == 0) mbar_arrive(&empty[stage]);
+    }
+  }
+  if (NDOT > 0) {
+    __shared__ double sm[NDOT > 0 ? NDOT : 1][TMA_NW];
+#pragma unroll
+    for (int j = 0; j < (NDOT > 0 ? NDOT : 1); j++) {
+      double s = dsum[j];
+#pragma unroll
+      for (int o = 16; o > 0; o >>= 1) s += __shfl_xor_sync(0xffffffffu, s, o);
+      if (lane == 0 && warp < TMA_NW) sm[j][warp] = s;
+    }
+    __syncthreads();
+    if (warp == 0) {
+#pragma unroll
+      for (int j = 0; j < (NDOT > 0 ? NDOT : 1); j++) {
+        double s = lane < TMA_NW ? sm[j][lane] : 0.0;
+#pragma unroll
+        for (int o = 16; o > 0; o >>= 1) s += __shfl_xor_sync(0xffffffffu, s, o);
+        if (lane == 0) a.partial[(long)blockIdx.x * NDOT + j] = s;
+      }
+    }
+  }
+}
+
+struct FuseArgs {
+  double* out;
+  const int2* dep;
+  const int* deferred; int ndeferred;
+  unsigned long long* prog;
+  unsigned* gen;
+  int* err;
+  int lag;
+  int reach;
+};
+static_assert(FUSE_TILE_ROWS == TMA_TR, "pnp_fuse.cuh tiles are the streaming SpMV's tiles");
+
+__device__ __forceinline__ unsigned long long ld_acquire_u64(const unsigned long long* p) {
+  unsigned long long v;
+  asm volatile("ld.acquire.gpu.global.u64 %0, [%1];" : "=l"(v) : "l"(p) : "memory");
+  return v;
+}
+__device__ __forceinline__ void st_release_u64(unsigned long long* p, unsigned long long v) {
+  asm volatile("st.release.gpu.global.u64 [%0], %1;" ::"l"(p), "l"(v) : "memory");
+}
+constexpr long FUSE_SPIN_CAP = 1l << 22;
+
+__device__ __forceinline__ bool fuse_ready(const FuseArgs& f, unsigned long long epoch, int lo, int hi, int lane) {
+  const int G = gridDim.x, n = min(hi - lo + 1, G);
+  bool ok = true;
+  for (int i = lane; i < n; i += 32) {
+    const int u = hi - i;
+    ok = ok && ld_acquire_u64(&f.prog[u % G]) >= (epoch | (unsigned)(u / G + 1));
+  }
+  return __all_sync(0xffffffffu, ok);
+}
+__device__ __forceinline__ bool fuse_give_up(const FuseArgs& f, long spin, int lane) {
+  if (!__any_sync(0xffffffffu, spin >= FUSE_SPIN_CAP || *(volatile int*)f.err != 0)) return false;
+  if (lane == 0) atomicExch(f.err, 1);
+  return true;
+}
+__device__ __forceinline__ bool fuse_wait(const FuseArgs& f, unsigned long long epoch, int lo, int hi, int lane) {
+  unsigned ns = 64;
+  for (long spin = 0;; spin++) {
+    if (fuse_ready(f, epoch, lo, hi, lane)) return true;
+    if (fuse_give_up(f, spin, lane)) return false;
+    __nanosleep(ns);
+    if (ns < 1024) ns *= 2;
+  }
+}
+
+constexpr int fuse_threads(int np, int lpr) { return tma_threads(np, EPI_JACOBI, 0, lpr) + 32; }
+
+template <int NP, int EPI2, int LPR>
+__global__ void __launch_bounds__(fuse_threads(NP, LPR), 1)
+k_star_op2_tma(const StarOpArgs a, const FuseArgs f, const int nstages) {
   using L = TmaLayout<NP>;
   constexpr int F = L::F;
   constexpr int TMA_NW = tma_nw(LPR);
@@ -97,217 +410,136 @@
   unsigned char* stages = smem + L::HEAD;
   double* ybuf = reinterpret_cast<double*>(stages + (size_t)nstages * L::STAGE);
   const int warp = threadIdx.x >> 5, lane = threadIdx.x & 31;
-  const int ntiles = (a.nv + TMA_TR - 1) / TMA_TR;
-  const int sp = (int)(a.stride & 1);
+  const int G = gridDim.x, ntiles = (a.nv + TMA_TR - 1) / TMA_TR;
+  const int n1 = (ntiles - (int)blockIdx.x + G - 1) / G;
+  const unsigned long long epoch = (unsigned long long)(*(volatile unsigned*)f.gen + 1u) << 32;
+  StarOpArgs a2 = a;
+  a2.x = a.y; a2.y = f.out;
+  constexpr int NPROD = tma_producers(NP, EPI_JACOBI, 0);
+  __shared__ unsigned done_warps;
+  __shared__ unsigned ready_tiles;
   if (threadIdx.x == 0) {
-    for (int s = 0; s < nstages; s++) { mbar_init(&full[s], tma_producers(NP, EPI, NDOT)); mbar_init(&empty[s], TMA_NW); }
+    done_warps = 0; ready_tiles = 0;
+    for (int s = 0; s < nstages; s++) { mbar_init(&full[s], tma_producers(NP, EPI_JACOBI, 0)); mbar_init(&empty[s], TMA_NW); }
     asm volatile("fence.mbarrier_init.release.cluster;" ::: "memory");
   }
   __syncthreads();
-  double dsum[NDOT > 0 ? NDOT : 1];
-#pragma unroll
-  for (int j = 0; j < (NDOT > 0 ? NDOT : 1); j++) dsum[j] = 0.0;
-
-  if (warp >= TMA_NW) {
+  double dsum[1] = {0.0};
+  const int nq = 2 * (n1 + f.lag);
+  auto task = [&](int q, int& j) { j = (q & 1) ? q / 2 - f.lag : q / 2; return j >= 0 && j < n1; };
+
+  if (warp == TMA_NW + NPROD) {
+    const unsigned sa = smem_u32(&done_warps), sr = smem_u32(&ready_tiles);
+    int pub = 0, ready = 0;
+    long spin = 0;
+    bool gave_up = false;
+    while (pub < n1 || ready < n1) {
+      bool idle = true;
+      unsigned v = 0;
+      if (lane == 0) asm volatile("ld.acquire.cta.shared::cta.u32 %0, [%1];" : "=r"(v) : "r"(sa) : "memory");
+      const int done = (int)(__shfl_sync(0xffffffffu, v, 0) / TMA_NW);
+      if (done > pub) {
+        pub = done; idle = false;
+        if (lane == 0) st_release_u64(&f.prog[blockIdx.x], epoch | (unsigned)pub);
+      }
+      if (ready < n1) {
+        const int2 d = f.dep[blockIdx.x + ready * G];
+        bool ok = gave_up || fuse_ready(f, epoch, d.x, d.y & ~FUSE_HAS_DEFERRED, lane);
+        if (!ok && fuse_give_up(f, ++spin, lane)) ok = gave_up = true;
+        if (ok) {
+          ready++; spin = 0; idle = false;
+          if (lane == 0) asm volatile("st.release.cta.shared::cta.u32 [%0], %1;" ::"r"(sr), "r"((unsigned)ready) : "memory");
+        }
+      }
+      if (idle) __nanosleep(64);
+    }
+    __syncwarp();
+  } else if (warp >= TMA_NW) {
     const int role = warp - TMA_NW;
-    auto load_batch = [&](int batch, int& lo, int& hi) {
-      const long tt = blockIdx.x + (long)(batch * 32 + lane) * gridDim.x;
-      lo = 0; hi = 0;
-      if (tt < ntiles) { lo = a.rp[tt * TMA_TR]; hi = a.rp[min((int)tt * TMA_TR + TMA_TR, a.nv)]; }
-    };
-    int cur_lo, cur_hi, nxt_lo, nxt_hi;
-    load_batch(0, cur_lo, cur_hi);
-    load_batch(1, nxt_lo, nxt_hi);
-    int t = blockIdx.x;
-    for (int it = 0; t < ntiles; t += gridDim.x, it++) {
-      if (it > 0 && (it & 31) == 0) { cur_lo = nxt_lo; cur_hi = nxt_hi; load_batch(it / 32 + 1, nxt_lo, nxt_hi); }
-      const int lo = __shfl_sync(0xffffffffu, cur_lo, it & 31), hi = __shfl_sync(0xffffffffu, cur_hi, it & 31);
+    TmaTileBounds tb1, tb2;
+    tb1.init(a, ntiles, lane); tb2.init(a, ntiles, lane);
+    int it = 0;
+    for (int q = 0; q < nq; q++) {
+      int j;
+      if (!task(q, j)) continue;
+      const bool two = q & 1;
+      const int t = blockIdx.x + j * G;
+      int lo, hi;
+      (two ? tb2 : tb1).next(a, ntiles, j, lane, lo, hi);
+      if (two && role == NP + 2 && lane == 0) {
+        const unsigned sr = smem_u32(&ready_tiles);
+        unsigned r;
+        do asm volatile("ld.acquire.cta.shared::cta.u32 %0, [%1];" : "=r"(r) : "r"(sr) : "memory");
+        while ((int)r <= j);
+        asm volatile("fence.proxy.async.global;" ::: "memory");
+      }
       if (lane == 0) {
         const int stage = it % nstages;
-        const unsigned parity = (unsigned)((it / nstages) & 1);
-        mbar_wait(&empty[stage], parity ^ 1u);
-        unsigned char* st = stages + (size_t)stage * L::STAGE;
-        const int r0 = t * TMA_TR, rows = min(TMA_TR, a.nv - r0);
-        const bool staged = hi - lo <= TMA_CAP;
-        const void* src = nullptr; void* dst = nullptr; unsigned nb = 0;
-        if (role < NP) {
-          if (staged) {
-            const int o = (lo + role * sp) & 1;
-            nb = (unsigned)(((hi - lo + o) + 1) & ~1) * 8u;
-            src = a.vals + (size_t)role * a.stride + (lo - o); dst = st + role * L::PLANE;
-          }
-        } else if (role == NP) {
-          if (staged) {
-            const int lo_c = lo & ~3;
-            nb = (unsigned)(((hi - lo_c) + 3) & ~3) * 4u;
-            src = a.col + lo_c; dst = st + L::COLS;
-          }
-        } else if (role == NP + 1) {
-          nb = (unsigned)((rows + 1 + 3) & ~3) * 4u;
-          src = a.rp + r0; dst = st + L::RP;
-        } else if (role == NP + 2) {
-          const int wlo = max(r0 - TMA_W, 0), whi = min(r0 + TMA_TR + TMA_W, a.nv);
-          nb = (unsigned)((F * (whi - wlo) + 1) & ~1) * 8u;
-          src = a.x + (size_t)F * wlo; dst = st + L::XW;
-        } else {
-          nb = (unsigned)((F * rows + 1) & ~1) * 8u;
-          src = (EPI == EPI_PLAIN ? a.w1 : a.b) + (size_t)F * r0; dst = st + L::B;
-        }
-        if (nb) { mbar_expect_tx(&full[stage], nb); bulk_g2s(dst, src, nb, &full[stage]); }
-        else mbar_arrive(&full[stage]);
+        mbar_wait(&empty[stage], (unsigned)((it / nstages) & 1) ^ 1u);
+        tma_produce<NP, EPI_JACOBI, 0>(two ? a2 : a, stages + (size_t)stage * L::STAGE, t, lo, hi, role, &full[stage]);
       }
       __syncwarp();
+      it++;
     }
   } else {
-    const int sub = lane % LPR;
-    double* yw = ybuf + warp * RW * F;
-    int t = blockIdx.x;
-    for (int it = 0; t < ntiles; t += gridDim.x, it++) {
+    int it = 0;
+    for (int q = 0; q < nq; q++) {
+      int j;
+      if (!task(q, j)) continue;
+      const int t = blockIdx.x + j * G;
       const int stage = it % nstages;
-      const unsigned parity = (unsigned)((it / nstages) & 1);
-      mbar_wait(&full[stage], parity);
+      mbar_wait(&full[stage], (unsigned)((it / nstages) & 1));
       const unsigned char* st = stages + (size_t)stage * L::STAGE;
-      const double* sv = reinterpret_cast<const double*>(st);
-      const unsigned* sc = reinterpret_cast<const unsigned*>(st + L::COLS);
-      const int* srp = reinterpret_cast<const int*>(st + L::RP);
-      const double* sb = reinterpret_cast<const double*>(st + L::B);
-      const double* sx = reinterpret_cast<const double*>(st + L::XW);
-      const int r0 = t * TMA_TR, rows = min(TMA_TR, a.nv - r0);
-      const int wlo = max(r0 - TMA_W, 0);
-      const unsigned wn = (unsigned)(min(r0 + TMA_TR + TMA_W, a.nv) - wlo);
-      const double* sxo = sx + (size_t)F * (r0 - wlo);
-      const int lo = srp[0], hi = srp[rows];
-      const bool staged = hi - lo <= TMA_CAP;
-      const int cbase = lo & ~3;
-      int vb[NP];
-#pragma unroll
-      for (int p = 0; p < NP; p++) vb[p] = p * (TMA_CAP + 2) - lo + ((lo + p * sp) & 1);
-      const int rl = RW * warp + lane / LPR;
-      const bool valid = rl < rows;
-      const int b0 = valid ? srp[rl] : hi, e0 = valid ? srp[rl + 1] : hi;
-      double acc[F], dg[NP];
-#pragma unroll
-      for (int k = 0; k < F; k++) acc[k] = 0.0;
-#pragma unroll
-      for (int p = 0; p < NP; p++) dg[p] = 0.0;
-      const int len = e0 - b0;
-      const int maxlen = __reduce_max_sync(0xffffffffu, len);
-      if (staged) {
-        constexpr int MAXS = (8 + LPR - 1) / LPR;
-        unsigned cj[MAXS];
-        bool okj[MAXS];
-        double xj[MAXS][F];
-#pragma unroll
-        for (int u = 0; u < MAXS; u++) {
-          const int j = sub + u * LPR;
-          okj[u] = j < len;
-          cj[u] = okj[u] ? (sc[b0 + j - cbase] & STAR_VMASK) : 0u;
-        }
-#pragma unroll
-        for (int u = 0; u < MAXS; u++) {
-          const unsigned cw = cj[u] - (unsigned)wlo;
-          const bool in = cw < wn;
-          const bool ldg = okj[u] && !in, lds = okj[u] && in;
-#pragma unroll
-          for (int k = 0; k < F; k++) {
-            double xg = 0.0, xs = 0.0;
-            if (ldg) xg = a.x[(size_t)F * cj[u] + k];
-            if (lds) xs = sx[F * cw + k];
-            xj[u][k] = in ? xs : xg;
-          }
-        }
-#pragma unroll
-        for (int u = 0; u < MAXS; u++) {
-          const int s = b0 + sub + u * LPR;
-          double v[NP];
-#pragma unroll
-          for (int p = 0; p < NP; p++) v[p] = okj[u] ? sv[vb[p] + s] : 0.0;
-          if (EPI == EPI_JACOBI && u == 0) {
-#pragma unroll
-            for (int p = 0; p < NP; p++) dg[p] = v[p];
-          }
-          if constexpr (NP == 1) acc[0] += v[0] * xj[u][0];
-          else block_mac<NP>(v, xj[u], acc);
-        }
-        for (int j = sub + MAXS * LPR; j < maxlen; j += LPR)
-          slot_product<NP, true>(a, j < len, b0 + j, sv, vb, sc, cbase, sx, wlo, wn, acc, nullptr);
+      if (!(q & 1)) {
+        tma_consume_tile<NP, EPI_JACOBI, 0, LPR, false>(a, st, t, warp, lane, ybuf, dsum, INT_MAX);
+        __syncwarp();
+        if (lane == 0) asm volatile("red.release.cta.shared::cta.add.u32 [%0], 1;" ::"r"(smem_u32(&done_warps)) : "memory");
       } else {
-        slot_product<NP, false>(a, sub < len, b0 + sub, sv, vb, sc, cbase, sx, wlo, wn, acc, EPI == EPI_JACOBI ? dg : nullptr);
-        for (int j = sub + LPR; j < maxlen; j += LPR)
-          slot_product<NP, false>(a, j < len, b0 + j, sv, vb, sc, cbase, sx, wlo, wn, acc, nullptr);
-      }
-      if (LPR > 1) {
-#pragma unroll
-        for (int k = 0; k < F; k++)
-#pragma unroll
-          for (int o = LPR / 2; o > 0; o >>= 1) acc[k] += __shfl_xor_sync(0xffffffffu, acc[k], o);
-      }
-      const bool mine = valid && sub == 0;
-      double yv[F];
-#pragma unroll
-      for (int k = 0; k < F; k++) yv[k] = 0.0;
-      if (mine) {
-        if (EPI == EPI_PLAIN) {
-#pragma unroll
-          for (int k = 0; k < F; k++) {
-            yv[k] = acc[k];
-            if (NDOT >= 1) dsum[0] += acc[k] * sb[F * rl + k];
-            if (NDOT >= 2) dsum[NDOT >= 2 ? 1 : 0] += acc[k] * acc[k];
-          }
-        } else if (EPI == EPI_RESIDUAL) {
-#pragma unroll
-          for (int k = 0; k < F; k++) yv[k] = sb[F * rl + k] - acc[k];
-        } else {
-          double r[F], z[F];
-#pragma unroll
-          for (int k = 0; k < F; k++) r[k] = sb[F * rl + k] - acc[k];
-          if constexpr (F == 3) {
-#pragma unroll
-            for (int k = 0; k < F; k++) {
-              double o[3];
-              block_inverse_row<NP>(dg, k, o);
-              z[k] = o[0] * r[0] + o[1] * r[1] + o[2] * r[2];
-            }
-          } else z[0] = (dg[0] != 0.0 ? 1.0 / dg[0] : 0.0) * r[0];
-#pragma unroll
-          for (int k = 0; k < F; k++) yv[k] = sxo[F * rl + k] + a.omega * z[k];
-        }
-      }
-      if (sub == 0) {
-#pragma unroll
-        for (int k = 0; k < F; k++) yw[F * (lane / LPR) + k] = yv[k];
-      }
-      __syncwarp();
-      {
-        const size_t g0 = (size_t)F * (r0 + RW * warp);
-        const size_t gend = (size_t)F * a.nv;
-#pragma unroll
-        for (int i = lane; i < RW * F; i += 32)
-          if (g0 + i < gend) a.y[g0 + i] = yw[i];
+        const int2 d = f.dep[t];
+        tma_consume_tile<NP, EPI2, 0, LPR, true>(a2, st, t, warp, lane, ybuf, dsum,
+                                                 (d.y & FUSE_HAS_DEFERRED) ? t + f.reach : INT_MAX);
       }
       __syncwarp();
       if (lane == 0) mbar_arrive(&empty[stage]);
-    }
-  }
-  if (NDOT > 0) {
-    __shared__ double sm[NDOT > 0 ? NDOT : 1][TMA_NW];
-#pragma unroll
-    for (int j = 0; j < (NDOT > 0 ? NDOT : 1); j++) {
-      double s = dsum[j];
-#pragma unroll
-      for (int o = 16; o > 0; o >>= 1) s += __shfl_xor_sync(0xffffffffu, s, o);
-      if (lane == 0 && warp < TMA_NW) sm[j][warp] = s;
-    }
-    __syncthreads();
-    if (warp == 0) {
-#pragma unroll
-      for (int j = 0; j < (NDOT > 0 ? NDOT : 1); j++) {
-        double s = lane < TMA_NW ? sm[j][lane] : 0.0;
-#pragma unroll
-        for (int o = 16; o > 0; o >>= 1) s += __shfl_xor_sync(0xffffffffu, s, o);
-        if (lane == 0) a.partial[(long)blockIdx.x * NDOT + j] = s;
-      }
-    }
+      it++;
+    }
+  }
+  if (f.ndeferred > 0 && fuse_wait(f, epoch, 0, ntiles - 1, lane)) {
+    const int nw = blockDim.x >> 5, sub = lane % LPR;
+    for (int base = ((int)blockIdx.x * nw + warp) * RW; base < f.ndeferred; base += G * nw * RW) {
+      const int k = base + lane / LPR;
+      const bool valid = k < f.ndeferred;
+      const int row = valid ? f.deferred[k] : 0;
+      const int b0 = valid ? a2.rp[row] : 0, len = valid ? a2.rp[row + 1] - b0 : 0;
+      const int maxlen = __reduce_max_sync(0xffffffffu, len);
+      double acc[F], dg[NP];
+#pragma unroll
+      for (int c = 0; c < F; c++) acc[c] = 0.0;
+#pragma unroll
+      for (int p = 0; p < NP; p++) dg[p] = 0.0;
+      for (int jj = sub; jj < maxlen; jj += LPR)
+        slot_product<NP, false>(a2, jj < len, b0 + jj, nullptr, nullptr, nullptr, 0, nullptr, 0, 0u, acc,
+                                EPI2 == EPI_JACOBI && jj == sub ? dg : nullptr);
+      if (LPR > 1) {
+#pragma unroll
+        for (int c = 0; c < F; c++)
+#pragma unroll
+          for (int o = LPR / 2; o > 0; o >>= 1) acc[c] += __shfl_xor_sync(0xffffffffu, acc[c], o);
+      }
+      if (valid && sub == 0) {
+        double bv[F], xo[F], yv[F];
+#pragma unroll
+        for (int c = 0; c < F; c++) { bv[c] = a2.b[(size_t)F * row + c]; xo[c] = a2.x[(size_t)F * row + c]; }
+        tma_epilogue<NP, EPI2, 0>(a2, acc, dg, bv, xo, yv, nullptr);
+#pragma unroll
+        for (int c = 0; c < F; c++) a2.y[(size_t)F * row + c] = yv[c];
+      }
+    }
+  }
+  __syncthreads();
+  if (threadIdx.x == 0) {
+    __threadfence();
+    if (atomicAdd(&f.gen[1], 1u) == (unsigned)G - 1u) { f.gen[1] = 0; f.gen[0] = (unsigned)(epoch >> 32); }
   }
 }
 
@@ -345,6 +577,34 @@
   return tune().tma_lpr == 2 ? launch_star_op_tma_lpr<NP, EPI, NDOT, 2>(c, a) : launch_star_op_tma_lpr<NP, EPI, NDOT, 1>(c, a);
 }
 
+template <int NP, int EPI2, int LPR>
+inline bool launch_star_op2_tma_lpr(Ctx& c, const StarOpArgs& a, const FuseArgs& f, int grid) {
+  using L = TmaLayout<NP>;
+  const int nstages = star_op_tma_stages();
+  static unsigned long long configured = 0;
+  if (!(configured >> (c.device & 63) & 1ull)) {
+    PNP_CUDA(cudaFuncSetAttribute(k_star_op2_tma<NP, EPI2, LPR>, cudaFuncAttributeMaxDynamicSharedMemorySize, L::smem_bytes(TMA_MAX_STAGES)));
+    configured |= 1ull << (c.device & 63);
+  }
+  cudaLaunchAttribute attr[1];
+  attr[0].id = cudaLaunchAttributeCooperative;
+  attr[0].val.cooperative = 1;
+  cudaLaunchConfig_t cfg = {};
+  cfg.gridDim = dim3(grid); cfg.blockDim = dim3(fuse_threads(NP, LPR));
+  cfg.dynamicSmemBytes = L::smem_bytes(nstages); cfg.stream = c.stream; cfg.attrs = attr; cfg.numAttrs = 1;
+  if (cudaLaunchKernelEx(&cfg, k_star_op2_tma<NP, EPI2, LPR>, a, f, nstages) != cudaSuccess) { cudaGetLastError(); return false; }
+  c.launches++;
+  return true;
+}
+template <int EPI2>
+inline bool launch_star_op2_tma(Ctx& c, int nplanes, const StarOpArgs& a, const FuseArgs& f, int grid) {
+  const bool l2 = tune().tma_lpr == 2;
+  if (nplanes == 1) return l2 ? launch_star_op2_tma_lpr<1, EPI2, 2>(c, a, f, grid) : launch_star_op2_tma_lpr<1, EPI2, 1>(c, a, f, grid);
+  if (nplanes == PNP_COMPACT_PLANES)
+    return l2 ? launch_star_op2_tma_lpr<PNP_COMPACT_PLANES, EPI2, 2>(c, a, f, grid) : launch_star_op2_tma_lpr<PNP_COMPACT_PLANES, EPI2, 1>(c, a, f, grid);
+  return l2 ? launch_star_op2_tma_lpr<7, EPI2, 2>(c, a, f, grid) : launch_star_op2_tma_lpr<7, EPI2, 1>(c, a, f, grid);
+}
+
 template <int EPI, int NDOT>
 inline double star_op_bytes(int nplanes, const StarOpArgs& a) {
   const double F = nplanes == 1 ? 1 : 3, nv = a.nv, ns = a.rp ? (double)a.stride : 0.0;
diff --git a/include/pnp_b200.h b/include/pnp_b200.h
--- a/include/pnp_b200.h
+++ b/include/pnp_b200.h
@@ -34,6 +34,7 @@
 
 pnp_status pnp_profile_spmv(pnp_ctx*, int enable);
 pnp_status pnp_profile_spmv_get(pnp_ctx*, long* launches, double* total_ms);
+pnp_status pnp_profile_spmv_fused_get(pnp_ctx*, long* launches, double* total_ms);
 pnp_status pnp_profile_bytes(pnp_ctx*, int reset, double* out6);
 pnp_status pnp_profiler_range(pnp_ctx*, int start);
 pnp_status pnp_timer_start(pnp_ctx*);
```

New measurement: 280.3 million (median of 6 runs). 0.635x the previous value.
